# open-policy-agent/gatekeeper

Measured on AMD Instinct MI355X. Metric: AdmissionReview x constraint evals/sec, higher is better.
Workload: dtype u32; 1 GPU; configs[2]: pkg/audit sweep, 50 constraints x 1000000 mixed synthetic cluster objects (80% Pod, 10% Deployment, 5% Namespace, 5% Service/ConfigMap); constraints=50, reviews_total=1000000, reviews_rank0=1000000, rows_rank0=15859334, table_bytes_rank0=529437232, parallelism=1 GPU

## Files before the change

### gatekeeper_amd/_lib.py

```python
from __future__ import annotations

import atexit
import ctypes as C
import os

_HERE = os.path.dirname(os.path.abspath(__file__))
_ROOT = os.path.dirname(_HERE)

GK_OK = 0
GK_ERR_INVALID, GK_ERR_REGO, GK_ERR_UNSUPPORTED, GK_ERR_NOT_FOUND, GK_ERR_DEVICE, GK_ERR_REVIEW, GK_ERR_INTERNAL, GK_ERR_LIMIT = (
    -1, -2, -3, -4, -5, -6, -7, -8)
GK_REVIEW_ADMISSION_REQUEST, GK_REVIEW_OBJECT = 0, 1
GK_SRC_EMPTY, GK_SRC_ORIGINAL, GK_SRC_GENERATED, GK_SRC_ALL, GK_SRC_INVALID = 0, 1, 2, 3, 4
GK_TABLE_KEEP_DOCS = 1
GK_TABLE_RESIDENT = 2
GK_TABLE_KEEP_TEXT = 16
GK_TABLE_PRUNED = 32
GK_TABLE_PRE_MATCHED = 64
GK_TABLE_PROCESS_AUDIT = 4
GK_TABLE_PROCESS_WEBHOOK = 8
GK_REVIEW_EXCLUDED = 1
GK_EVAL_WANT_MATCH, GK_EVAL_NO_DOWNLOAD, GK_EVAL_WANT_LIST, GK_EVAL_ASYNC, GK_EVAL_COLLECT, GK_EVAL_TIME_EACH, GK_EVAL_KERNEL_ONLY = 1, 2, 4, 8, 16, 32, 64
GK_EVAL_DEVICE_ONLY = 128
GK_SWEEP_RESULT_TOTALS = 1
GK_VIOLATIONS_RENDER = 1

EXPORTS = [
    "gk_engine_create", "gk_engine_destroy", "gk_last_error", "gk_version", "gk_template_add", "gk_template_remove",
    "gk_constraint_add", "gk_constraint_remove", "gk_data_put", "gk_data_remove", "gk_excluder_replace", "gk_excluder_excluded", "gk_table_create", "gk_table_free",
    "gk_table_eval", "gk_eval_free", "gk_render", "gk_render_error", "gk_free", "gk_dump", "gk_table_topk", "gk_topk_free",
    "gk_table_totals", "gk_totals_free", "gk_table_get_stats", "gk_batcher_start", "gk_batcher_stop", "gk_query", "gk_query_ex", "gk_query_ex2",
    "gk_resident_sweep", "gk_sweep_free", "gk_resident_review", "gk_resident_review_ex", "gk_resident_audit", "gk_audit_free",
    "gk_resident_violations", "gk_violations_free", "gk_table_verify", "gk_verify_free", "gk_resident_verify",
    "gk_comm_unique_id", "gk_comm_init", "gk_comm_destroy", "gk_comm_info", "gk_table_sweep_sharded", "gk_shard_free",
    "gk_jit_quiesce", "gk_jit_cache_stats", "gk_jit_cache_dir", "gk_jit_cache_drop_memory", "gk_host_cpus", "gk_table_create_spool", "gk_spool_info_free", "gk_debug_set",
    "gk_synth_batch_create", "gk_synth_batch_reviews", "gk_synth_batch_size", "gk_synth_batch_json_bytes", "gk_synth_batch_free", "gk_synth_query_storm", "gk_synth_query_storm_ex",
]


GK_OPT_NO_REFERENTIAL, GK_OPT_GATHER_STATS, GK_OPT_TRACE = 1, 2, 4
GK_QUERY_TRACE = 1
GK_QUERY_PRE_MATCHED = 2


class gk_opts(C.Structure):
    _fields_ = [("device", C.c_int32), ("elem_cap", C.c_uint16 * 3), ("reserved", C.c_uint16), ("flags", C.c_uint32), ("reserved2", C.c_uint32),
                ("disabled_builtins", C.POINTER(C.c_char_p)), ("n_disabled_builtins", C.c_size_t)]


class gk_review_in(C.Structure):
    _fields_ = [("kind", C.c_int32), ("source", C.c_int32),
                ("json", C.c_char_p), ("json_len", C.c_size_t),
                ("namespace_json", C.c_char_p), ("namespace_len", C.c_size_t),
                ("ns_object_json", C.c_char_p), ("ns_object_len", C.c_size_t),
                ("operation", C.c_char_p)]


class gk_eval_out(C.Structure):
    _fields_ = [("n_reviews", C.c_uint32), ("n_constraints", C.c_uint32), ("n_tiles", C.c_uint32),
                ("constraint_ids", C.POINTER(C.c_uint32)),
                ("viol", C.POINTER(C.c_uint64)), ("err", C.POINTER(C.c_uint64)), ("match", C.POINTER(C.c_uint64)),
                ("too_big", C.POINTER(C.c_uint64)), ("counts", C.POINTER(C.c_uint32)), ("list", C.POINTER(C.c_uint32)),
                ("list_len", C.c_uint32), ("list_total", C.c_uint32), ("n_overflow", C.c_uint32),
                ("kernel_ms", C.c_float), ("fast_kernel_ms", C.c_float),
                ("algo_bytes", C.c_uint64), ("n_rows", C.c_uint64), ("n_launches", C.c_uint32), ("lds_bytes", C.c_uint32),
                ("d_viol", C.c_void_p), ("d_err", C.c_void_p), ("d_counts", C.c_void_p), ("n_rows_read", C.c_uint64),
                ("algo_bytes_once", C.c_uint64), ("n_plan_groups", C.c_uint32), ("n_host_evaluated", C.c_uint32),
                ("host_evaluated", C.POINTER(C.c_uint32)), ("kernel_text_hash", C.c_uint64)]


class gk_topk_out(C.Structure):
    _fields_ = [("n_constraints", C.c_uint32), ("stride", C.c_uint32), ("constraint_ids", C.POINTER(C.c_uint32)),
                ("counts", C.POINTER(C.c_uint32)), ("reviews", C.POINTER(C.c_uint32)), ("overflow", C.POINTER(C.c_uint32))]


class gk_totals_out(C.Structure):
    _fields_ = [("n_constraints", C.c_uint32), ("constraint_ids", C.POINTER(C.c_uint32)), ("results", C.POINTER(C.c_uint64)),
                ("pairs", C.POINTER(C.c_uint64)), ("rendered_pairs", C.c_uint64)]


class gk_table_stats(C.Structure):
    _fields_ = [("n_reviews", C.c_uint64), ("n_rows", C.c_uint64), ("json_bytes", C.c_uint64), ("heap_bytes", C.c_uint64),
                ("device_bytes", C.c_uint64), ("flatten_s", C.c_double), ("upload_s", C.c_double), ("host_threads", C.c_uint32),
                ("reserved", C.c_uint32), ("fast_reviews", C.c_uint64), ("digest", C.c_uint64)]


class gk_sweep_out(C.Structure):
    _fields_ = [("n_objects", C.c_uint64), ("n_constraints", C.c_uint32), ("n_chunks", C.c_uint32), ("constraint_ids", C.POINTER(C.c_uint32)),
                ("pairs", C.POINTER(C.c_uint64)), ("results", C.POINTER(C.c_uint64)), ("flattened", C.c_uint64), ("beyond_limits", C.c_uint64),
                ("sync_s", C.c_double), ("eval_s", C.c_double)]


class gk_audit_out(C.Structure):
    _fields_ = [("n_objects", C.c_uint64), ("n_constraints", C.c_uint32), ("stride", C.c_uint32), ("n_chunks", C.c_uint32),
                ("constraint_ids", C.POINTER(C.c_uint32)), ("pairs", C.POINTER(C.c_uint64)), ("results", C.POINTER(C.c_uint64)),
                ("counts", C.POINTER(C.c_uint32)), ("objects", C.POINTER(C.c_uint32)), ("overflow", C.POINTER(C.c_uint32)),
                ("n_paths", C.c_uint32), ("paths", C.POINTER(C.c_char_p)), ("beyond_limits", C.c_uint64), ("err_pairs", C.POINTER(C.c_uint64))]


class gk_violations_out(C.Structure):
    _fields_ = [("n_objects", C.c_uint64), ("n_constraints", C.c_uint32), ("n_chunks", C.c_uint32), ("mask_words", C.c_uint32),
                ("constraint_ids", C.POINTER(C.c_uint32)), ("total_objects", C.c_uint64), ("n_entries", C.c_uint32), ("paths", C.POINTER(C.c_char_p)),
                ("viol", C.POINTER(C.c_uint64)), ("err", C.POINTER(C.c_uint64)), ("results_json", C.POINTER(C.c_char_p)),
                ("beyond_limits", C.c_uint64), ("next_cursor", C.c_uint64)]


class gk_verify_entry(C.Structure):
    _fields_ = [("kind", C.c_uint32), ("row", C.c_uint32), ("review", C.c_uint32), ("specialised_bit", C.c_uint32)]


class gk_verify_out(C.Structure):
    _fields_ = [("n_reviews", C.c_uint32), ("n_constraints", C.c_uint32), ("n_plan_groups", C.c_uint32), ("constraint_ids", C.POINTER(C.c_uint32)),
                ("specialised_groups", C.c_uint32), ("kernel_text_hash", C.c_uint64),
                ("diff_viol", C.POINTER(C.c_uint64)), ("diff_err", C.POINTER(C.c_uint64)), ("diff_match", C.POINTER(C.c_uint64)),
                ("diff_too_big", C.c_uint64), ("diff_total", C.c_uint64), ("n_entries", C.c_uint32), ("entries_total", C.c_uint64),
                ("entries", C.POINTER(gk_verify_entry)), ("quarantined_groups", C.c_uint32),
                ("specialised_ms", C.c_float), ("bytecode_ms", C.c_float), ("diff_ms", C.c_float)]


GK_VERIFY_WANT_MATCH = 1
GK_VERIFY_QUARANTINE = 2
GK_VERIFY_KINDS = ("viol", "err", "match", "too_big")


class gk_shard_out(C.Structure):
    _fields_ = [("world", C.c_uint32), ("rank", C.c_uint32), ("n_constraints", C.c_uint32), ("stride_tiles", C.c_uint32), ("slot_bytes", C.c_uint64),
                ("constraint_ids", C.POINTER(C.c_uint32)), ("shard_reviews", C.POINTER(C.c_uint32)), ("totals", C.POINTER(C.c_int64)),
                ("gathered", C.POINTER(C.c_uint64)), ("d_gathered", C.c_void_p), ("kernel_ms", C.c_float), ("fast_kernel_ms", C.c_float),
                ("n_overflow", C.c_uint32), ("err_totals", C.POINTER(C.c_int64)), ("beyond_limits", C.c_int64), ("not_evaluated", C.c_int64),
                ("exchange_ms", C.c_float), ("exchange_overlapped", C.c_uint32), ("exchange_bytes_inbound", C.c_uint64)]


GK_SHARD_DOWNLOAD = 1
GK_SHARD_ENQUEUE = 2
GK_SHARD_COLLECT = 4
GK_COMM_ID_BYTES = 128
HE_ALLGATHER = C.CFUNCTYPE(None, C.c_void_p, C.c_void_p, C.c_uint64)
HE_ALLREDUCE = C.CFUNCTYPE(None, C.c_void_p, C.POINTER(C.c_longlong), C.c_uint64)


class gk_spool_info(C.Structure):
    _fields_ = [("n_files", C.c_uint64), ("n_reviews", C.c_uint64), ("n_unreadable", C.c_uint64), ("n_namespace_missing", C.c_uint64), ("bytes", C.c_uint64),
                ("names", C.POINTER(C.c_char_p)), ("n_folders_missing", C.c_uint64), ("statuses", C.POINTER(C.c_int32)), ("n_rejected", C.c_uint64),
                ("n_excluded", C.c_uint64)]


class gk_batch_opts(C.Structure):
    _fields_ = [("max_batch", C.c_uint32), ("window_us", C.c_uint32), ("workers", C.c_uint32), ("reserved", C.c_uint32)]


class gk_storm_out(C.Structure):
    _fields_ = [("calls", C.c_uint64), ("errors", C.c_uint64), ("seconds", C.c_double), ("p50_us", C.c_double), ("p90_us", C.c_double),
                ("p99_us", C.c_double), ("max_us", C.c_double), ("mean_batch", C.c_double), ("mean_queue_us", C.c_double),
                ("mean_device_us", C.c_double), ("results", C.c_uint64)]


class gk_query_stats(C.Structure):
    _fields_ = [("batch_size", C.c_uint32), ("reserved", C.c_uint32), ("queue_us", C.c_double), ("device_us", C.c_double),
                ("total_us", C.c_double)]


class EngineLoadError(RuntimeError):
    pass


def library_path(hostemu: bool = False) -> str:
    if hostemu:
        return os.path.join(_ROOT, "tests", "native", "libgkgpu_hostemu.so")
    return os.path.join(_HERE, "libgkgpu.so")


_cache = {}


def load(hostemu: bool | None = None):
    hostemu = bool(hostemu)
    if hostemu in _cache:
        return _cache[hostemu]
    path = library_path(hostemu)
    if not os.path.exists(path):
        raise EngineLoadError(
            "%s not found: build it with `python -c 'import __graft_entry__ as g; g.build()'` "
            "(there is no CPU fallback for the constraint-evaluation path)" % path)
    if not hostemu:
        try:
            import torch
        except ImportError:
            pass
    lib = C.CDLL(path)
    vp, cp, sz, u32 = C.c_void_p, C.c_char_p, C.c_size_t, C.c_uint32
    lib.gk_engine_create.argtypes = [C.POINTER(gk_opts), C.POINTER(vp)]
    lib.gk_engine_destroy.argtypes = [vp]
    lib.gk_engine_destroy.restype = None
    lib.gk_last_error.restype = cp
    lib.gk_version.restype = cp
    lib.gk_host_cpus.argtypes = []
    lib.gk_host_cpus.restype = C.c_uint32
    lib.gk_template_add.argtypes = [vp, cp, cp, C.POINTER(cp), sz]
    lib.gk_template_remove.argtypes = [vp, cp]
    lib.gk_constraint_add.argtypes = [vp, cp, sz, C.POINTER(u32)]
    lib.gk_constraint_remove.argtypes = [vp, cp, cp]
    lib.gk_data_put.argtypes = [vp, C.POINTER(cp), sz, cp, sz]
    lib.gk_data_remove.argtypes = [vp, C.POINTER(cp), sz]
    lib.gk_excluder_replace.argtypes = [vp, C.c_char_p, sz]
    lib.gk_excluder_excluded.argtypes = [vp, C.c_char_p, C.POINTER(gk_review_in), C.POINTER(C.c_int32)]
    lib.gk_table_create.argtypes = [vp, C.POINTER(gk_review_in), sz, u32, C.POINTER(C.c_int32), C.POINTER(vp)]
    lib.gk_table_free.argtypes = [vp]
    lib.gk_table_free.restype = None
    lib.gk_table_create_spool.argtypes = [vp, cp, cp, u32, u32, C.POINTER(C.POINTER(gk_spool_info)), C.POINTER(vp)]
    lib.gk_spool_info_free.argtypes = [C.POINTER(gk_spool_info)]
    lib.gk_spool_info_free.restype = None
    lib.gk_jit_quiesce.argtypes = []
    lib.gk_jit_quiesce.restype = None
    lib.gk_jit_cache_stats.argtypes = [C.POINTER(C.c_uint64), C.POINTER(C.c_uint64)]
    lib.gk_jit_cache_stats.restype = None
    lib.gk_jit_cache_dir.argtypes = []
    lib.gk_jit_cache_dir.restype = C.c_char_p
    lib.gk_jit_cache_drop_memory.argtypes = []
    lib.gk_jit_cache_drop_memory.restype = None
    lib.gk_table_eval.argtypes = [vp, vp, u32, C.POINTER(C.POINTER(gk_eval_out))]
    lib.gk_eval_free.argtypes = [C.POINTER(gk_eval_out)]
    lib.gk_eval_free.restype = None
    lib.gk_render.argtypes = [vp, vp, u32, u32, C.POINTER(vp)]
    lib.gk_render_error.argtypes = [vp, vp, u32, u32, C.POINTER(vp)]
    lib.gk_free.argtypes = [vp]
    lib.gk_free.restype = None
    lib.gk_dump.argtypes = [vp, C.POINTER(vp)]
    lib.gk_table_topk.argtypes = [vp, vp, u32, C.POINTER(C.POINTER(gk_topk_out))]
    lib.gk_topk_free.argtypes = [C.POINTER(gk_topk_out)]
    lib.gk_topk_free.restype = None
    lib.gk_comm_unique_id.argtypes = [C.c_char_p]
    lib.gk_comm_init.argtypes = [vp, C.c_char_p, C.c_int, C.c_int]
    lib.gk_comm_destroy.argtypes = [vp]
    lib.gk_comm_destroy.restype = None
    lib.gk_comm_info.argtypes = [vp, C.POINTER(C.c_int32), C.POINTER(C.c_int32)]
    lib.gk_table_sweep_sharded.argtypes = [vp, vp, u32, C.POINTER(C.POINTER(gk_shard_out))]
    lib.gk_shard_free.argtypes = [C.POINTER(gk_shard_out)]
    lib.gk_shard_free.restype = None
    if hostemu:
        lib.gk_comm_init_host.argtypes = [vp, C.c_int, C.c_int, HE_ALLGATHER, HE_ALLREDUCE, vp]
    lib.gk_resident_sweep.argtypes = [vp, u32, C.POINTER(C.POINTER(gk_sweep_out))]
    lib.gk_sweep_free.argtypes = [C.POINTER(gk_sweep_out)]
    lib.gk_sweep_free.restype = None
    lib.gk_resident_review.argtypes = [vp, C.POINTER(cp), sz, C.POINTER(vp)]
    lib.gk_resident_audit.argtypes = [vp, u32, u32, C.POINTER(C.POINTER(gk_audit_out))]
    lib.gk_audit_free.argtypes = [C.POINTER(gk_audit_out)]
    lib.gk_audit_free.restype = None
    lib.gk_resident_violations.argtypes = [vp, C.c_uint64, u32, u32, C.POINTER(C.POINTER(gk_violations_out))]
    lib.gk_violations_free.argtypes = [C.POINTER(gk_violations_out)]
    lib.gk_violations_free.restype = None
    lib.gk_table_verify.argtypes = [vp, vp, u32, u32, C.POINTER(C.POINTER(gk_verify_out))]
    lib.gk_verify_free.argtypes = [C.POINTER(gk_verify_out)]
    lib.gk_verify_free.restype = None
    lib.gk_resident_verify.argtypes = [vp, u32, u32, C.POINTER(C.POINTER(gk_verify_out)), C.POINTER(C.POINTER(cp))]
    lib.gk_batcher_start.argtypes = [vp, C.POINTER(gk_batch_opts)]
    lib.gk_batcher_stop.argtypes = [vp]
    lib.gk_batcher_stop.restype = None
    lib.gk_query.argtypes = [vp, C.POINTER(gk_review_in), C.POINTER(vp), C.POINTER(gk_query_stats)]
    lib.gk_query_ex.argtypes = [vp, C.POINTER(gk_review_in), u32, C.POINTER(vp), C.POINTER(vp), C.POINTER(gk_query_stats)]
    lib.gk_query_ex2.argtypes = [vp, C.POINTER(gk_review_in), C.POINTER(u32), sz, u32, C.POINTER(vp), C.POINTER(vp), C.POINTER(gk_query_stats)]
    lib.gk_resident_review_ex.argtypes = [vp, C.POINTER(cp), sz, C.POINTER(u32), sz, u32, C.POINTER(vp)]
    lib.gk_debug_set.argtypes = [cp, C.c_int64]
    lib.gk_table_get_stats.argtypes = [vp, C.POINTER(gk_table_stats)]
    lib.gk_table_totals.argtypes = [vp, vp, C.POINTER(C.POINTER(gk_totals_out))]
    lib.gk_totals_free.argtypes = [C.POINTER(gk_totals_out)]
    lib.gk_totals_free.restype = None
    lib.gk_synth_batch_create.argtypes = [C.c_uint64, C.c_uint64, C.c_uint64, C.c_int, C.POINTER(cp), sz, C.POINTER(vp)]
    lib.gk_synth_batch_reviews.argtypes = [vp]
    lib.gk_synth_batch_reviews.restype = C.POINTER(gk_review_in)
    lib.gk_synth_batch_size.argtypes = [vp]
    lib.gk_synth_batch_size.restype = sz
    lib.gk_synth_batch_json_bytes.argtypes = [vp]
    lib.gk_synth_batch_json_bytes.restype = C.c_uint64
    lib.gk_synth_batch_free.argtypes = [vp]
    lib.gk_synth_batch_free.restype = None
    lib.gk_synth_query_storm.argtypes = [vp, vp, u32, u32, C.POINTER(gk_storm_out)]
    lib.gk_synth_query_storm_ex.argtypes = [vp, vp, u32, u32, C.POINTER(u32), sz, u32, C.POINTER(gk_storm_out)]
    atexit.register(lib.gk_jit_quiesce)
    _cache[hostemu] = lib
    return lib
```

### gatekeeper_amd/csrc/device.hpp

```cpp
#pragma once
#include <cstdint>
#include <string>
#include <vector>

#include "flatten.hpp"
#include "lower.hpp"
#include "verify_merge.hpp"

namespace gk {

struct DevTable;
struct DevPlan;

struct EvalOptions {
  bool download = true;
  bool want_match = false;
  uint32_t list_capacity = 0;
  bool shard = false;
  bool detached = false;
  bool kernel_only = false;
  bool time_each = false;
  bool timed = true;
  bool jit_wait = true;
  bool bytecode = false;
};

struct EvalOut {
  uint32_t n_reviews = 0, n_constraints = 0, n_tiles = 0;
  std::vector<uint64_t> viol;
  std::vector<uint64_t> err;
  std::vector<uint64_t> match;
  std::vector<uint64_t> too_big;
  std::vector<uint32_t> counts;
  std::vector<uint32_t> list;
  uint32_t list_total = 0;
  uint32_t n_overflow = 0;
  float kernel_ms = 0;
  float fast_kernel_ms = 0;
  uint32_t n_launches = 0;
  uint32_t lds_bytes = 0;
  uint64_t list_bytes = 0;
  uint64_t kernel_hash = 0;
  bool specialised = false;
  const void *d_viol = nullptr, *d_err = nullptr, *d_counts = nullptr;
};

std::string dev_init(int device);
int dev_count();
struct DevPart;
DevPart* dev_part_upload(int device, HostTable& part);
void dev_part_free(DevPart* p);
DevTable* dev_table_assemble(int device, std::vector<DevPart*>& parts, const HostTable& meta);
void dev_table_free(DevTable* t);
DevTable* dev_table_view(DevTable* base);
uint64_t dev_table_bytes(const DevTable* t);
DevPlan* dev_plan_upload(int device, const HostPlan& fast, const HostPlan& big);
void dev_plan_free(DevPlan* p);
void dev_plan_no_jit(DevPlan* p);
void dev_eval(const DevPlan* p, const DevTable* t, const EvalOptions& opt, EvalOut* out);
void dev_topk(const DevTable* t, uint32_t nc, const std::vector<uint32_t>& order, const std::vector<uint32_t>& grp, uint32_t k, uint32_t cap,
              std::vector<uint32_t>* idx, std::vector<uint32_t>* n, std::vector<uint32_t>* ovf);
void dev_audit_select(const DevTable* t, uint32_t nc, uint32_t n_reviews, const std::vector<uint32_t>& order, const std::vector<uint32_t>& grp,
                      const std::vector<uint64_t>& shown, uint64_t shown_gen, uint32_t k, uint32_t cap,
                      std::vector<uint32_t>* pairs, std::vector<uint32_t>* idx, std::vector<uint32_t>* n, std::vector<uint32_t>* ovf);
void dev_viol_index(const DevTable* t, uint32_t nc, uint32_t n_reviews, const std::vector<uint64_t>& shown, uint64_t shown_gen,
                    std::vector<uint32_t>* cnt, std::vector<uint64_t>* any = nullptr);
void dev_viol_entries(const DevTable* t, uint32_t nc, uint32_t n_reviews, const std::vector<uint64_t>& shown, uint64_t shown_gen, uint32_t w0, uint32_t w1,
                      std::vector<uint32_t>* reviews, std::vector<uint64_t>* masks);
void dev_last_viol(const DevTable* t, uint32_t nc, std::vector<uint64_t>* viol);
void dev_verify_eval(const DevPlan* p, const DevTable* t, const EvalOptions& opt, EvalOut* out);
DevPlan* dev_verify_twin(int device, const HostPlan& fast, const HostPlan& big);
void dev_verify_forget(const DevTable* t);
void dev_verify_diff(const DevTable* a, const DevTable* b, uint32_t nc, uint32_t n_reviews, bool want_match, const std::vector<uint64_t>* mask,
                     uint32_t cap, VerifyDiff* out);
void dev_verify_flip(const DevTable* t, uint32_t nc, uint32_t kind, uint32_t row, uint32_t review, bool whole_word);
struct DevComm;
bool dev_comm_unique_id(char id[128], std::string* err);
DevComm* dev_comm_init(int device, const char id[128], int rank, int world, std::string* err);
void dev_comm_free(DevComm* c);
int dev_comm_rank(const DevComm* c);
int dev_comm_world(const DevComm* c);
bool dev_comm_query(const DevComm* c, int* rank, int* world, std::string* err);
struct ShardInfo {
  uint32_t stride_tiles = 0;
  uint64_t slot_bytes = 0;
  std::vector<uint32_t> shard_reviews;
};
void dev_shard_setup(DevTable* t, DevComm* c, uint32_t nc, ShardInfo* info);
void dev_shard_exchange(DevTable* t, DevComm* c, uint32_t nc, uint64_t not_evaluated, std::vector<int64_t>* totals,
                        std::vector<uint64_t>* gathered , const void** d_gathered);
struct ShardExchangeStats { float exchange_ms = 0; uint64_t inbound_bytes = 0; bool overlap = false; };
ShardExchangeStats dev_shard_exchange_stats(const DevTable* t, const DevComm* c);
void dev_shard_enqueue(const DevPlan* p, DevTable* t, DevComm* c, const EvalOptions& opt, uint32_t nc, uint64_t not_evaluated, bool allow_graph);
bool dev_shard_collect(DevTable* t, DevComm* c, uint32_t nc, std::vector<int64_t>* totals, std::vector<uint64_t>* gathered, const void** d_gathered);
void dev_jit_quiesce();
void dev_jit_cache_stats(uint64_t* hits, uint64_t* compiles);
void dev_jit_cache_drop_memory();
const char* dev_jit_cache_dir();
void dev_jit_prefetch(const DevPlan* p, const DevTable* t);
void dev_eval_launch(const DevPlan* p, const DevTable* t, const EvalOptions& opt);
void dev_eval_finish(const DevPlan* p, const DevTable* t, const EvalOptions& opt, EvalOut* out);

}
```

### gatekeeper_amd/csrc/embed_sources.py

```python
#!/usr/bin/env python3
import os
import sys

here = os.path.dirname(os.path.abspath(__file__))


def text(name):
    out = []
    for line in open(os.path.join(here, name), encoding="utf-8"):
        if line.startswith("#include") or line.startswith("#pragma once"):
            continue
        out.append(line)
    return "".join(out)


with open(sys.argv[1], "w", encoding="utf-8") as f:
    for var, name in (("kPlanHpp", "plan.hpp"), ("kVmCoreHpp", "vm_core.hpp"), ("kKernelBody", "kernel_body.inc")):
        f.write("static const char %s[] = R\"GKSRC(%s)GKSRC\";\n" % (var, text(name)))
```

### gatekeeper_amd/csrc/engine.cpp

```cpp
#include <atomic>
#include <cstring>
#include <dirent.h>
#include <algorithm>
#include <chrono>
#include <condition_variable>
#include <deque>
#include <functional>
#include <thread>
#include <map>
#include <set>
#include <unordered_map>
#include <unordered_set>
#include <memory>
#include <mutex>
#include <shared_mutex>
#include <sstream>

#include "../../include/gkgpu.h"
#include "audit_merge.hpp"
#include "codegen.hpp"
#include "device.hpp"
#include "flatten.hpp"
#include "lower.hpp"
#include "pe.hpp"
#include "regex.hpp"
#include "verify_merge.hpp"
#include "viol_stream.hpp"

using namespace gk;

static std::atomic<int64_t> g_debug_verify_flip{-1};
static std::atomic<int> g_debug_group_max{0};
namespace {

thread_local std::string g_err;
int fail(int code, const std::string& msg) { g_err = msg; return code; }

std::string lower_str(std::string s) { for (auto& c : s) if (c >= 'A' && c <= 'Z') c += 32; return s; }

struct ConstraintRec {
  uint32_t id;
  std::string kind, name;
  Value object, params, match;
  FP viol;
  MatchFormulas mf;
  std::shared_ptr<const PreparedConstraint> prep;
  std::shared_ptr<const PreparedConstraint> multi_prep;
  bool multi_ready = false;
  std::shared_ptr<const Template::CountForms> cforms;
  std::vector<Pattern> count_reads;
  std::vector<std::shared_ptr<const PreparedConstraint>> count_rows;
  std::shared_ptr<const PreparedConstraint> count_flag;
  bool count_ready = false;
  bool referential = false;
  std::string broken;
  bool alive = true;
};

bool wildcard_matches(const std::string& w, const std::string& c) {
  bool pre = !w.empty() && w.front() == '*', suf = !w.empty() && w.back() == '*';
  if (pre && suf) { std::string in = w.substr(1); if (!in.empty() && in.back() == '*') in.pop_back(); return c.find(in) != std::string::npos; }
  if (pre) { std::string s = w.substr(1); return c.size() >= s.size() && c.compare(c.size() - s.size(), s.size(), s) == 0; }
  if (suf) { std::string p = w.substr(0, w.size() - 1); return c.compare(0, p.size(), p) == 0; }
  return w == c;
}

std::string selector_error(const Value& sel) { return selector_error_text(sel); }

bool excluder_matches(const std::vector<std::string>& pats, const std::string& ns);
bool review_excluded(const std::vector<std::string>& pats, int kind, const Value& body) {
  if (!body.is_object()) return false;
  const Value* obj = &body;
  std::string ns;
  if (kind == GK_REVIEW_ADMISSION_REQUEST) {
    const Value* op = body.get("operation");
    const bool del = op && op->is_string() && op->str() == "DELETE";
    obj = body.get(del ? "oldObject" : "object");
    const Value* k = obj && obj->is_object() ? obj->get("kind") : nullptr;
    if (!k || !k->is_string() || k->str().empty()) return false;
    const Value* rns = body.get("namespace");
    if (rns && rns->is_string()) ns = rns->str();
  } else {
    ns = obj_string(*obj, "metadata", "namespace");
  }
  if (obj_is_namespace(*obj)) return excluder_matches(pats, obj_string(*obj, "metadata", "name"));
  return excluder_matches(pats, ns);
}

bool excluder_matches(const std::vector<std::string>& pats, const std::string& ns) {
  for (auto& w : pats) if (wildcard_matches(w, ns)) return true;
  return false;
}

std::string candidate_error(const Value& m, const Value& obj, const Value& ns, int source, bool* matched) {
  *matched = false;
  std::string g, v, k;
  obj_gvk(obj, &g, &v, &k);
  bool is_ns = k == "Namespace" && g.empty();
  std::string name = obj_string(obj, "metadata", "name"), nsfield = obj_string(obj, "metadata", "namespace");
  auto strs = [](const Value* l) { std::vector<std::string> o; if (l && l->is_array()) for (auto& x : l->items()) if (x.is_string()) o.push_back(x.str()); return o; };
  const Value* kinds = m.get("kinds");
  if (kinds && kinds->is_array() && kinds->size()) {
    bool any = false;
    for (auto& kk : kinds->items()) {
      auto ks = strs(kk.get("kinds")), gs = strs(kk.get("apiGroups"));
      auto has = [](const std::vector<std::string>& l, const std::string& x) { return l.empty() || std::find(l.begin(), l.end(), "*") != l.end() || std::find(l.begin(), l.end(), x) != l.end(); };
      if (has(ks, k) && has(gs, g)) any = true;
    }
    if (!any) return "";
  }
  std::string scope = obj_string(m, "scope");
  bool has_ns = !nsfield.empty() || ns.defined();
  if (scope == "Cluster" && !(is_ns || !has_ns)) return "";
  if (scope == "Namespaced" && !(!is_ns && has_ns)) return "";
  bool has_nsname = true;
  std::string nsname;
  if (is_ns) nsname = name; else if (ns.defined()) nsname = obj_string(ns, "metadata", "name"); else if (!nsfield.empty()) nsname = nsfield; else has_nsname = false;
  auto nss = strs(m.get("namespaces"));
  if (!nss.empty() && has_nsname) { bool any = false; for (auto& w : nss) if (wildcard_matches(w, nsname)) any = true; if (!any) return ""; }
  auto ex = strs(m.get("excludedNamespaces"));
  if (!ex.empty() && has_nsname) for (auto& w : ex) if (wildcard_matches(w, nsname)) return "";
  const Value* ls = m.get("labelSelector");
  if (ls && ls->is_object()) { std::string e = selector_error(*ls); if (!e.empty()) return e; }
  const Value* nsel = m.get("namespaceSelector");
  if (nsel && nsel->is_object() && !(!is_ns && !ns.defined() && nsfield.empty())) {
    std::string e = selector_error(*nsel);
    if (!e.empty()) return e;
    if (!is_ns && !ns.defined()) return "namespace selector for namespace-scoped object but missing Namespace";
  }
  std::string src = obj_string(m, "source");
  if (src.empty()) src = "All";
  if (src != "All" && src != "Original" && src != "Generated") return "invalid source field \"" + src + "\"";
  if (source == SRC_EMPTY && src != "All") return "source field not specified for resource " + name;
  if (src != "All" && source == SRC_INVALID) return "invalid source field";
  *matched = true;
  return "";
}

std::string autoreject_message(const Value& match, const ReviewDoc& doc) {
  const Value* obj = doc.request.get("object");
  const Value* old = doc.request.get("oldObject");
  if (obj && obj->is_object() && obj_string(*obj, "kind").empty())
    return "unable to match constraints: invalid request object: failed to unmarshal gkReview object " + to_json(*obj);
  if (old && old->is_object() && obj_string(*old, "kind").empty())
    return "unable to match constraints: invalid request object: failed to unmarshal gkReview oldObject " + to_json(*old);
  bool any = false;
  for (const Value* c : {obj, old}) {
    if (!c || !c->is_object()) continue;
    any = true;
    bool matched;
    std::string e = candidate_error(match, *c, doc.match_ns, doc.source, &matched);
    if (!e.empty())
      return "unable to match constraints: error matching the requested object: " + obj_string(*c, "metadata", "name") +
             " :failed to run Match criteria: " + e;
    if (matched) break;
  }
  if (!any) return "unable to match constraints: invalid request object: neither object nor old object are defined";
  return "unable to match constraints: error matching the requested object";
}

}

class HostWorkers {
 public:
  static HostWorkers& get() { static HostWorkers w; return w; }
  void run(size_t n, const std::function<void(size_t)>& fn) {
    if (n <= 1) { if (n) fn(0); return; }
    std::lock_guard<std::mutex> serial(run_mu_);
    {
      std::lock_guard<std::mutex> l(mu_);
      while (threads_.size() + 1 < n && threads_.size() < max_) threads_.emplace_back([this] { loop(); });
      fn_ = &fn; n_ = n; next_ = 0; done_ = 0; gen_++;
    }
    cv_.notify_all();
    work();
    std::unique_lock<std::mutex> l(mu_);
    done_cv_.wait(l, [&] { return done_ == n_; });
    fn_ = nullptr;
  }
  ~HostWorkers() {
    { std::lock_guard<std::mutex> l(mu_); stop_ = true; }
    cv_.notify_all();
    for (auto& t : threads_) t.join();
  }
// ... 1003 lines not shown
          const gk_review_in& r = reviews[i];
          if (i + 2 < hi && reviews[i + 2].json) {
            const char* nj = reviews[i + 2].json;
            const size_t nl = std::min<size_t>(reviews[i + 2].json_len, 4096);
            for (size_t o = 0; o < nl; o += 64) __builtin_prefetch(nj + o, 0, 1);
          }
          if (!slow_only) {
            RawReview rr;
            rr.kind = r.kind; rr.source = r.source; rr.json = r.json; rr.json_len = r.json_len;
            rr.ns_json = r.namespace_json; rr.ns_len = r.namespace_len; rr.nsobj_json = r.ns_object_json; rr.nsobj_len = r.ns_object_len;
            rr.operation = r.operation;
            int rc = fl.add_json(rr, e->ns_cache, &parts[w], &key_scratch, excl.empty() ? nullptr : &excl_fn);
            if (rc == Flattener::ADDED) { put_key(i, key_scratch); if (statuses) statuses[i] = GK_OK; part_fast[w]++; keep_if_big(i, parts[w]); continue; }
            if (rc == Flattener::EXCLUDED) {
              if (statuses) statuses[i] = GK_REVIEW_EXCLUDED;
              fl.add_skipped(&parts[w]);
              part_fast[w]++;
              continue;
            }
          }
          ReviewDoc doc;
          int st = GK_OK;
          try {
            Value body = parse_json(r.json, r.json_len);
            Value mns = parse_opt(r.namespace_json, r.namespace_len);
            Value nso = parse_opt(r.ns_object_json, r.ns_object_len);
            if (!excl.empty() && review_excluded(excl, r.kind, body)) {
              if (statuses) statuses[i] = GK_REVIEW_EXCLUDED;
              doc.request = Value::object({});
              fl.add_skipped(&parts[w]);
              if (keep) t->docs[i] = doc;
              continue;
            }
            if (r.kind == GK_REVIEW_OBJECT) doc = normalize_object(body, mns, nso, r.source, r.operation ? r.operation : "", e->ns_cache);
            else doc = normalize_admission_request(body, mns, nso, r.source, e->ns_cache);
          } catch (const std::exception& ex) {
            st = GK_ERR_REVIEW;
            t->review_errors[i] = ex.what();
            doc = ReviewDoc();
            doc.request = Value::object({});
          }
          if (statuses) statuses[i] = st;
          {
            const Value* o = doc.request.get("object");
            if (!o || !o->is_object()) o = doc.request.get("oldObject");
            std::string g_, v_, k_, key;
            if (o && o->is_object()) {
              obj_gvk(*o, &g_, &v_, &k_);
              key = g_; key.push_back('\0'); key += v_; key.push_back('\0'); key += k_; key.push_back('\0');
              key += obj_string(*o, "metadata", "namespace"); key.push_back('\0'); key += obj_string(*o, "metadata", "name");
            }
            put_key(i, key);
          }
          if (st == GK_ERR_REVIEW) fl.add_skipped(&parts[w]);
          else { fl.add(doc, &parts[w]); keep_if_big(i, parts[w]); }
          if (keep) t->docs[i] = doc;
        }
        fl.flush(&parts[w]);
      } catch (const std::exception& ex) { part_err[w] = ex.what(); }
    };
    auto run_threads = [&](const std::function<void(size_t)>& fn) {
      if (n_threads <= 1) { fn(0); return; }
      HostWorkers::get().run(n_threads, fn);
    };
    const bool want_digest = getenv("GK_TABLE_DIGEST") != nullptr;
    std::vector<std::vector<uint64_t>> part_digest(n_threads);
    auto digest_part = [&](size_t w) {
      const HostTable& P = parts[w];
      for (size_t tl = 0; tl + 0 < P.tile_seg.size(); tl++) {
        uint64_t d = 1469598103934665603ull;
        auto mix = [&](uint64_t v) { d ^= v; d *= 1099511628211ull; d ^= d >> 31; };
        const uint32_t s0 = P.tile_seg[tl], s1 = tl + 1 < P.tile_seg.size() ? P.tile_seg[tl + 1] : (uint32_t)P.segs.size();
        for (uint32_t sg = s0; sg < s1; sg++) {
          const uint32_t a = P.segs[sg].start, b = sg + 1 < P.segs.size() ? P.segs[sg + 1].start : (uint32_t)P.rows.size();
          for (uint32_t i = a; i < b; i++) {
            const Row& r = P.rows[i];
            mix(P.segs[sg].path); mix(((uint64_t)r.rev << 32) | r.meta);
            if ((r.meta & ROW_TYPE_MASK) == T_STRING && !(r.meta & ROW_STR_INLINE)) {
              uint32_t len; memcpy(&len, &P.heap[r.lo - 4], 4);
              mix(len); mix(r.hi);
              for (uint32_t k = 0; k < len; k++) mix(P.heap[r.lo + k]);
              for (int k = 0; k < 4; k++) mix(P.shdr[i].w[k]);
            } else mix(((uint64_t)r.hi << 32) | r.lo);
          }
        }
        part_digest[w].push_back(d);
      }
    };
    std::vector<DevPart*> dev_parts(n_threads, nullptr);
    std::vector<double> part_upload_s(n_threads, 0);
    run_threads([&](size_t w) {
      work(w);
      if (!part_err[w].empty()) return;
      try {
        if (want_digest) digest_part(w);
        const auto u0 = std::chrono::steady_clock::now();
        dev_parts[w] = dev_part_upload(e->opts.device, parts[w]);
        part_upload_s[w] = std::chrono::duration<double>(std::chrono::steady_clock::now() - u0).count();
      } catch (const std::exception& ex) { part_err[w] = ex.what(); }
    });
    for (auto& pe_ : part_err) if (!pe_.empty()) { for (DevPart* dp : dev_parts) dev_part_free(dp); return fail(GK_ERR_INTERNAL, pe_); }
    HostTable& H = t->host;
    H.rpt = rpt;
    {
      size_t rb = 0, hb = 0;
      for (size_t w = 0; w < n_threads; w++) {
        HostTable& P = parts[w];
        const uint32_t sb = (uint32_t)H.segs.size();
        for (const auto& sg : P.segs) H.segs.push_back({sg.path, (uint32_t)(sg.start + rb)});
        for (uint32_t ts : P.tile_seg) H.tile_seg.push_back(ts + sb);
        H.rflags.insert(H.rflags.end(), P.rflags.begin(), P.rflags.end());
        if (P.path_rows.size() > H.path_rows.size()) H.path_rows.resize(P.path_rows.size(), 0);
        for (size_t i = 0; i < P.path_rows.size(); i++) H.path_rows[i] += P.path_rows[i];
        if (P.path_max.size() > H.path_max.size()) H.path_max.resize(P.path_max.size(), 0);
        for (size_t i = 0; i < P.path_max.size(); i++) H.path_max[i] = std::max(H.path_max[i], P.path_max[i]);
        rb += P.n_rows_total; hb += P.heap_total;
        t->stats.fast_reviews += part_fast[w];
        H.n_reviews += P.n_reviews;
      }
      if (rb >= 0xFFFFFFF0ull || hb >= 0xFFFFFFF0ull) {
        for (DevPart* dp : dev_parts) dev_part_free(dp);
        return fail(GK_ERR_INVALID, "table too large for 32-bit row/heap offsets: split the batch");
      }
      t->n_rows = rb;
      t->stats.heap_bytes = hb;
      H.n_rows_total = rb;
    }
    if (prem || (flags & GK_TABLE_PRE_MATCHED))
      for (size_t i = 0; i < n && i < H.rflags.size(); i++) if ((flags & GK_TABLE_PRE_MATCHED) || prem[i]) { H.rflags[i] |= RF_PREMATCHED; t->any_prematched = true; }
    Flattener::build_index(&t->host);
    if (want_digest) {
      uint64_t d = 1469598103934665603ull;
      auto mix = [&](uint64_t v) { d ^= v; d *= 1099511628211ull; d ^= d >> 31; };
      for (auto& pd : part_digest) for (uint64_t x : pd) mix(x);
      for (uint32_t f : H.rflags) mix(f);
      for (uint32_t sp : H.slot_path) mix(sp);
      for (size_t i = 0; i < n; i++) for (unsigned char c : t->obj_key(i)) mix(c);
      t->stats.digest = d;
    }
    const auto t_indexed = std::chrono::steady_clock::now();
    t->dev = dev_table_assemble(e->opts.device, dev_parts, t->host);
    const auto t_up = std::chrono::steady_clock::now();
    t->n_reviews = (uint32_t)n;
    t->dir_bytes = t->host.rflags.size() * 4;
    t->slot_path = t->host.slot_path;
    t->path_rows = t->host.path_rows;
    t->path_max = t->host.path_max;
    t->resident = (flags & GK_TABLE_RESIDENT) != 0;
    t->stats.n_reviews = n; t->stats.n_rows = t->n_rows; t->stats.host_threads = (uint32_t)n_threads;
    t->stats.device_bytes = dev_table_bytes(t->dev);
    t->stats.upload_s = std::chrono::duration<double>(t_up - t_indexed).count();
    t->stats.flatten_s = std::chrono::duration<double>(t_indexed - t_begin).count();
    for (size_t i = 0; i < n; i++) t->stats.json_bytes += reviews[i].json_len;
    t->host.tile_idx.clear(); t->host.tile_idx.shrink_to_fit();
    *out = t.release();
    return GK_OK;
  } catch (const std::exception& ex) { return fail(GK_ERR_DEVICE, ex.what()); }
}

namespace {
struct SpoolHolder {
  gk_spool_info pub;
  std::vector<std::string> names;
  std::vector<const char*> ptrs;
  std::vector<int32_t> statuses;
};
bool read_file(const std::string& path, std::string* out) {
  FILE* f = fopen(path.c_str(), "rb");
  if (!f) return false;
  char buf[65536];
  size_t n;
  out->clear();
  while ((n = fread(buf, 1, sizeof buf, f)) > 0) out->append(buf, n);
  const bool ok = !ferror(f);
  fclose(f);
  return ok;
}
}

int gk_table_create_spool(gk_engine* e, const char* api_cache_dir, const char* kind, uint32_t folders, uint32_t flags,
                          gk_spool_info** info, gk_table** out) {
  if (!e || !api_cache_dir || !kind || !out) return fail(GK_ERR_INVALID, "NULL argument");
  try {
    std::unique_ptr<SpoolHolder> h(new SpoolHolder());
    memset(&h->pub, 0, sizeof h->pub);
    struct Item { std::string name, text, ns_text; };
    std::vector<Item> items;
    for (uint32_t fo = 0; fo < folders; fo++) {
      const std::string sub = std::string(kind) + "_" + std::to_string(fo), dir = std::string(api_cache_dir) + "/" + sub;
      std::vector<std::string> files;
      if (DIR* d = opendir(dir.c_str())) {
        while (dirent* de = readdir(d)) { if (de->d_name[0] != '.') files.emplace_back(de->d_name); }
        closedir(d);
      } else h->pub.n_folders_missing++;
      std::sort(files.begin(), files.end(), [](const std::string& a, const std::string& b) { return a.size() != b.size() ? a.size() < b.size() : a < b; });
      for (const std::string& fn : files) {
        h->pub.n_files++;
        Item it;
        it.name = sub + "/" + fn;
        if (!read_file(dir + "/" + fn, &it.text)) { h->pub.n_unreadable++; continue; }
        h->pub.bytes += it.text.size();
        items.push_back(std::move(it));
      }
    }
    std::unordered_map<std::string, std::string> ns_json;
    std::vector<Item> kept;
    for (Item& it : items) {
      std::string nsname;
      try {
        Value v = parse_json(it.text.data(), it.text.size());
        if (!v.is_object()) { h->pub.n_unreadable++; continue; }
        nsname = obj_string(v, "metadata", "namespace");
      } catch (const std::exception&) { h->pub.n_unreadable++; continue; }
      if (!nsname.empty()) {
        auto f = ns_json.find(nsname);
        if (f == ns_json.end()) {
          Value ns = e->ns_cache.get(nsname);
          f = ns_json.emplace(nsname, ns.defined() ? to_json(ns) : std::string()).first;
        }
        if (f->second.empty()) { h->pub.n_namespace_missing++; continue; }
        it.ns_text = f->second;
      }
      kept.push_back(std::move(it));
    }
    std::vector<gk_review_in> rins(kept.size());
    for (size_t i = 0; i < kept.size(); i++) {
      gk_review_in& r = rins[i];
      memset(&r, 0, sizeof r);
      r.kind = GK_REVIEW_OBJECT;
      r.source = GK_SRC_ORIGINAL;
      r.json = kept[i].text.data(); r.json_len = kept[i].text.size();
      if (!kept[i].ns_text.empty()) {
        r.namespace_json = kept[i].ns_text.data(); r.namespace_len = kept[i].ns_text.size();
        r.ns_object_json = kept[i].ns_text.data(); r.ns_object_len = kept[i].ns_text.size();
      }
      h->names.push_back(kept[i].name);
    }
    h->statuses.assign(std::max<size_t>(1, kept.size()), GK_OK);
    int rc = gk_table_create(e, rins.data(), rins.size(), flags, h->statuses.data(), out);
    if (rc != GK_OK) return rc;
    h->statuses.resize(kept.size());
    h->pub.n_reviews = kept.size();
    h->pub.statuses = h->statuses.data();
    for (int32_t st : h->statuses) { if (st == GK_REVIEW_EXCLUDED) h->pub.n_excluded++; else if (st != GK_OK) h->pub.n_rejected++; }
    if ((*out)->texts.size() == kept.size() && !kept.empty()) (*out)->owned_text = std::make_shared<std::vector<Item>>(std::move(kept));
    for (auto& nm : h->names) h->ptrs.push_back(nm.c_str());
    h->pub.names = h->ptrs.data();
    if (info) *info = &h.release()->pub;
    return GK_OK;
  } catch (const std::exception& ex) { return fail(GK_ERR_INTERNAL, ex.what()); }
}

void gk_spool_info_free(gk_spool_info* info) { if (info) delete reinterpret_cast<SpoolHolder*>(info); }

int gk_table_get_stats(const gk_table* t, gk_table_stats* out) {
  if (!t || !out) return fail(GK_ERR_INVALID, "NULL argument");
  *out = t->stats;
  return GK_OK;
}

void gk_table_free(gk_table* t) {
  if (!t) return;
  for (DevTable* v : t->views) dev_table_free(v);
  for (DevTable* v : t->tviews) dev_table_free(v);
  for (DevTable* v : t->views) dev_verify_forget(v);
  for (DevTable* v : t->vviews) { dev_verify_forget(v); dev_table_free(v); }
  for (DevPlan* p : t->vtwins) dev_plan_free(p);
  dev_verify_forget(t->dev);
  dev_table_free(t->dev);
  delete t;
}

struct EvalHolder {
  gk_eval_out pub;
  uint32_t lds_bytes = 0;
  EvalOut out;
  std::vector<uint32_t> ids;
  std::vector<uint32_t> host_evaluated;
};
static void complete_on_host(gk_engine* e, gk_table* t, EvalHolder* h, bool want_match, bool want_list);

int gk_table_eval(gk_engine* e, gk_table* t, uint32_t flags, gk_eval_out** out) {
  if (!e || !t || !out) return fail(GK_ERR_INVALID, "NULL argument");
  try {
    ensure_plan(e);
    if (t->dict_gen != e->dict_reg.gen())
      return fail(GK_ERR_INVALID, "the table was flattened before a constraint with dictionary predicates was added (its <leaf>.$d rows are missing): create it again");
    if (t->pruned && t->reads_gen != e->dict_reg.reads_gen())
      return fail(GK_ERR_INVALID, "the pruned table was flattened before a constraint that reads other key paths was added (GK_TABLE_PRUNED): create it again");
    std::unique_ptr<EvalHolder> h(new EvalHolder());
    EvalOptions opt;
    opt.download = !(flags & GK_EVAL_NO_DOWNLOAD);
    opt.want_match = flags & GK_EVAL_WANT_MATCH;
    opt.time_each = (flags & GK_EVAL_TIME_EACH) != 0;
    opt.kernel_only = (flags & GK_EVAL_KERNEL_ONLY) != 0 && (flags & GK_EVAL_ASYNC) != 0;
    opt.timed = !(flags & GK_EVAL_ASYNC) || opt.time_each || opt.kernel_only;
    opt.jit_wait = t->resident || t->n_reviews >= 8192;
    {
      { std::lock_guard<std::mutex> gate(e->plan_gate); }
      std::shared_lock<std::shared_mutex> l(e->plan_rw);
      h->ids = e->plan_ids;
      if (flags & GK_EVAL_WANT_LIST) opt.list_capacity = std::max<uint32_t>(1024, t->n_reviews * 4u);
      const HostPlan* hp = nullptr;
      DevPlan* dp = nullptr;
      { std::lock_guard<std::mutex> vl(e->variants_mu); dp = plan_for_table(e, t, &hp); }
      while (t->views.size() < e->extra.size()) t->views.push_back(dev_table_view(t->dev));
      std::vector<DevPlan*> gdev(e->extra.size(), nullptr);
      { std::lock_guard<std::mutex> vl(e->variants_mu); for (size_t gi = 0; gi < e->extra.size(); gi++) { const HostPlan* gh = nullptr; gdev[gi] = plan_for_group(e, t, gi + 1, &gh); } }
      if (!(flags & GK_EVAL_COLLECT)) {
        if (!e->extra.empty() && opt.jit_wait) { dev_jit_prefetch(dp, t->dev); for (size_t gi = 0; gi < e->extra.size(); gi++) dev_jit_prefetch(gdev[gi], t->views[gi]); }
        dev_eval_launch(dp, t->dev, opt);
        for (size_t gi = 0; gi < e->extra.size(); gi++) dev_eval_launch(gdev[gi], t->views[gi], opt);
      }
      if (flags & GK_EVAL_ASYNC) {
        *out = nullptr;
        return GK_OK;
      }
      dev_eval_finish(dp, t->dev, opt, &h->out);
      h->lds_bytes = h->out.lds_bytes;
      for (size_t gi = 0; gi < e->extra.size(); gi++) {
        EvalOut og;
        dev_eval_finish(gdev[gi], t->views[gi], opt, &og);
        const uint32_t row_base = h->out.n_constraints;
        EvalOut& o = h->out;
        o.viol.insert(o.viol.end(), og.viol.begin(), og.viol.end());
        o.err.insert(o.err.end(), og.err.begin(), og.err.end());
        o.match.insert(o.match.end(), og.match.begin(), og.match.end());
        o.counts.insert(o.counts.end(), og.counts.begin(), og.counts.end());
        for (size_t k = 0; k + 1 < og.list.size(); k += 2) { o.list.push_back(og.list[k] + row_base); o.list.push_back(og.list[k + 1]); }
        for (size_t k = 0; k < og.too_big.size() && k < o.too_big.size(); k++) o.too_big[k] |= og.too_big[k];
        o.list_total += og.list_total;
        o.n_overflow += og.n_overflow;
        o.kernel_ms += og.kernel_ms; o.fast_kernel_ms += og.fast_kernel_ms;
        o.list_bytes += og.list_bytes;
        o.kernel_hash = o.kernel_hash * 1099511628211ull ^ og.kernel_hash;
        o.n_constraints += og.n_constraints;
        o.d_viol = o.d_err = o.d_counts = nullptr;
        h->ids.insert(h->ids.end(), e->extra[gi]->ids.begin(), e->extra[gi]->ids.end());
      }
    }
    if (opt.download && !(flags & GK_EVAL_DEVICE_ONLY)) complete_on_host(e, t, h.get(), opt.want_match, (flags & GK_EVAL_WANT_LIST) != 0);
    else if (opt.download) { std::lock_guard<std::mutex> hl(t->host_mu); t->host_viol.clear(); t->host_err.clear(); t->host_ids.clear(); }
    gk_eval_out& p = h->pub;
    memset(&p, 0, sizeof p);
    p.n_host_evaluated = (uint32_t)h->host_evaluated.size();
    p.host_evaluated = h->host_evaluated.empty() ? nullptr : h->host_evaluated.data();
    p.n_reviews = h->out.n_reviews; p.n_constraints = h->out.n_constraints; p.n_tiles = h->out.n_tiles;
    p.constraint_ids = h->ids.data();
    p.viol = h->out.viol.data(); p.err = h->out.err.data();
    p.match = h->out.match.empty() ? nullptr : h->out.match.data();
    p.too_big = h->out.too_big.data();
    p.counts = h->out.counts.data();
    p.list = h->out.list.data(); p.list_len = (uint32_t)(h->out.list.size() / 2); p.list_total = h->out.list_total;
    p.n_overflow = h->out.n_overflow;
    p.kernel_ms = h->out.kernel_ms; p.fast_kernel_ms = h->out.fast_kernel_ms; p.n_launches = h->out.n_launches;
    p.d_viol = h->out.d_viol; p.d_err = h->out.d_err; p.d_counts = h->out.d_counts;
    p.n_rows = t->n_rows;
    t->last_nc = p.n_constraints; t->last_ids = h->ids;
    p.lds_bytes = h->lds_bytes;
    p.kernel_text_hash = h->out.kernel_hash;
    uint64_t rows_read = 0, hdrs_read = 0, bound = 0, plan_bytes = 0;
    std::vector<uint8_t> seen(t->slot_path.size(), 0);
    uint64_t rows_once = 0, hdrs_once = 0;
    auto account = [&](const HostPlan& hp) {
      for (size_t si = 0; si < t->slot_path.size(); si++) {
        const uint32_t pth = t->slot_path[si];
        if (pth >= hp.ptab.size() || !hp.ptab[pth]) continue;
        bound++;
        uint64_t n = pth < t->path_rows.size() ? t->path_rows[pth] : 0;
        rows_read += n;
        uint32_t ent = hp.ptab[pth];
        bool str = false;
        for (uint32_t j = 0; j < (ent & 0xFF); j++) str = str || pred_needs_str(hp.path_preds[(ent >> 8) + j]);
        if (str) hdrs_read += n;
        static const bool dbg_path_rows = getenv("GK_DEBUG_PATH_ROWS") != nullptr;
        if (dbg_path_rows) fprintf(stderr, "[gkgpu paths] %-70s rows %9llu preds %3u%s\n", e->dict.to_string(pth).c_str(), (unsigned long long)n, ent & 0xFF, str ? " +hdr" : "");
        if (!(seen[si] & 1)) { seen[si] |= 1; rows_once += n; }
        if (str && !(seen[si] & 2)) { seen[si] |= 2; hdrs_once += n; }
      }
      plan_bytes += (uint64_t)hp.path_preds.size() * sizeof(Pred) + hp.code.size() * 4 + hp.cheap.size();
    };
    {
      std::shared_lock<std::shared_mutex> l(e->plan_rw);
      account(e->fast);
      for (auto& g : e->extra) account(g->fast);
    }
    p.n_rows_read = rows_read;
    (void)bound;
    p.algo_bytes = rows_read * sizeof(Row) + hdrs_read * sizeof(StrHdr) + h->out.list_bytes +
                   t->dir_bytes * (1 + e->extra.size()) + plan_bytes + (uint64_t)p.n_constraints * p.n_tiles * 16 + (uint64_t)p.list_total * 8;
    p.algo_bytes_once = p.algo_bytes - (rows_read - rows_once) * sizeof(Row) - (hdrs_read - hdrs_once) * sizeof(StrHdr) - t->dir_bytes * e->extra.size();
    p.n_plan_groups = 1 + (uint32_t)e->extra.size();
    *out = &h.release()->pub;
    return GK_OK;
  } catch (const Unsupported& ex) { return fail(GK_ERR_UNSUPPORTED, ex.what());
  } catch (const std::exception& ex) { return fail(GK_ERR_DEVICE, ex.what()); }
}

struct TopkHolder {
  gk_topk_out pub;
  std::vector<uint32_t> ids, counts, reviews, overflow;
};

static void table_key_order(gk_table* t) {
  if (t->order.size() == t->n_reviews) return;
  t->order.resize(t->n_reviews);
  for (uint32_t i = 0; i < t->n_reviews; i++) t->order[i] = i;
  std::stable_sort(t->order.begin(), t->order.end(), [&](uint32_t a, uint32_t b) { return t->obj_key(a) < t->obj_key(b); });
  t->grp.resize(t->n_reviews);
  uint32_t gid = 0;
  for (uint32_t p = 0; p < t->n_reviews; p++) {
    if (p && t->obj_key(t->order[p]) != t->obj_key(t->order[p - 1])) gid++;
    t->grp[p] = gid;
  }
}

int gk_table_topk(gk_engine* e, gk_table* t, uint32_t k, gk_topk_out** out) {
  if (!e || !t || !out) return fail(GK_ERR_INVALID, "NULL argument");
  try {
    table_key_order(t);
    std::unique_ptr<TopkHolder> h(new TopkHolder());
    const uint32_t cap = k + 64;
    h->ids = t->last_ids;
    {
      std::shared_lock<std::shared_mutex> l(e->plan_rw);
      const uint32_t nc0 = (uint32_t)e->plan_ids.size();
      dev_topk(t->dev, nc0, t->order, t->grp, k, cap, &h->reviews, &h->counts, &h->overflow);
      for (size_t gi = 0; gi < e->extra.size() && gi < t->views.size(); gi++) {
        std::vector<uint32_t> r, c, o;
        dev_topk(t->views[gi], (uint32_t)e->extra[gi]->ids.size(), t->order, t->grp, k, cap, &r, &c, &o);
        h->reviews.insert(h->reviews.end(), r.begin(), r.end());
        h->counts.insert(h->counts.end(), c.begin(), c.end());
        h->overflow.insert(h->overflow.end(), o.begin(), o.end());
      }
    }
    std::vector<std::pair<uint32_t, uint32_t>> hv;
    { std::lock_guard<std::mutex> hl(t->host_mu); if (t->host_ids == h->ids) hv = t->host_viol; }
    if (!hv.empty()) {
      std::vector<std::unordered_set<uint32_t>> have(h->counts.size());
      for (auto& hp : hv) {
        const uint32_t row = hp.first;
        if (row >= h->counts.size()) continue;
        uint32_t* lst = &h->reviews[(size_t)row * cap];
        if (have[row].empty()) have[row].insert(lst, lst + h->counts[row]);
        if (!have[row].insert(hp.second).second) continue;
        if (h->counts[row] < cap) lst[h->counts[row]++] = hp.second; else h->overflow[row] = 1;
      }
    }
    h->pub.n_constraints = t->last_nc; h->pub.stride = cap;
    h->pub.constraint_ids = h->ids.data(); h->pub.counts = h->counts.data(); h->pub.reviews = h->reviews.data(); h->pub.overflow = h->overflow.data();
    *out = &h.release()->pub;
    return GK_OK;
  } catch (const std::exception& ex) { return fail(GK_ERR_DEVICE, ex.what()); }
}

struct TotalsHolder {
  gk_totals_out pub;
  std::vector<uint32_t> ids;
  std::vector<uint64_t> results, pairs;
};

static ReviewDoc make_doc(gk_engine* e, const gk_review_in& in) {
  Value body = parse_json(in.json, in.json_len);
  Value mns = parse_opt(in.namespace_json, in.namespace_len);
  Value nso = parse_opt(in.ns_object_json, in.ns_object_len);
  if (in.kind == GK_REVIEW_OBJECT) return normalize_object(body, mns, nso, in.source, in.operation ? in.operation : "", e->ns_cache);
  return normalize_admission_request(body, mns, nso, in.source, e->ns_cache);
}
static const ReviewDoc* doc_for(gk_engine* e, const gk_table* t, uint32_t r, ReviewDoc* tmp) {
  if (r < t->docs.size()) return &t->docs[r];
  if (r < t->texts.size()) { *tmp = make_doc(e, t->texts[r]); return tmp; }
  auto it = t->big_texts.find(r);
  if (it != t->big_texts.end()) { const gk_review_in in = it->second.in(); *tmp = make_doc(e, in); return tmp; }
  return nullptr;
}

static Value strip_object(const Value& o) {
  if (!o.is_object()) return o;
  ValuePairs keep;
  for (auto& kv : o.pairs()) if (kv.first.is_string() && (kv.first.str() == "apiVersion" || kv.first.str() == "kind" || kv.first.str() == "metadata")) keep.push_back(kv);
  return Value::object(std::move(keep));
}
static thread_local int tl_host_completion_depth = 0;
static constexpr size_t GK_HOST_COMPLETIONS_MAX = 4096;
static void complete_on_host(gk_engine* e, gk_table* t, EvalHolder* h, bool want_match, bool want_list) {
  EvalOut& o = h->out;
  static const bool env_off = [] { const char* off = getenv("GK_HOST_EVAL"); return off && atoi(off) == 0; }();
  static const bool dbg = getenv("GK_DEBUG_HOST") != nullptr;
  auto why = [&](uint32_t r, const char* what) { if (dbg) fprintf(stderr, "[gkgpu host] review %u stays refused: %s\n", r, what); };
  std::vector<std::pair<uint32_t, uint32_t>> add_viol, add_err;
  struct Publish {
    gk_table* t; EvalHolder* h; std::vector<std::pair<uint32_t, uint32_t>>*v, *er;
    ~Publish() { std::lock_guard<std::mutex> hl(t->host_mu); t->host_viol.swap(*v); t->host_err.swap(*er); t->host_ids = h->ids; }
  } publish{t, h, &add_viol, &add_err};
  if (env_off || tl_host_completion_depth > 0) return;
  struct Depth { Depth() { tl_host_completion_depth++; } ~Depth() { tl_host_completion_depth--; } } depth_guard;
  const uint32_t nt = o.n_tiles, nc = o.n_constraints;
  if (nc == 0 || h->ids.size() != nc) return;
  struct Cand { uint32_t r; gk_review_in in; bool prem; std::string stext; int mrow = -1; };
  std::vector<Cand> cands;
  for (uint32_t w = 0; w < nt && w < o.too_big.size(); w++)
    for (uint64_t m = o.too_big[w]; m; m &= m - 1) {
      const uint32_t r = w * GK_TILE + (uint32_t)__builtin_ctzll(m);
      if (r >= t->n_reviews) continue;
      if (cands.size() >= GK_HOST_COMPLETIONS_MAX) { why(r, "more refused reviews than one evaluation completes"); continue; }
      Cand c;
      c.r = r;
      if (r < t->texts.size()) c.in = t->texts[r];
      else { auto it = t->big_texts.find(r); if (it == t->big_texts.end()) { why(r, "no text kept"); continue; } c.in = it->second.in(); }
      c.prem = r < t->host.rflags.size() && (t->host.rflags[r] & RF_PREMATCHED) != 0;
      cands.push_back(std::move(c));
    }
  if (cands.empty()) return;
  std::vector<gk_review_in> sins;
  for (Cand& c : cands) {
    if (c.prem) continue;
    try {
      Value body = parse_json(c.in.json, c.in.json_len);
      if (!body.is_object()) { why(c.r, "not an object"); continue; }
      Value stripped;
      if (c.in.kind == GK_REVIEW_OBJECT) stripped = strip_object(body);
      else {
        ValuePairs kv = body.pairs();
        for (auto& pr : kv) if (pr.first.is_string() && (pr.first.str() == "object" || pr.first.str() == "oldObject")) pr.second = strip_object(pr.second);
        stripped = Value::object(std::move(kv));
      }
      c.stext = to_json(stripped);
      c.mrow = (int)sins.size();
      sins.push_back(c.in);
    } catch (const std::exception& ex) { why(c.r, ex.what()); }
  }
  for (Cand& c : cands) if (c.mrow >= 0) { sins[c.mrow].json = c.stext.data(); sins[c.mrow].json_len = c.stext.size(); }
  gk_table* mt = nullptr;
  gk_eval_out* mo = nullptr;
  std::vector<int32_t> mst(sins.size(), GK_OK);
  std::unique_ptr<gk_table, void (*)(gk_table*)> mt_guard(nullptr, gk_table_free);
  std::unique_ptr<gk_eval_out, void (*)(gk_eval_out*)> mo_guard(nullptr, gk_eval_free);
  bool match_ok = sins.empty();
  if (!sins.empty()) {
    if (gk_table_create(e, sins.data(), sins.size(), 0, mst.data(), &mt) == GK_OK && mt) {
      mt_guard.reset(mt);
      if (gk_table_eval(e, mt, GK_EVAL_WANT_MATCH | GK_EVAL_DEVICE_ONLY, &mo) == GK_OK && mo) {
// ... 1369 lines not shown
    std::lock_guard<std::mutex> l(B.mu);
    if (!B.running) return;
    B.stop = true;
  }
  B.cv.notify_all();
  for (auto& w : B.workers) w.join();
  std::lock_guard<std::mutex> l(B.mu);
  B.workers.clear();
  B.running = false;
  B.stop = false;
  for (auto* r : B.queue) { r->status = GK_ERR_INVALID; r->error = "the admission batcher was stopped"; r->done = true; r->cv.notify_one(); }
  B.queue.clear();
}

int gk_query(gk_engine* e, const gk_review_in* review, char** results_json, gk_query_stats* stats) { return gk_query_ex(e, review, 0, results_json, nullptr, stats); }

static std::string query_trace(gk_engine* e, const char* where, const std::string& results, const gk_query_stats* st, const std::vector<uint32_t>* wanted = nullptr) {
  std::ostringstream os;
  os << "gkgpu trace: evaluated " << where;
  if (st) os << "; batch of " << st->batch_size << " review(s), queued " << (long long)(st->queue_us * 1e3) << " ns, device " << (long long)(st->device_us * 1e3) << " ns";
  os << "\n";
  std::map<uint32_t, std::vector<std::string>> by;
  try {
    Value rows = parse_json(results.data(), results.size());
    if (rows.is_array()) for (const Value& r : rows.items()) {
      const Value* c = r.get("constraint"); const Value* m = r.get("msg"); const Value* ar = r.get("autoreject");
      if (c && c->is_number() && m && m->is_string()) by[(uint32_t)c->i].push_back(std::string(ar ? "autoreject: " : "violation: ") + m->str());
    }
  } catch (const std::exception&) {}
  std::shared_lock<std::shared_mutex> l(e->mu);
  for (const ConstraintRec& c : e->constraints) {
    if (!c.alive || (wanted && !std::binary_search(wanted->begin(), wanted->end(), c.id))) continue;
    os << "  constraint " << c.kind << "/" << c.name << " (id " << c.id << "): ";
    auto it = by.find(c.id);
    if (it == by.end()) { os << (wanted ? "no result\n" : "no result (does not match, or matches and is satisfied)\n"); continue; }
    os << it->second.size() << " result(s)\n";
    for (auto& m : it->second) os << "    " << m << "\n";
  }
  return os.str();
}

int gk_query_ex(gk_engine* e, const gk_review_in* review, uint32_t qflags, char** results_json, char** trace_out, gk_query_stats* stats) {
  return gk_query_ex2(e, review, nullptr, 0, qflags, results_json, trace_out, stats);
}

int gk_query_ex2(gk_engine* e, const gk_review_in* review, const uint32_t* constraint_ids, size_t n_constraints, uint32_t qflags,
                 char** results_json, char** trace_out, gk_query_stats* stats) {
  if (!e || !review || !results_json) return fail(GK_ERR_INVALID, "NULL argument");
  if (trace_out) *trace_out = nullptr;
  const bool pre_matched = (qflags & GK_QUERY_PRE_MATCHED) != 0;
  std::vector<uint32_t> wanted_v;
  const std::vector<uint32_t>* wanted = nullptr;
  if (constraint_ids) {
    int rc = wanted_ids(e, constraint_ids, n_constraints, &wanted_v);
    if (rc != GK_OK) return rc;
    wanted = &wanted_v;
    if (wanted_v.empty()) {
      if (stats) memset(stats, 0, sizeof *stats);
      return put_string("[]", results_json);
    }
  }
  const bool want_trace = trace_out && ((qflags & GK_QUERY_TRACE) || (e->opts.flags & GK_OPT_TRACE));
  auto put_trace = [&](const char* where, const std::string& js, const gk_query_stats* st) {
    if (!want_trace) return;
    const std::string t = query_trace(e, where, js, st, wanted);
    char* b = (char*)malloc(t.size() + 1);
    memcpy(b, t.c_str(), t.size() + 1);
    *trace_out = b;
  };
  if (!pre_matched && review->kind == GK_REVIEW_OBJECT && review->source == GK_SRC_EMPTY && review->json && !(review->operation && *review->operation)) {
    gk_engine::Resident& R = e->resident;
    std::unique_lock<std::mutex> rl(R.mu, std::try_to_lock);
    if (rl.owns_lock() && R.swept) {
      auto it = R.by_text.find(text_hash(review->json, review->json_len));
      if (it != R.by_text.end()) {
        const gk_engine::ResObj& o = R.objs[it->second];
        const gk_review_in want = resident_review_in(R, o);
        auto same = [](const char* a, size_t an, const char* b, size_t bn) { return (an == 0 && bn == 0) || (a && b && an == bn && memcmp(a, b, an) == 0); };
        if (o.alive && same(o.json.data(), o.json.size(), review->json, review->json_len) &&
            same(want.namespace_json, want.namespace_len, review->namespace_json, review->namespace_len) &&
            same(want.ns_object_json, want.ns_object_len, review->ns_object_json, review->ns_object_len)) {
          std::string js, err;
          int st = GK_OK;
          try {
            if (resident_answer(e, it->second, &js, &st, &err, false, wanted)) {
              if (stats) { stats->batch_size = 0; stats->queue_us = 0; stats->device_us = 0; stats->total_us = 0; }
              if (st != GK_OK) return fail(st, err);
              char* buf = (char*)malloc(js.size() + 1);
              memcpy(buf, js.c_str(), js.size() + 1);
              *results_json = buf;
              put_trace("from the resident sweep's bitmaps (the review is a swept object: no flatten, no launch)", js, nullptr);
              return GK_OK;
            }
          } catch (const std::exception&) {  }
        }
      }
    }
  }
  gk_engine::Request req;
  req.in = review;
  req.pre_matched = pre_matched;
  req.arrived = std::chrono::steady_clock::now();
  gk_engine::Batcher& B = e->batcher;
  for (;;) {
    std::unique_lock<std::mutex> l(B.mu);
    if (B.running && !B.stop) {
      B.queue.push_back(&req);
      B.cv.notify_all();
      req.cv.wait(l, [&] { return req.done; });
      break;
    }
    if (B.stop) return fail(GK_ERR_INVALID, "the admission batcher is shutting down");
    l.unlock();
    int rc = gk_batcher_start(e, nullptr);
    if (rc != GK_OK) return rc;
  }
  std::string results;
  bool on_host = false;
  if (req.status == GK_OK && req.batch) {
    try {
      bool too_big = false;
      for (uint32_t k = 0; k < req.batch->ev->n_host_evaluated; k++) on_host = on_host || req.batch->ev->host_evaluated[k] == req.index;
      results = query_results_json(e, req.batch->table, *req.batch->ev, req.index, *review, &too_big, wanted);
      if (too_big) { req.status = GK_ERR_LIMIT; req.error = "review is beyond the engine's limits (more than 255 elements in an array that constraint predicates iterate, or an object where they iterate array elements)"; }
    } catch (const RegoError& ex) { req.status = GK_ERR_REGO; req.error = ex.what();
    } catch (const std::exception& ex) { req.status = GK_ERR_INTERNAL; req.error = ex.what(); }
    req.batch.reset();
  }
  if (stats) {
    stats->batch_size = req.batch_size;
    stats->queue_us = req.queue_us;
    stats->device_us = req.device_us;
    stats->total_us = std::chrono::duration<double, std::micro>(std::chrono::steady_clock::now() - req.arrived).count();
  }
  if (req.status != GK_OK) return fail(req.status, req.error);
  char* buf = (char*)malloc(results.size() + 1);
  memcpy(buf, results.c_str(), results.size() + 1);
  *results_json = buf;
  gk_query_stats mine{};
  mine.batch_size = req.batch_size; mine.queue_us = req.queue_us; mine.device_us = req.device_us;
  put_trace(on_host ? (pre_matched ? "by the host evaluator (the review is beyond the device's limits; pre-matched by the caller: violation sets by the concrete evaluator)"
                                   : "by the host evaluator (the review is beyond the device's limits: match layer from the stripped review on the device, violation sets by the concrete evaluator)")
                    : (pre_matched ? "on the device (pre-matched by the caller: violation bitmaps of the batch's one launch; messages rendered by the host evaluator for the flagged pairs)"
                                   : "on the device (match + violation bitmaps of the batch's one launch; messages rendered by the host evaluator for the flagged pairs)"), results, &mine);
  return GK_OK;
}

int gk_debug_set(const char* key, int64_t value) {
  if (!key) return fail(GK_ERR_INVALID, "NULL argument");
  if (strcmp(key, "dict_facts") == 0) { g_debug_dict_facts.store(value != 0); return GK_OK; }
  if (strcmp(key, "group_max") == 0) { g_debug_group_max.store((int)std::max<int64_t>(0, std::min<int64_t>(value, 1 << 20))); return GK_OK; }
  if (strcmp(key, "verify_flip") == 0) { g_debug_verify_flip.store(value < 0 ? -1 : value); return GK_OK; }
  if (strcmp(key, "fold_match_labels") == 0) { g_test_fold_match_labels.store(value != 0); return GK_OK; }
  return fail(GK_ERR_NOT_FOUND, std::string("gk_debug_set: unknown key ") + key);
}

void gk_jit_quiesce(void) { dev_jit_quiesce(); }
void gk_jit_cache_drop_memory(void) { dev_jit_cache_drop_memory(); }
const char* gk_jit_cache_dir(void) { return dev_jit_cache_dir(); }
void gk_jit_cache_stats(uint64_t* cache_hits, uint64_t* compiles) {
  uint64_t h = 0, c = 0;
  dev_jit_cache_stats(&h, &c);
  if (cache_hits) *cache_hits = h;
  if (compiles) *compiles = c;
}

int gk_dump(gk_engine* e, char** text_out) {
  if (!e || !text_out) return fail(GK_ERR_INVALID, "NULL argument");
  try {
    ensure_plan(e);
    std::ostringstream os;
    std::shared_lock<std::shared_mutex> l(e->plan_rw);
    const HostPlan& p = e->fast;
    os << "constraints=" << p.dims.n_constraints << " viol_formulas=" << p.n_viol << " match_formulas=" << p.n_match
       << " preds=" << p.dims.n_preds << " scopes=" << p.dims.n_scopes << " code_words=" << p.dims.n_code
       << " gwords=" << p.dims.n_gwords << " acc_words=" << p.dims.acc_words << " lds_bytes_per_64_reviews=" << p.dims.acc_words * 256
       << " paths=" << p.dims.n_paths << "\n";
    for (size_t i = 0; i < p.preds.size(); i++)
      os << "pred " << i << " op=" << (int)p.preds[i].op << " dst=" << (int)p.preds[i].dst << " scope=" << (int)p.preds[i].scope
         << " bit=" << p.preds[i].bit << " " << pattern_to_string(p.pred_patterns[i]) << "\n";
    {
      std::shared_lock<std::shared_mutex> rl(e->mu);
      for (auto& c : e->constraints) if (c.alive) os << "constraint " << c.id << " " << c.kind << "/" << c.name << " viol: " << f_to_string(c.viol) << "\n";
    }
    std::string s = os.str();
    char* buf = (char*)malloc(s.size() + 1);
    memcpy(buf, s.c_str(), s.size() + 1);
    *text_out = buf;
    return GK_OK;
  } catch (const std::exception& ex) { return fail(GK_ERR_INTERNAL, ex.what()); }
}

}
```

### gatekeeper_amd/csrc/jit_source.hpp

```cpp
#pragma once
#include <algorithm>
#include <cstdio>
#include <cstdlib>
#include <stdexcept>
#include <string>
#include <vector>

#include "codegen.hpp"
#include "lower.hpp"
#include "plan.hpp"

namespace gk {

constexpr size_t GK_LDS_PER_CU = 160 * 1024;

inline int jit_block_of(uint32_t rpt) {
  static const int forced = getenv("GK_JIT_BLOCK") ? atoi(getenv("GK_JIT_BLOCK")) : 0;
  if (forced >= (int)rpt && forced <= 1024 && forced % (int)rpt == 0 && forced % GK_TILE == 0) return forced;
  return gk_block_of((int)rpt);
}
inline uint32_t list_cap_of(int block) { return (uint32_t)std::min(block / GK_TILE, 8) * GK_WAVE_CHUNKS; }
inline uint32_t jit_list_cap(int block, uint32_t need) {
  static const bool trim = !(getenv("GK_JIT_LIST_TRIM") && atoi(getenv("GK_JIT_LIST_TRIM")) == 0);
  const uint32_t full = list_cap_of(block);
  if (!trim || need == 0) return full;
  return std::min(full, std::max<uint32_t>(128u, (need + 127u) / 128u * 128u));
}
inline uint32_t jit_tot_k(uint32_t n_constraints) {
  static const bool on = !(getenv("GK_FUSED_TOTALS") && atoi(getenv("GK_FUSED_TOTALS")) == 0);
  return on && n_constraints && n_constraints <= 256u ? (n_constraints + 63u) / 64u * 64u : 0u;
}
constexpr size_t GK_LDS_PER_CU_MEASURED = 157696;
inline size_t jit_static_lds_exact(uint32_t rpt, uint32_t res_k, uint32_t list_cap, uint32_t tot_k) {
  const size_t list = (size_t)list_cap * 8, masks = (size_t)(rpt / GK_TILE) * res_k * 8;
  return 2 * list + (masks <= list ? 0 : masks) + GK_TILE * 4 + (size_t)tot_k * 4;
}
inline uint32_t jit_tot_k(uint32_t n_constraints, size_t dyn_lds, uint32_t rpt, int block, uint32_t res_k, uint32_t list_cap) {
  const uint32_t tk = jit_tot_k(n_constraints);
  if (!tk || !list_cap) return tk;
  const size_t by_waves = std::max<size_t>(1, 32 / (size_t)std::max(1, block / GK_TILE));
  const size_t with = std::min(by_waves, GK_LDS_PER_CU_MEASURED / (dyn_lds + jit_static_lds_exact(rpt, res_k, list_cap, tk)));
  const size_t without = std::min(by_waves, GK_LDS_PER_CU_MEASURED / (dyn_lds + jit_static_lds_exact(rpt, res_k, list_cap, 0)));
  return with < without ? 0u : tk;
}
inline size_t static_lds_of(uint32_t rpt, int block, uint32_t res_k, uint32_t list_cap = 0, uint32_t tot_k = 0) {
  const size_t list = (size_t)(list_cap ? list_cap : list_cap_of(block)) * 8;
  const size_t masks = (size_t)(rpt / GK_TILE) * (res_k ? res_k : (uint32_t)(GK_MAX_VIOL + 2 * GK_MAX_RES)) * 8;
  const size_t bounds = res_k ? 0 : (size_t)(block / GK_TILE) * GK_MAX_SCOPES * 4;
  return 2 * list + (masks <= list ? 8 : masks) + bounds + GK_TILE * 4 + 64 + (size_t)tot_k * 4;
}
inline size_t max_dyn_lds_of(uint32_t rpt) { return GK_LDS_PER_CU - static_lds_of(rpt, gk_block_of((int)rpt), 0) - 256; }
inline size_t max_dyn_lds_jit(uint32_t rpt, uint32_t res_k, uint32_t list_cap = 0, uint32_t tot_k = 0) { return GK_LDS_PER_CU - static_lds_of(rpt, jit_block_of(rpt), res_k, list_cap, tot_k) - 256; }

inline std::string jit_res_macros() {
  static const bool lanes = !(getenv("GK_JIT_RES_LANES") && atoi(getenv("GK_JIT_RES_LANES")) == 0);
  const std::string bit =
      "#ifndef GK_BIT\nstatic __device__ inline uint32_t gk_bit(uint32_t b) { asm volatile(\"\" : \"+v\"(b)); return b & 1u; }\n#define GK_BIT(b) gk_bit(b)\n#endif\n";
  const std::string base = bit +
      "#define GK_RES_BASE(kind) ((kind) == 0 ? 0u : (kind) == 1 ? (uint32_t)GK_RES_KV : (kind) == 2 ? (uint32_t)(GK_RES_KV + GK_RES_KM) : ((uint32_t)(kind) - 2u) * 64u)\n";
  if (!lanes)
    return base +
           "#define GK_RES_PROLOGUE const bool gk_l0 = GK_LANE_ID() == 0u;\n"
           "#define GK_RES(kind, slot, b) do { const unsigned long long m_ = __ballot(GK_BIT(b) != 0u); if (gk_l0) masks[GK_RES_BASE(kind) + (slot)] = m_; } while (0)\n"
           "#define GK_RES_FLUSH(m0, m1, m2, m3, m4, m5)\n";
  std::string pro = "#define GK_RES_PROLOGUE uint32_t", flush = "#define GK_RES_FLUSH(m0, m1, m2, m3, m4, m5) do { const uint32_t l_ = GK_LANE_ID() & 63u; ", voids;
  for (int k = 0; k < 2 + GK_VIOL_WORDS; k++) {
    const std::string ks = std::to_string(k);
    pro += std::string(k ? "," : "") + " gk_rl" + ks + " = 0u, gk_rh" + ks + " = 0u";
    flush += "if (((unsigned long long)(m" + ks + ") >> l_) & 1ull) masks[GK_RES_BASE(" + ks + ") + l_] = ((unsigned long long)gk_rh" + ks + " << 32) | gk_rl" + ks + "; ";
    voids += "(void)gk_rl" + ks + "; (void)gk_rh" + ks + "; ";
  }
  return base + pro + ";\n"
         "#define GK_RES(kind, slot, b) do { const unsigned long long m_ = __ballot(GK_BIT(b) != 0u); GK_WRITELANE2(m_, slot, gk_rl##kind, gk_rh##kind); } while (0)\n" +
         flush + voids + "} while (0)\n";
}

inline std::string assemble_jit_source(const HostPlan& plan, uint32_t rpt, uint32_t rpp, const char* plan_hpp,
                                       const char* vm_core_hpp, const char* kernel_body, uint32_t list_cap = 0) {
  std::string src =
      "typedef unsigned char uint8_t; typedef unsigned short uint16_t; typedef unsigned int uint32_t; typedef unsigned long long uint64_t;\n"
      "typedef short int16_t; typedef int int32_t; typedef long long int64_t;\n";
  src += plan_hpp;
  src += vm_core_hpp;
  src += "#define GK_LANE_ID() __builtin_amdgcn_mbcnt_hi(~0u, __builtin_amdgcn_mbcnt_lo(~0u, 0u))\n"
         "static __device__ inline void gk_writelane2(unsigned long long m, const uint32_t l, uint32_t& lo, uint32_t& hi) {\n"
         "  asm(\"s_nop 1\\n\\tv_writelane_b32 %0, %2, %4\\n\\tv_writelane_b32 %1, %3, %4\" : \"+v\"(lo), \"+v\"(hi) : \"s\"((uint32_t)m), \"s\"((uint32_t)(m >> 32)), \"n\"(l)); }\n"
         "#define GK_WRITELANE2(m, l, lo, hi) gk_writelane2((m), (l), (lo), (hi))\n";
  src += jit_res_macros();
  const int block = jit_block_of(rpt);
  src += generate_plan_source(plan, (uint32_t)(block / GK_TILE / ((int)rpt / GK_TILE)));
  if (block != gk_block_of((int)rpt)) src += "#define GK_BLOCK_K " + std::to_string(block) + "\n";
  {
    const size_t per_group = (size_t)plan.dims.acc_words * rpp * 4 + static_lds_of(rpt, block, jit_res_k(plan), list_cap, jit_tot_k(plan.dims.n_constraints, (size_t)plan.dims.acc_words * rpp * 4, rpt, block, jit_res_k(plan), list_cap ? list_cap : list_cap_of(block)));
    const size_t groups_per_cu = std::max<size_t>(1, GK_LDS_PER_CU / per_group);
    int waves = (int)std::min<size_t>(8, std::max<size_t>(block / 256, groups_per_cu * (block / GK_TILE) / 4));
    if (const char* w = getenv("GK_JIT_WAVES")) waves = atoi(w);
    src += "#define GK_TILES_BOUNDS __launch_bounds__(" + std::to_string(block) + ", " + std::to_string(waves) + ")\n";
  }
  {
    int depth = 1;
    if (const char* d = getenv("GK_JIT_PREFETCH")) depth = std::max(1, std::min(8, atoi(d)));
    src += "#define GK_PREFETCH " + std::to_string(depth) + "\n";
  }
  {
    int prio = 3003;
    if (const char* pm = getenv("GK_JIT_PRIO")) prio = std::max(0, std::min(3333, atoi(pm)));
    if (prio) src += "#define GK_PRIO_LEVELS " + std::to_string(prio) + "\n";
    int part0 = 1;
    if (const char* pp = getenv("GK_JIT_PRIO_PART0")) part0 = std::max(0, std::min(3, atoi(pp)));
    if (prio && part0) src += "#define GK_PRIO_PART0 " + std::to_string(part0) + "\n";
  }
  if (getenv("GK_KERNEL_PROF") || getenv("GK_DBG_PHASE")) src += "#define GK_WITH_PROF 1\n";
  src += "#define GK_RPT_K " + std::to_string(rpt) + "\n#define GK_RPP_K " + std::to_string(rpp) + "\n";
  if (list_cap) src += "#define GK_LIST_CAP_K " + std::to_string(list_cap) + "\n";
  if (const uint32_t tk = jit_tot_k(plan.dims.n_constraints, (size_t)plan.dims.acc_words * rpp * 4, rpt, block, jit_res_k(plan), list_cap ? list_cap : list_cap_of(block))) src += "#define GK_TOT_K " + std::to_string(tk) + "\n";
  if (const char* defs = getenv("GK_JIT_DEFINES")) {
    std::string d = defs, item;
    for (size_t i = 0; i <= d.size(); i++) {
      if (i < d.size() && d[i] != ';') { item.push_back(d[i]); continue; }
      if (!item.empty()) { size_t eq = item.find('='); src += "#define " + (eq == std::string::npos ? item : item.substr(0, eq) + " " + item.substr(eq + 1)) + "\n"; }
      item.clear();
    }
  }
  src += "namespace gk {\n#define GK_KERNEL_TILES gk_jit_tiles\n#define GK_KERNEL_BIG gk_jit_big\n#define GK_KERNEL_LINKAGE extern \"C\"\n#define GK_SKIP_BIG\n"
         "#define GK_ROW_FN(r, i, ent, h, pv, heap, acc, on) jit_row(r, ent, h, heap, acc, on)\n#define GK_BIND_ALWAYS_STR 0\n"
         "#define GK_FORMULA_FN(pv, acc, flags, rows, heap, bounds) jit_formulas(pv, acc, flags, rows, heap, bounds)\n";
  if (const char* bf = getenv("GK_JIT_BODY_FILE")) {
    FILE* f = fopen(bf, "r");
    if (!f) throw std::runtime_error(std::string("GK_JIT_BODY_FILE: cannot open ") + bf);
    std::string body, line;
    char buf[4096];
    while (fgets(buf, sizeof buf, f)) { line = buf; if (line.rfind("#include", 0) != 0 && line.rfind("#pragma once", 0) != 0) body += line; }
    fclose(f);
    src += body;
  } else src += kernel_body;
  src += "}\n";
  return src;
}

}
```

### gatekeeper_amd/csrc/kernels.hip

```cpp
#include <hip/hip_runtime.h>
#include <hip/hiprtc.h>
#include <dlfcn.h>
#include <sys/wait.h>
#include <spawn.h>
#include <unistd.h>
#include <cstring>
#include <cerrno>

#include <cstdio>
#include <cstdlib>
#include <atomic>
#include <condition_variable>
#include <list>
#include <map>
#include <thread>
#include <memory>
#include <mutex>
#include <stdexcept>
#include <string>
#include <vector>

extern char** environ;

#include "chunks.hpp"
#include "code_cache.hpp"
#include "codegen.hpp"
#include "device.hpp"
#include "jit_source.hpp"
#include "shard_pipe.hpp"
#include "jit_sources.inc"
#include "vm_core.hpp"

namespace gk {

#define HIP_OK(expr)                                                                                          \
  do {                                                                                                        \
    hipError_t e_ = (expr);                                                                                   \
    if (e_ != hipSuccess) throw std::runtime_error(std::string("HIP error: ") + hipGetErrorString(e_) + " at " #expr); \
  } while (0)

namespace {
struct DevPool {
  std::mutex mu;
  std::map<size_t, std::vector<void*>> free_;
  std::map<void*, size_t> class_of;
  size_t cached = 0;
};
DevPool& pool() { static DevPool p; return p; }
constexpr size_t kPoolMaxBlock = 32u << 20, kPoolMaxCached = 2048ull << 20;
std::mutex g_hip_alloc_mu;
hipError_t hip_malloc_serial(void** out, size_t bytes) { std::lock_guard<std::mutex> l(g_hip_alloc_mu); return hipMalloc(out, bytes); }
void hip_free_serial(void* p) { std::lock_guard<std::mutex> l(g_hip_alloc_mu); (void)hipFree(p); }
}
static size_t pool_max_block() {
  static const size_t v = [] { const char* mb = getenv("GK_DEVICE_POOL_BLOCK_MB"); return mb ? (size_t)std::max(0, atoi(mb)) << 20 : kPoolMaxBlock; }();
  return v;
}
static hipError_t pool_malloc(void** out, size_t bytes) {
  if (bytes > pool_max_block()) return hip_malloc_serial(out, bytes);
  size_t bytes_cls = 256;
  while (bytes_cls < bytes) bytes_cls <<= 1;
  int dev = 0;
  (void)hipGetDevice(&dev);
  const size_t cls = bytes_cls | ((size_t)dev << 48);
  DevPool& P = pool();
  {
    std::lock_guard<std::mutex> l(P.mu);
    auto it = P.free_.find(cls);
    if (it != P.free_.end() && !it->second.empty()) { *out = it->second.back(); it->second.pop_back(); P.cached -= bytes_cls; return hipSuccess; }
  }
  hipError_t e = hip_malloc_serial(out, bytes_cls);
  if (e == hipSuccess) { std::lock_guard<std::mutex> l(P.mu); P.class_of[*out] = cls; }
  return e;
}
static void pool_free(void* p) {
  if (!p) return;
  DevPool& P = pool();
  {
    std::lock_guard<std::mutex> l(P.mu);
    auto it = P.class_of.find(p);
    if (it != P.class_of.end()) {
      const size_t b = it->second & ((1ull << 48) - 1);
      if (P.cached + b <= kPoolMaxCached) { P.free_[it->second].push_back(p); P.cached += b; return; }
      P.class_of.erase(it);
    }
  }
  hip_free_serial(p);
}
template <class T>
static hipError_t pool_malloc(T** out, size_t bytes) { return pool_malloc(reinterpret_cast<void**>(out), bytes); }

namespace {
struct StreamPool { std::mutex mu; std::map<int, std::vector<hipStream_t>> free_; };
StreamPool& stream_pool() { static StreamPool p; return p; }
}
static hipStream_t stream_acquire(int device) {
  {
    StreamPool& P = stream_pool();
    std::lock_guard<std::mutex> l(P.mu);
    auto& v = P.free_[device];
    if (!v.empty()) { hipStream_t s = v.back(); v.pop_back(); return s; }
  }
  hipStream_t s = nullptr;
  if (hipStreamCreateWithFlags(&s, hipStreamNonBlocking) != hipSuccess) { (void)hipGetLastError(); return nullptr; }
  return s;
}
static void stream_release(int device, hipStream_t s) {
  if (!s) return;
  (void)hipStreamSynchronize(s);
  StreamPool& P = stream_pool();
  std::lock_guard<std::mutex> l(P.mu);
  auto& v = P.free_[device];
  if (v.size() < 96) v.push_back(s); else hipStreamDestroy(s);
}

namespace {
struct PinPool { std::mutex mu; std::map<size_t, std::vector<uint8_t*>> free_; size_t cached = 0; };
PinPool& pin_pool() { static PinPool p; return p; }
}
static uint8_t* pinned_acquire(size_t bytes, size_t* cap) {
  size_t c = 4096;
  while (c < bytes) c <<= 1;
  {
    PinPool& P = pin_pool();
    std::lock_guard<std::mutex> l(P.mu);
    auto it = P.free_.find(c);
    if (it != P.free_.end() && !it->second.empty()) { uint8_t* p = it->second.back(); it->second.pop_back(); P.cached -= c; *cap = c; return p; }
  }
  uint8_t* p = nullptr;
  if (hipHostMalloc(reinterpret_cast<void**>(&p), c, hipHostMallocDefault) != hipSuccess) { (void)hipGetLastError(); *cap = 0; return nullptr; }
  *cap = c;
  return p;
}
static void pinned_release(uint8_t* p, size_t cap) {
  if (!p) return;
  PinPool& P = pin_pool();
  {
    std::lock_guard<std::mutex> l(P.mu);
    if (P.cached + cap <= ((size_t)256 << 20)) { P.free_[cap].push_back(p); P.cached += cap; return; }
  }
  hipHostFree(p);
}

struct Work;
struct AuditSide {
  uint64_t* d_shown = nullptr;
  uint64_t shown_gen = 0;
  uint32_t *d_order = nullptr, *d_grp = nullptr;
  ~AuditSide() { pool_free(d_shown); pool_free(d_order); pool_free(d_grp); }
};
struct ViolIndex {
  uint64_t* d_any = nullptr;
  uint32_t* d_off = nullptr;
  std::vector<uint32_t> off;
  uint32_t nc = 0, pw = 0;
  uint64_t shown_gen = 0;
  ~ViolIndex() { pool_free(d_any); pool_free(d_off); }
};
struct DevTable {
  Work* work = nullptr;
  std::shared_ptr<AuditSide> audit = std::make_shared<AuditSide>();
  std::shared_ptr<ViolIndex> vidx = std::make_shared<ViolIndex>();
  hipStream_t stream = nullptr;
  Row* rows = nullptr;
  StrHdr* shdr = nullptr;
  uint32_t* tile_idx = nullptr;
  uint32_t* rflags = nullptr;
  uint8_t* heap = nullptr;
  uint32_t n_reviews = 0, n_rows = 0, n_slots = 0;
  uint64_t bytes = 0;
  int device = 0;
  uint32_t rpt = GK_RPT_MIN;
  std::vector<uint32_t> slot_path;
  std::shared_ptr<const std::vector<uint32_t>> h_tile_idx;
  struct Binding { uint64_t plan_id = 0; Bind* d = nullptr; uint32_t n = 0; ChunkDesc* lists = nullptr; uint32_t capg = 1; uint64_t list_bytes = 0; };
  Binding bind_fast, bind_big;
  bool is_view = false;
  uint64_t chunk_need_plan = 0;
  uint32_t chunk_need = 0;
  uint64_t launch_plan = 0;
  uint32_t launch_rpp = 0, launch_lcap = 0;
  void* launch_jit = nullptr;
};

struct DevPlanVariant {
  uint32_t* ptab = nullptr;
  Pred* preds = nullptr;
  Scope* scopes = nullptr;
  uint32_t* code = nullptr;
  uint8_t* cheap = nullptr;
  PlanDims dims{};
  PlanView view() const { return PlanView{ptab, preds, scopes, code, cheap, dims}; }
};

struct JitKernel {
  hipModule_t module = nullptr;
  hipFunction_t tiles = nullptr;
  size_t max_dyn_lds = 64 * 1024;
  std::string source;
  uint64_t source_hash = 0;
  uint32_t tot_k = 0;
};
struct JitSlot {
  std::mutex mu;
  std::condition_variable cv;
  enum State { PENDING, READY, FAILED } state = PENDING;
  std::unique_ptr<JitKernel> k;
  std::string error;
  bool abandoned = false;
  ~JitSlot() { if (k && k->module) hipModuleUnload(k->module); }
};

struct DevPlan {
  uint64_t id = 0;
  int device = 0;
  std::vector<uint32_t> ptab_fast, ptab_big;
  DevPlanVariant fast, big;
  ConstraintSlot* slots = nullptr;
  uint32_t n_constraints = 0;
  bool want_jit = false;
  HostPlan host_fast;
  std::mutex jit_mu;
  std::map<uint32_t, std::shared_ptr<JitSlot>> jit;
  std::vector<uint32_t> cls;
  std::vector<uint32_t> path_cost;
  uint32_t res_k = GK_MAX_VIOL + 2 * GK_MAX_RES, n_scopes = 0;
};

#define GK_RPT_K 64
#define GK_KERNEL_TILES gk_eval_tiles_64
#define GK_KERNEL_BIG gk_eval_big
#define GK_KERNEL_LINKAGE
#define GK_ROW_FN(r, i, ent, h, pv, heap, acc, on) do { if (on) eval_row_ent(r, i, ent, h, pv, heap, acc); } while (0)
#define GK_FORMULA_FN(pv, acc, flags, rows, heap, bounds) eval_formulas(pv, acc, flags, rows, heap, bounds)
#include "kernel_body.inc"
#define GK_SKIP_BIG
#undef GK_RPT_K
#undef GK_KERNEL_TILES
#undef GK_TILES_BOUNDS
#define GK_RPT_K 128
#define GK_KERNEL_TILES gk_eval_tiles_128
#include "kernel_body.inc"
#undef GK_RPT_K
#undef GK_KERNEL_TILES
#undef GK_TILES_BOUNDS
#define GK_RPT_K 256
#define GK_KERNEL_TILES gk_eval_tiles_256
#include "kernel_body.inc"
#undef GK_RPT_K
#undef GK_KERNEL_TILES
#undef GK_TILES_BOUNDS
#define GK_RPT_K 512
#define GK_KERNEL_TILES gk_eval_tiles_512
#include "kernel_body.inc"
#undef GK_RPT_K
#undef GK_KERNEL_TILES

__device__ __forceinline__ uint32_t gk_row_popcount(const uint64_t* __restrict__ row, uint32_t n_words, uint32_t* partial ) {
  uint32_t c = 0;
  uint32_t i = threadIdx.x;
  for (; i + 3072u < n_words; i += 4096u) {
    const uint64_t a0 = row[i], a1 = row[i + 1024u], a2 = row[i + 2048u], a3 = row[i + 3072u];
    c += (uint32_t)__popcll(a0) + (uint32_t)__popcll(a1) + (uint32_t)__popcll(a2) + (uint32_t)__popcll(a3);
  }
  for (; i < n_words; i += 1024u) c += (uint32_t)__popcll(row[i]);
  for (int off = 32; off > 0; off >>= 1) c += (uint32_t)__shfl_xor((int)c, off);
  if ((threadIdx.x & 63u) == 0u) partial[threadIdx.x >> 6] = c;
  __syncthreads();
  uint32_t sum = 0;
  if (threadIdx.x == 0) for (int k = 0; k < 16; k++) sum += partial[k];
  return sum;
}
__global__ __launch_bounds__(1024) void gk_count_rows(const uint64_t* __restrict__ bitmap, uint32_t stride, uint32_t n_words, uint32_t* __restrict__ counts) {
  __shared__ uint32_t partial[16];
  const uint32_t sum = gk_row_popcount(bitmap + (size_t)blockIdx.x * stride, n_words, partial);
  if (threadIdx.x == 0) counts[blockIdx.x] = sum;
}
__global__ __launch_bounds__(1024) void gk_count_rows_sliced(const uint64_t* __restrict__ bitmap, uint32_t stride, uint32_t n_words, uint32_t* __restrict__ counts) {
  __shared__ uint32_t partial[16];
  const uint32_t per = (n_words + gridDim.y - 1u) / gridDim.y, lo = blockIdx.y * per, hi = lo + per < n_words ? lo + per : n_words;
  if (lo >= hi) return;
  const uint32_t sum = gk_row_popcount(bitmap + (size_t)blockIdx.x * stride + lo, hi - lo, partial);
  if (threadIdx.x == 0 && sum) atomicAdd(&counts[blockIdx.x], sum);
}
__global__ __launch_bounds__(1024) void gk_sum_partials(const uint32_t* __restrict__ partial, uint32_t rows, uint32_t stride, uint32_t nc, uint32_t* __restrict__ counts) {
  __shared__ uint32_t s[64][64];
  __shared__ uint32_t s2[4][64];
  const uint32_t tid = threadIdx.x, lane = tid & 63u, wave = tid >> 6, sub = lane >> 4, q = (lane & 15u) * 4u;
  const uint32_t c0 = blockIdx.x * 64u + q;
  uint32_t a0 = 0, a1 = 0, a2 = 0, a3 = 0;
#pragma unroll 4
  for (uint32_t r = wave * 4u + sub; r < rows; r += 64u) {
    const uint4 v = *reinterpret_cast<const uint4*>(partial + (size_t)r * stride + c0);
    a0 += v.x; a1 += v.y; a2 += v.z; a3 += v.w;
  }
  uint32_t* mine = &s[wave * 4u + sub][q];
  mine[0] = a0; mine[1] = a1; mine[2] = a2; mine[3] = a3;
  __syncthreads();
  if (tid < 256u) {
    uint32_t t = 0;
#pragma unroll
    for (uint32_t k = 0; k < 16u; k++) t += s[wave * 16u + k][lane];
    s2[wave][lane] = t;
  }
  __syncthreads();
  const uint32_t c = blockIdx.x * 64u + lane;
  if (tid < 64u && c < nc) counts[c] = s2[0][lane] + s2[1][lane] + s2[2][lane] + s2[3][lane];
}
static void launch_sum_partials(const uint32_t* d_partial, uint32_t rows, uint32_t stride, uint32_t nc, uint32_t* d_counts, hipStream_t stream) {
  hipLaunchKernelGGL(gk_sum_partials, dim3((nc + 63u) / 64u), dim3(1024), 0, stream, d_partial, rows, stride, nc, d_counts);
  HIP_OK(hipGetLastError());
}
static void launch_count_rows(const uint64_t* d_viol, uint32_t nc, uint32_t n_tiles, uint32_t* d_counts, hipStream_t stream, uint32_t n_words = 0, bool zeroed = false) {
  if (!n_words) n_words = n_tiles;
  static const bool sliced_on = !(getenv("GK_COUNT_SLICED") && atoi(getenv("GK_COUNT_SLICED")) == 0);
  if (zeroed && sliced_on && n_words >= 8192u) {
    const uint32_t slices = n_words >= 65536u ? 16u : 8u;
    hipLaunchKernelGGL(gk_count_rows_sliced, dim3(nc, slices), dim3(1024), 0, stream, d_viol, n_tiles, n_words, d_counts);
  } else hipLaunchKernelGGL(gk_count_rows, dim3(nc), dim3(1024), 0, stream, d_viol, n_tiles, n_words, d_counts);
  HIP_OK(hipGetLastError());
}

__global__ __launch_bounds__(GK_TILE) void gk_topk_rows(const uint64_t* __restrict__ viol, uint32_t n_tiles, const uint32_t* __restrict__ order,
                                                        const uint32_t* __restrict__ grp, uint32_t n, uint32_t k, uint32_t cap,
                                                        uint32_t* __restrict__ out_idx, uint32_t* __restrict__ out_n, uint32_t* __restrict__ out_ovf) {
  const uint32_t c = blockIdx.x, lane = threadIdx.x;
  const uint64_t* row = viol + (size_t)c * n_tiles;
  uint32_t count = 0, grp_k = 0, ovf = 0;
  bool known = false;
  for (uint32_t base = 0; base < n; base += GK_TILE) {
    const uint32_t p = base + lane;
    uint32_t rev = 0, g = 0;
    bool bit = false;
    if (p < n) { rev = order[p]; g = grp[p]; bit = (row[rev / GK_TILE] >> (rev % GK_TILE)) & 1ull; }
    const uint64_t mask = __ballot(bit);
    if (!mask) continue;
    const uint32_t pos = count + (uint32_t)__popcll(mask & ((1ull << lane) - 1ull));
    if (!known && count + (uint32_t)__popcll(mask) >= k) {
      const uint64_t kth = __ballot(bit && pos == k - 1u);
      grp_k = (uint32_t)__shfl((int)g, (int)__builtin_ctzll(kth));
      known = true;
    }
    const bool emit = bit && (pos < k || (known && g == grp_k));
    const bool stop = bit && pos >= k && known && g != grp_k;
    if (emit) { if (pos < cap) out_idx[(size_t)c * cap + pos] = rev; else ovf = 1; }
    count += (uint32_t)__popcll(__ballot(emit));
    if (__ballot(stop)) break;
  }
  ovf = __ballot(ovf != 0) ? 1u : 0u;
  if (lane == 0) { out_n[c] = count < cap ? count : cap; out_ovf[c] = ovf; }
}

__global__ __launch_bounds__(256) void gk_audit_permute(const uint64_t* __restrict__ viol, uint32_t n_tiles, uint32_t nc, const uint32_t* __restrict__ order,
                                                        const uint64_t* __restrict__ shown, uint32_t n, uint32_t pw, uint64_t* __restrict__ perm) {
  const uint32_t lane = threadIdx.x & 63u, word = blockIdx.x * 4u + (threadIdx.x >> 6);
  if (word >= pw) return;
  const uint32_t p = word * GK_TILE + lane;
  uint32_t wi = 0, sh = 0;
  uint64_t keep = 0;
  if (p < n) {
    const uint32_t rev = order[p];
    if (rev < n) { wi = rev / GK_TILE; sh = rev % GK_TILE; keep = (shown[wi] >> sh) & 1ull; }
  }
  for (uint32_t c0 = 0; c0 < nc; c0 += 64u) {
    const uint32_t m = nc - c0 < 64u ? nc - c0 : 64u;
    uint64_t mine = 0;
    uint32_t j = 0;
    for (; j + 4u <= m; j += 4u) {
      const uint64_t* v = viol + (size_t)(c0 + j) * n_tiles + wi;
      const uint64_t x0 = v[0], x1 = v[n_tiles], x2 = v[(size_t)n_tiles * 2u], x3 = v[(size_t)n_tiles * 3u];
      const uint64_t b0 = __ballot(((x0 >> sh) & keep) != 0ull), b1 = __ballot(((x1 >> sh) & keep) != 0ull);
      const uint64_t b2 = __ballot(((x2 >> sh) & keep) != 0ull), b3 = __ballot(((x3 >> sh) & keep) != 0ull);
      if (lane == j) mine = b0;
      if (lane == j + 1u) mine = b1;
      if (lane == j + 2u) mine = b2;
      if (lane == j + 3u) mine = b3;
    }
    for (; j < m; j++) {
      const uint64_t b = __ballot(((viol[(size_t)(c0 + j) * n_tiles + wi] >> sh) & keep) != 0ull);
      if (lane == j) mine = b;
// ... 177 lines not shown
  const void* fns[4] = {reinterpret_cast<const void*>(gk_eval_tiles_64), reinterpret_cast<const void*>(gk_eval_tiles_128),
                        reinterpret_cast<const void*>(gk_eval_tiles_256), reinterpret_cast<const void*>(gk_eval_tiles_512)};
  const uint32_t rpts[4] = {64, 128, 256, 512};
  for (int k = 0; k < 4; k++) {
    e = hipFuncSetAttribute(fns[k], hipFuncAttributeMaxDynamicSharedMemorySize, (int)max_dyn_lds_of(rpts[k]));
    if (e != hipSuccess) return std::string("hipFuncSetAttribute(MaxDynamicSharedMemorySize) failed: ") + hipGetErrorString(e);
  }
  {
    static std::mutex mu;
    static std::vector<int> warmed;
    std::lock_guard<std::mutex> l(mu);
    if (std::find(warmed.begin(), warmed.end(), device) == warmed.end()) {
      warmed.push_back(device);
      void* d = nullptr;
      if (hipMalloc(&d, 512u << 20) == hipSuccess) {
        std::vector<char> h(16u << 20, 1);
        hipStream_t st = stream_acquire(device);
        if (hipMemcpyAsync(d, h.data(), h.size(), hipMemcpyHostToDevice, st) == hipSuccess) (void)hipStreamSynchronize(st);
        stream_release(device, st);
        (void)hipFree(d);
      }
      {
        std::vector<hipStream_t> ss;
        const size_t want = std::min<size_t>(std::max<size_t>(std::thread::hardware_concurrency(), 8), 64) + 8;
        for (size_t i = 0; i < want; i++) ss.push_back(stream_acquire(device));
        for (hipStream_t x : ss) stream_release(device, x);
      }
      (void)hipGetLastError();
    }
  }
  return "";
}

int dev_count() {
  int n = 0;
  if (hipGetDeviceCount(&n) != hipSuccess) return 0;
  return n;
}

template <class T>
static T* upload(const T* src, size_t n) {
  T* d = nullptr;
  size_t bytes = std::max<size_t>(n, 1) * sizeof(T);
  HIP_OK(pool_malloc(&d, bytes));
  if (n) HIP_OK(hipMemcpy(d, src, n * sizeof(T), hipMemcpyHostToDevice));
  return d;
}

__global__ __launch_bounds__(256) void gk_place_rows(Row* __restrict__ dst, const Row* __restrict__ src, uint32_t n, uint32_t heap_base) {
  const uint32_t i = blockIdx.x * 256u + threadIdx.x;
  if (i >= n) return;
  uint4 v = reinterpret_cast<const uint4*>(src)[i];
  if ((v.y & ROW_TYPE_MASK) == T_STRING && !(v.y & ROW_STR_INLINE)) v.z += heap_base;
  reinterpret_cast<uint4*>(dst)[i] = v;
}

struct DevPart {
  Row* rows = nullptr; StrHdr* shdr = nullptr; uint8_t* heap = nullptr;
  size_t n_rows = 0, heap_bytes = 0;
};

DevPart* dev_part_upload(int device, HostTable& part) {
  HIP_OK(hipSetDevice(device));
  std::unique_ptr<DevPart> p(new DevPart());
  p->n_rows = part.rows.size();
  p->heap_bytes = part.heap.size();
  hipStream_t st = stream_acquire(device);
  auto put = [&](void** d, const void* src, size_t bytes) {
    HIP_OK(pool_malloc(d, std::max<size_t>(bytes, 16)));
    if (bytes) HIP_OK(hipMemcpyAsync(*d, src, bytes, hipMemcpyHostToDevice, st));
  };
  put(reinterpret_cast<void**>(&p->rows), part.rows.data(), part.rows.size() * sizeof(Row));
  put(reinterpret_cast<void**>(&p->shdr), part.shdr.data(), part.shdr.size() * sizeof(StrHdr));
  {
    HIP_OK(pool_malloc(reinterpret_cast<void**>(&p->heap), part.heap.size() + 16));
    if (part.heap.size()) HIP_OK(hipMemcpyAsync(p->heap, part.heap.data(), part.heap.size(), hipMemcpyHostToDevice, st));
    HIP_OK(hipMemsetAsync(p->heap + part.heap.size(), 0, 16, st));
  }
  HIP_OK(hipStreamSynchronize(st));
  stream_release(device, st);
  part.rows = PodVec<Row>(); part.shdr = PodVec<StrHdr>(); part.heap = PodVec<uint8_t>();
  return p.release();
}

void dev_part_free(DevPart* p) {
  if (!p) return;
  pool_free(p->rows); pool_free(p->shdr); pool_free(p->heap);
  delete p;
}

DevTable* dev_table_assemble(int device, std::vector<DevPart*>& parts, const HostTable& meta) {
  HIP_OK(hipSetDevice(device));
  DevTable* d = new DevTable();
  d->device = device;
  size_t n_rows = 0, heap_bytes = 0;
  for (DevPart* p : parts) { n_rows += p->n_rows; heap_bytes += p->heap_bytes; }
  d->n_reviews = meta.n_reviews;
  d->rpt = meta.rpt;
  d->n_rows = (uint32_t)n_rows;
  d->n_slots = meta.n_slots();
  d->slot_path = meta.slot_path;
  d->h_tile_idx = std::make_shared<const std::vector<uint32_t>>(meta.tile_idx.data(), meta.tile_idx.data() + meta.tile_idx.size());
  d->tile_idx = upload(meta.tile_idx.data(), meta.tile_idx.size());
  d->rflags = upload(meta.rflags.data(), meta.rflags.size());
  d->stream = stream_acquire(device);
  hipStream_t st = d->stream;
  if (parts.size() == 1 && parts[0]->n_rows) {
    DevPart* p = parts[0];
    d->rows = p->rows; d->shdr = p->shdr; d->heap = p->heap;
    p->rows = nullptr; p->shdr = nullptr; p->heap = nullptr;
    dev_part_free(p);
    parts.clear();
    d->bytes = n_rows * (sizeof(Row) + sizeof(StrHdr)) + meta.tile_idx.size() * 4 + meta.rflags.size() * 4 + heap_bytes + 16;
    return d;
  }
  HIP_OK(pool_malloc(&d->rows, std::max<size_t>(n_rows, 1) * sizeof(Row)));
  HIP_OK(pool_malloc(&d->shdr, std::max<size_t>(n_rows, 1) * sizeof(StrHdr)));
  HIP_OK(pool_malloc(&d->heap, heap_bytes + 16));
  HIP_OK(hipMemsetAsync(d->heap + heap_bytes, 0, 16, st));
  size_t rb = 0, hb = 0;
  for (DevPart* p : parts) {
    if (p->n_rows) {
      hipLaunchKernelGGL(gk_place_rows, dim3((unsigned)((p->n_rows + 255) / 256)), dim3(256), 0, st, d->rows + rb, p->rows, (uint32_t)p->n_rows, (uint32_t)hb);
      HIP_OK(hipGetLastError());
      HIP_OK(hipMemcpyAsync(d->shdr + rb, p->shdr, p->n_rows * sizeof(StrHdr), hipMemcpyDeviceToDevice, st));
    }
    if (p->heap_bytes) HIP_OK(hipMemcpyAsync(d->heap + hb, p->heap, p->heap_bytes, hipMemcpyDeviceToDevice, st));
    rb += p->n_rows; hb += p->heap_bytes;
  }
  HIP_OK(hipStreamSynchronize(st));
  for (DevPart* p : parts) dev_part_free(p);
  parts.clear();
  d->bytes = n_rows * (sizeof(Row) + sizeof(StrHdr)) + meta.tile_idx.size() * 4 + meta.rflags.size() * 4 + heap_bytes + 16;
  return d;
}

void dev_table_free_work(DevTable* t);
DevTable* dev_table_view(DevTable* base) {
  DevTable* v = new DevTable(*base);
  v->work = nullptr;
  v->vidx = std::make_shared<ViolIndex>();
  v->bind_fast = DevTable::Binding();
  v->bind_big = DevTable::Binding();
  v->is_view = true;
  v->stream = stream_acquire(base->device);
  return v;
}

void dev_table_free(DevTable* t) {
  if (!t) return;
  if (t->stream) { stream_release(t->device, t->stream); t->stream = nullptr; }
  else (void)hipStreamSynchronize(0);
  dev_table_free_work(t);
  if (t->is_view) { pool_free(t->bind_fast.d); pool_free(t->bind_big.d); pool_free(t->bind_fast.lists); delete t; return; }
  pool_free(t->rows); pool_free(t->shdr); pool_free(t->tile_idx); pool_free(t->rflags); pool_free(t->heap);
  pool_free(t->bind_fast.d); pool_free(t->bind_big.d); pool_free(t->bind_fast.lists);
  delete t;
}
uint64_t dev_table_bytes(const DevTable* t) { return t->bytes; }

static void upload_variant(const HostPlan& h, DevPlanVariant* v) {
  v->ptab = upload(h.ptab.data(), h.ptab.size());
  v->preds = upload(h.path_preds.data(), h.path_preds.size());
  v->scopes = upload(h.scopes.data(), h.scopes.size());
  v->code = upload(h.code.data(), h.code.size());
  v->cheap = upload(h.cheap.data(), h.cheap.size());
  v->dims = h.dims;
}
static void free_variant(DevPlanVariant* v) {
  pool_free(v->ptab); pool_free(v->preds); pool_free(v->scopes); pool_free(v->code); pool_free(v->cheap);
}

#define RTC_OK(expr)                                                                                  \
  do {                                                                                                \
    hiprtcResult r_ = (expr);                                                                         \
    if (r_ != HIPRTC_SUCCESS) throw std::runtime_error(std::string("hiprtc: ") + hiprtcGetErrorString(r_) + " at " #expr); \
  } while (0)

namespace {
std::atomic<bool> g_exiting{false};
void quiesce_at_exit() { g_exiting.store(true); dev_jit_quiesce(); }
}

static bool helper_compile(const std::string& src, std::vector<char>* code) {
  static const std::string helper = [] {
    Dl_info info;
    if (getenv("GK_JIT_INPROCESS") || !dladdr(reinterpret_cast<const void*>(&helper_compile), &info) || !info.dli_fname) return std::string();
    std::string path = info.dli_fname;
    const size_t slash = path.rfind('/');
    path = (slash == std::string::npos ? std::string(".") : path.substr(0, slash)) + "/gkjitc";
    return access(path.c_str(), X_OK) == 0 ? path : std::string();
  }();
  if (helper.empty()) return false;
  std::string base = cache_dir();
  if (base.empty()) { const char* t = getenv("TMPDIR"); base = (t && *t) ? t : "/tmp"; }
  std::string tmpl = base + "/gk_build_XXXXXX";
  if (!mkdtemp(&tmpl[0])) return false;
  const std::string dir = tmpl;
  const std::string in = dir + "/plan.hip", out = dir + "/plan.co";
  bool ok = false;
  {
    const bool wrote = write_new(in, src.data(), src.size(), nullptr, 0);
    if (wrote) {
      char* argv[] = {const_cast<char*>(helper.c_str()), const_cast<char*>(in.c_str()), const_cast<char*>(out.c_str()), nullptr};
      pid_t pid = 0;
      if (posix_spawn(&pid, helper.c_str(), nullptr, nullptr, argv, environ) == 0) {
        int status = 0;
        while (waitpid(pid, &status, 0) < 0 && errno == EINTR) {}
        if (WIFEXITED(status) && WEXITSTATUS(status) == 0)
          ok = read_whole(out, code) && code->size() > 64 && memcmp(code->data(), "\x7f" "ELF", 4) == 0;
      }
    }
  }
  unlink(in.c_str());
  unlink(out.c_str());
  unlink((out + ".part").c_str());
  rmdir(dir.c_str());
  if (!ok) code->clear();
  return ok;
}

static std::shared_ptr<const std::vector<char>> jit_compile(const std::string& src) {
  static const int rtc_version = [] {
    code_cache_set_compile_slots(std::max<size_t>(1, std::min<size_t>(8, host_cpus() / 2)));
    int major = 0, minor = 0;
    return hiprtcVersion(&major, &minor) == HIPRTC_SUCCESS ? major * 1000 + minor : 0;
  }();
  return code_cache_get(src, rtc_version, [](const std::string& text) {
    std::vector<char> code;
    if (!helper_compile(text, &code)) {
      hiprtcProgram prog;
      RTC_OK(hiprtcCreateProgram(&prog, text.c_str(), "gk_plan.hip", 0, nullptr, nullptr));
      const char* opt_level = getenv("GK_JIT_OPT") ? getenv("GK_JIT_OPT") : "-O3";
      const char* opts[] = {"--offload-arch=gfx950", opt_level, "-std=c++17"};
      hiprtcResult rc = hiprtcCompileProgram(prog, 3, opts);
      if (rc != HIPRTC_SUCCESS) {
        size_t ls = 0;
        hiprtcGetProgramLogSize(prog, &ls);
        std::string log(ls, 0);
        if (ls) hiprtcGetProgramLog(prog, &log[0]);
        hiprtcDestroyProgram(&prog);
        throw std::runtime_error("hiprtc compile failed: " + log.substr(0, 2000));
      }
      size_t cs = 0;
      RTC_OK(hiprtcGetCodeSize(prog, &cs));
      code.resize(cs);
      RTC_OK(hiprtcGetCode(prog, code.data()));
      hiprtcDestroyProgram(&prog);
    }
    { static std::once_flag once; std::call_once(once, [] { std::atexit(quiesce_at_exit); }); }
    return code;
  });
}
void dev_jit_cache_stats(uint64_t* hits, uint64_t* compiles) { code_cache_stats(hits, compiles); }
void dev_jit_cache_drop_memory() { code_cache_drop_memory(); }
const char* dev_jit_cache_dir() { return code_cache_dir(); }

static JitKernel* jit_build(int device, const std::string& src, uint32_t rpt, uint32_t res_k, uint32_t list_cap, uint32_t tot_k) {
  std::unique_ptr<JitKernel> j(new JitKernel());
  j->source = src;
  j->tot_k = tot_k;
  j->source_hash = fnv64(src);
  if (const char* dump = getenv("GK_JIT_DUMP")) { FILE* f = fopen(dump, "w"); if (f) { fwrite(src.data(), 1, src.size(), f); fclose(f); } }
  std::shared_ptr<const std::vector<char>> code = jit_compile(src);
  if (g_exiting.load()) throw std::runtime_error("process is exiting");
  HIP_OK(hipSetDevice(device));
  HIP_OK(hipModuleLoadData(&j->module, code->data()));
  HIP_OK(hipModuleGetFunction(&j->tiles, j->module, "gk_jit_tiles"));
  const size_t want_lds = max_dyn_lds_jit(rpt, res_k, list_cap, tot_k);
  if (hipFuncSetAttribute(reinterpret_cast<const void*>(j->tiles), hipFuncAttributeMaxDynamicSharedMemorySize, (int)want_lds) == hipSuccess)
    j->max_dyn_lds = want_lds;
  else (void)hipGetLastError();
  return j.release();
}

static std::atomic<uint64_t> g_next_plan_id{1};
DevPlan* dev_plan_upload(int device, const HostPlan& fast, const HostPlan& big) {
  HIP_OK(hipSetDevice(device));
  DevPlan* p = new DevPlan();
  p->id = g_next_plan_id++;
  p->device = device;
  p->ptab_fast = fast.ptab;
  p->ptab_big = big.ptab;
  upload_variant(fast, &p->fast);
  upload_variant(big, &p->big);
  p->slots = upload(fast.slots.data(), fast.slots.size());
  p->n_constraints = (uint32_t)fast.slots.size();
  size_t lds = (size_t)fast.dims.acc_words * GK_TILE * 4;
  if (lds > max_dyn_lds_of(64)) {
    dev_plan_free(p);
    throw Unsupported("plan needs " + std::to_string(lds) + " B of LDS per 64 reviews (limit 160 KiB): lower the element capacities");
  }
  p->want_jit = !getenv("GK_NO_JIT");
  if (p->want_jit) {
    p->host_fast = fast;
    std::vector<std::vector<Pred>> classes;
    p->cls = jit_path_classes(fast, &classes);
  }
  p->path_cost.assign(fast.ptab.size(), 0);
  for (size_t i = 0; i < fast.ptab.size(); i++) {
    const uint32_t ent = fast.ptab[i];
    p->path_cost[i] = ent ? pred_list_cost<Pred>(&fast.path_preds[ent >> 8], ent & 0xFF, [](const Pred& q) { return pred_needs_str(q); }) : 0u;
  }
  p->res_k = jit_res_k(fast);
  p->n_scopes = (uint32_t)fast.scopes.size();
  return p;
}

void dev_plan_no_jit(DevPlan* p) { if (p) { p->want_jit = false; p->id = g_next_plan_id++; } }
void dev_plan_free(DevPlan* p) {
  if (!p) return;
  int prev = -1;
  (void)hipGetDevice(&prev);
  if (prev != p->device) (void)hipSetDevice(p->device);
  (void)hipDeviceSynchronize();
  free_variant(&p->fast); free_variant(&p->big);
  pool_free(p->slots);
  for (auto& kv : p->jit) { std::lock_guard<std::mutex> l(kv.second->mu); kv.second->abandoned = true; }
  const int dev = p->device;
  delete p;
  if (prev >= 0 && prev != dev) (void)hipSetDevice(prev);
}

static uint32_t chunk_need(const DevPlan* p, const DevTable* t) {
  if (!t || !t->h_tile_idx) return 0xFFFFFFFFu;
  const uint32_t n_groups = (t->n_reviews + t->rpt - 1) / t->rpt, S = t->n_slots;
  const uint32_t* ix = t->h_tile_idx->data();
  std::vector<uint32_t> slots;
  for (uint32_t s = 0; s < t->slot_path.size(); s++) { const uint32_t path = t->slot_path[s]; if (path < p->ptab_fast.size() && p->ptab_fast[path]) slots.push_back(s); }
  uint32_t most = 0;
  for (uint32_t g = 0; g < n_groups; g++) {
    uint32_t n = 0;
    for (uint32_t s : slots) n += (ix[(size_t)g * (S + 1) + s + 1] - ix[(size_t)g * (S + 1) + s] + GK_TILE - 1) / GK_TILE;
    most = std::max(most, n);
  }
  return most + 1u;
}

namespace {
struct JitThreads {
  std::mutex mu;
  std::list<std::pair<std::thread, std::shared_ptr<std::atomic<bool>>>> running;
  void reap(bool all) {
    std::list<std::pair<std::thread, std::shared_ptr<std::atomic<bool>>>> done;
    {
      std::lock_guard<std::mutex> l(mu);
      for (auto it = running.begin(); it != running.end();) { auto nx = std::next(it); if (all || it->second->load()) done.splice(done.end(), running, it); it = nx; }
    }
    for (auto& t : done) if (t.first.joinable()) t.first.join();
  }
};
JitThreads& jit_threads() {
  static JitThreads* t = new JitThreads();
  static struct Guard { ~Guard() { quiesce_at_exit(); } } guard;
  return *t;
}
}
void dev_jit_quiesce() { jit_threads().reap(true); }

static JitKernel* jit_for(DevPlan* p, uint32_t rpt, uint32_t rpp, const DevTable* t, bool wait, uint32_t list_cap, bool prefetch = false) {
  if (!p->want_jit) return nullptr;
  const bool always_wait = getenv("GK_JIT_SYNC") != nullptr || getenv("GK_JIT_STRICT") != nullptr;
  const bool never_wait = getenv("GK_JIT_ASYNC") != nullptr;
  wait = (wait || always_wait) && !never_wait && !prefetch;
  std::shared_ptr<JitSlot> slot;
  {
    std::lock_guard<std::mutex> l(p->jit_mu);
    const uint32_t key = (rpt * 1024u + rpp) ^ (list_cap << 20);
    auto it = p->jit.find(key);
    if (it != p->jit.end()) slot = it->second;
    else {
      slot = std::make_shared<JitSlot>();
      p->jit.emplace(key, slot);
      std::string src;
      try { src = assemble_jit_source(p->host_fast, rpt, rpp, kPlanHpp, kVmCoreHpp, kKernelBody, list_cap); }
      catch (const std::exception& ex) { slot->state = JitSlot::FAILED; slot->error = ex.what(); }
      if (slot->state == JitSlot::PENDING) {
        const int device = p->device;
        const uint32_t res_k = jit_res_k(p->host_fast), tot_k = jit_tot_k(p->host_fast.dims.n_constraints, (size_t)p->host_fast.dims.acc_words * rpp * 4, rpt, jit_block_of(rpt), res_k, list_cap ? list_cap : list_cap_of(jit_block_of(rpt)));
        auto build = [slot, src, device, rpt, res_k, list_cap, tot_k]() {
          std::unique_ptr<JitKernel> k;
          std::string err;
          try { k.reset(jit_build(device, src, rpt, res_k, list_cap, tot_k)); } catch (const std::exception& ex) { err = ex.what(); }
          std::lock_guard<std::mutex> l(slot->mu);
          slot->k = std::move(k);
          slot->error = err;
          slot->state = slot->k ? JitSlot::READY : JitSlot::FAILED;
          slot->cv.notify_all();
        };
        if (wait) build();
        else {
          jit_threads().reap(false);
          auto flag = std::make_shared<std::atomic<bool>>(false);
          std::thread th([build, flag]() { build(); flag->store(true); });
          std::lock_guard<std::mutex> tl(jit_threads().mu);
          jit_threads().running.emplace_back(std::move(th), flag);
        }
      }
    }
  }
  std::unique_lock<std::mutex> l(slot->mu);
  if (prefetch) return nullptr;
  if (wait) slot->cv.wait(l, [&] { return slot->state != JitSlot::PENDING; });
  if (slot->state == JitSlot::PENDING) return nullptr;
  if (slot->state == JitSlot::FAILED) {
    if (getenv("GK_JIT_STRICT")) throw std::runtime_error("plan specialisation failed: " + slot->error);
    if (!slot->error.empty()) { fprintf(stderr, "[gkgpu] plan specialisation unavailable, using the bytecode kernel: %s\n", slot->error.c_str()); slot->error.clear(); }
    return nullptr;
  }
  return slot->k.get();
}

struct Work {
  uint32_t nc = 0, n_tiles = 0, list_cap = 0;
  bool has_match = false, own_viol = true;
  uint64_t *d_viol = nullptr, *d_err = nullptr, *d_match = nullptr, *d_ovf = nullptr, *d_big = nullptr;
  uint32_t *d_counts = nullptr, *d_list = nullptr, *d_lc = nullptr, *d_done = nullptr;
  bool lc_pinned = false;
  size_t lc_pin_cap = 0;
  unsigned long long* d_prof = nullptr;
  uint32_t* d_partial = nullptr;
  uint32_t partial_cap = 0, partial_rows = 0, partial_stride = 0;
  bool partial_live = false;
  uint8_t* d_all = nullptr;
  size_t slot_bytes = 0;
  uint32_t stride_tiles = 0, shard_nc = 0;
  int shard_rank = 0, shard_world = 1;
  long long* d_totals = nullptr;
  bool overlap = false;
  uint8_t* d_all_buf[2] = {nullptr, nullptr};
  int shard_device = 0;
  hipStream_t comm_stream = nullptr;
  hipEvent_t ev_sweep[2] = {nullptr, nullptr}, ev_xchg[2] = {nullptr, nullptr};
  struct HipShardBackend;
  ShardPipe<HipShardBackend> pipe;
  void shard_teardown() {
    if (comm_stream) { stream_release(shard_device, comm_stream); comm_stream = nullptr; }
    for (int b = 0; b < 2; b++) {
      if (ev_sweep[b]) { hipEventDestroy(ev_sweep[b]); ev_sweep[b] = nullptr; }
      if (ev_xchg[b]) { hipEventDestroy(ev_xchg[b]); ev_xchg[b] = nullptr; }
    }
    pool_free(d_all_buf[0]); pool_free(d_all_buf[1]);
    d_all_buf[0] = d_all_buf[1] = nullptr; d_all = nullptr; overlap = false; pipe.overlap = false; pipe.reset();
  }
  uint32_t* last_lc = nullptr;
  unsigned long long shard_not_eval = ~0ull;
  int graph_state = 0;
  uint64_t graph_key = 0;
  hipGraphExec_t graph_exec = nullptr;
  void drop_graph() { if (graph_exec) hipGraphExecDestroy(graph_exec); graph_exec = nullptr; graph_state = 0; graph_key = 0; }
  static constexpr uint32_t LC_SLOTS = 64;
  static constexpr uint32_t LC_WORDS = 2, LC_BYTES = LC_WORDS * 4;
  std::vector<uint32_t*> lc_more;
  std::vector<size_t> lc_more_cap;
  size_t lc_used = 0;
  uint32_t* lc_slot(size_t i) const { return (i < LC_SLOTS ? d_lc : lc_more[i / LC_SLOTS - 1]) + LC_WORDS * (i % LC_SLOTS); }
  template <class Fill> void lc_zero_used(Fill fill) {
    if (lc_used) fill(d_lc, std::min<size_t>(lc_used, LC_SLOTS) * LC_BYTES);
    for (size_t k = 0; k < lc_more.size() && (k + 1) * LC_SLOTS < lc_used; k++) fill(lc_more[k], std::min<size_t>(lc_used - (k + 1) * LC_SLOTS, LC_SLOTS) * LC_BYTES);
    lc_used = 0;
  }
  void lc_release_more() {
    for (size_t k = 0; k < lc_more.size(); k++) { if (lc_pinned) pinned_release(reinterpret_cast<uint8_t*>(lc_more[k]), lc_more_cap[k]); else pool_free(lc_more[k]); }
    lc_more.clear(); lc_more_cap.clear(); lc_used = 0;
  }
  struct Launch {
    uint64_t plan = 0;
    bool want_match = false;
    hipFunction_t fn = nullptr;
    uint32_t grid = 0, block = 0, lds = 0, tot_k = 0;
    uint64_t kernel_hash = 0;
    PlanView pv{};
    const Row* rows = nullptr; const StrHdr* shdr = nullptr; const ChunkDesc* lists = nullptr; const uint32_t* rflags = nullptr; const uint8_t* heap = nullptr;
    const ConstraintSlot* slots = nullptr;
    uint32_t cg = 0, nn = 0, nt = 0, dd = 0, rp = 0;
    OutPtrs out{};
  } cached;
  bool timed = false;
  size_t timed_from = 0;
  void open_bracket(size_t launch_no, bool want, hipStream_t stream) {
    if (launch_no == 0) timed = false;
    if (want && !timed) { HIP_OK(hipEventRecord(ev_first, stream)); timed = true; timed_from = launch_no; }
  }
  hipEvent_t ev_first = nullptr, ev_last = nullptr;
  std::vector<std::pair<hipEvent_t, hipEvent_t>> evs;
  size_t pending = 0;
  bool lc_dirty = false;
  bool per_launch = false;
  uint32_t lds_bytes = 0;
  hipEvent_t ev_x0 = nullptr, ev_x1 = nullptr;
  float exchange_ms = 0;
  uint64_t kernel_hash = 0;
  uint8_t* h_pin = nullptr;
  size_t pin_cap = 0;
  uint8_t* pinned(size_t bytes) {
    if (bytes > pin_cap) {
      pinned_release(h_pin, pin_cap);
      h_pin = pinned_acquire(bytes, &pin_cap);
    }
    return h_pin;
  }
  void release() {
    drop_graph();
    cached.plan = 0;
    lc_release_more();
    pool_free(own_viol ? d_viol : nullptr); pool_free(d_err); pool_free(d_match); pool_free(d_ovf); pool_free(d_big); pool_free(d_list); if (lc_pinned) pinned_release(reinterpret_cast<uint8_t*>(d_lc), lc_pin_cap); else pool_free(d_lc); lc_pinned = false; pool_free(d_done); pool_free(d_partial);
    d_viol = d_err = d_match = d_ovf = d_big = nullptr; d_counts = d_list = d_lc = d_done = d_partial = nullptr; partial_cap = partial_rows = 0; partial_live = false; last_lc = nullptr;
  }
  ~Work() { drop_graph(); release(); pinned_release(h_pin, pin_cap); shard_teardown(); pool_free(d_totals); for (auto& e : evs) { hipEventDestroy(e.first); hipEventDestroy(e.second); } if (ev_first) hipEventDestroy(ev_first); if (ev_last) hipEventDestroy(ev_last); if (ev_x0) hipEventDestroy(ev_x0); if (ev_x1) hipEventDestroy(ev_x1); }
};

static bool host_atomics_work(int device) {
  static std::mutex mu;
  static std::map<int, bool> known;
  std::lock_guard<std::mutex> l(mu);
  auto it = known.find(device);
  if (it == known.end()) {
    int v = 0;
    if (hipDeviceGetAttribute(&v, hipDeviceAttributeHostNativeAtomicSupported, device) != hipSuccess) { (void)hipGetLastError(); v = 0; }
    it = known.emplace(device, v != 0).first;
  }
  return it->second;
}

static Work* get_work(const DevTable* t, uint32_t nc, uint32_t n_tiles, const EvalOptions& opt) {
  DevTable* mt = const_cast<DevTable*>(t);
  if (!mt->work) mt->work = new Work();
  Work* w = mt->work;
  bool want_match = opt.want_match;
  if (opt.shard && (!w->d_all || w->shard_nc != nc || w->stride_tiles != n_tiles)) throw std::runtime_error("sharded evaluation without dev_shard_setup for this plan");
  if (w->nc != nc || w->n_tiles != n_tiles || w->list_cap < opt.list_capacity || (want_match && !w->has_match) || w->own_viol == opt.shard) {
    if (w->d_err) (void)hipStreamSynchronize(t->stream);
    w->release();
    const size_t bm = std::max<size_t>((size_t)nc * n_tiles, 1);
    if (opt.shard) {
      w->d_viol = reinterpret_cast<uint64_t*>(w->d_all + (size_t)w->shard_rank * w->slot_bytes);
      w->own_viol = false;
    } else {
      HIP_OK(pool_malloc(&w->d_viol, bm * 8 + std::max<size_t>(nc, 1) * 4));
      w->own_viol = true;
    }
    w->d_counts = reinterpret_cast<uint32_t*>(w->d_viol + bm);
    HIP_OK(pool_malloc(&w->d_err, bm * 8));
    if (want_match) HIP_OK(pool_malloc(&w->d_match, bm * 8));
    HIP_OK(pool_malloc(&w->d_ovf, std::max<size_t>(n_tiles, 1) * 8));
    HIP_OK(pool_malloc(&w->d_big, std::max<size_t>(n_tiles, 1) * 8));
    static const bool lc_host = !(getenv("GK_LC_PINNED") && atoi(getenv("GK_LC_PINNED")) == 0);
    if (lc_host && !opt.shard && opt.list_capacity == 0 && host_atomics_work(t->device)) {
      w->d_lc = reinterpret_cast<uint32_t*>(pinned_acquire((Work::LC_SLOTS + 1) * Work::LC_BYTES, &w->lc_pin_cap));
      w->lc_pinned = w->d_lc != nullptr;
    }
    if (!w->lc_pinned) HIP_OK(pool_malloc(&w->d_lc, (Work::LC_SLOTS + 1) * Work::LC_BYTES));
    HIP_OK(hipMemsetAsync(w->d_lc, 0, (Work::LC_SLOTS + 1) * Work::LC_BYTES, t->stream));
    HIP_OK(pool_malloc(&w->d_done, 4));
    HIP_OK(hipMemsetAsync(w->d_done, 0, 4, t->stream));
    if (opt.list_capacity) HIP_OK(pool_malloc(&w->d_list, (size_t)opt.list_capacity * 8));
    w->nc = nc; w->n_tiles = n_tiles; w->list_cap = opt.list_capacity; w->has_match = want_match;
  }
  return w;
}

void dev_table_free_work(DevTable* t) { delete t->work; t->work = nullptr; }

static void bind_paths(DevTable* t, DevTable::Binding* b, uint64_t plan_id, const std::vector<uint32_t>& entries) {
  if (b->plan_id == plan_id) return;
  std::vector<Bind> v;
  for (uint32_t s = 0; s < t->slot_path.size(); s++) {
    uint32_t path = t->slot_path[s];
    if (path < entries.size() && entries[path] != 0) v.push_back(Bind{s, entries[path]});
  }
  if (b->d) (void)hipStreamSynchronize(t->stream);
  pool_free(b->d);
  b->d = upload(v.data(), v.size());
  b->n = (uint32_t)v.size();
  b->plan_id = plan_id;
}

static void bind_chunks(DevTable* t, DevTable::Binding* b, uint64_t key, const std::vector<uint32_t>& entries, const std::vector<uint32_t>& cost,
                        bool generic, int block, uint32_t list_cap) {
  if (b->plan_id == key && b->lists) return;
  if (!t->h_tile_idx) throw std::runtime_error("table without a host slot index");
  std::vector<BoundPath> bound;
  for (uint32_t s = 0; s < t->slot_path.size(); s++) {
    const uint32_t path = t->slot_path[s];
    if (path >= entries.size() || entries[path] == 0) continue;
    if (generic && entries[path] > GK_DESC_ENT_MASK) throw Unsupported("plan too large for the chunk descriptors (predicate table beyond 2^17 entries)");
    bound.push_back(BoundPath{s, entries[path], path < cost.size() ? cost[path] : 1u});
  }
  const uint32_t n_groups = (t->n_reviews + t->rpt - 1) / t->rpt;
  ChunkLists cl = build_chunk_lists(t->h_tile_idx->data(), n_groups, t->n_slots, std::move(bound), list_cap, (uint32_t)(block / GK_TILE));
  if (b->lists) (void)hipStreamSynchronize(t->stream);
  pool_free(b->lists);
  b->lists = upload(cl.d.data(), cl.d.size());
  b->capg = cl.capg;
  b->list_bytes = (uint64_t)cl.d.size() * sizeof(ChunkDesc);
  b->plan_id = key;
}

static uint32_t grid_for(int device, uint32_t n_groups, size_t lds_per_group, int block) {
  static std::mutex mu;
  static std::map<int, int> cus;
  int n_cu;
  {
    std::lock_guard<std::mutex> l(mu);
    auto it = cus.find(device);
    if (it == cus.end()) {
      int v = 0;
      if (hipDeviceGetAttribute(&v, hipDeviceAttributeMultiprocessorCount, device) != hipSuccess || v <= 0) v = 256;
      it = cus.emplace(device, v).first;
    }
    n_cu = it->second;
  }
  const uint32_t all = (n_groups + 7u) / 8u * 8u;
  static const int persist = getenv("GK_PERSIST") ? atoi(getenv("GK_PERSIST")) : -1;
  if (persist == 0) return all;
  size_t per_cu = std::max<size_t>(1, std::min<size_t>(GK_LDS_PER_CU / std::max<size_t>(lds_per_group, 1), (size_t)2048 / (size_t)block));
  if (persist > 0) per_cu = (size_t)persist;
  const uint32_t fit = (uint32_t)((size_t)n_cu * per_cu + 7u) / 8u * 8u;
  return std::min(all, fit);
}

static void jit_geometry(const DevPlan* p, const DevTable* t, uint32_t* rpp_out, uint32_t* lcap_out) {
  const uint32_t rpt = t->rpt;
  uint32_t rpp = rpt;
  const size_t dyn_cap = p->want_jit ? max_dyn_lds_jit(rpt, p->res_k, 0, jit_tot_k(p->n_constraints)) : max_dyn_lds_of(rpt);
  while (rpp > (uint32_t)GK_TILE && (size_t)p->fast.dims.acc_words * rpp * 4 > dyn_cap) rpp /= 2;
  if (const char* f = getenv("GK_FORCE_RPP")) rpp = std::min<uint32_t>(rpt, std::max<uint32_t>(GK_TILE, (uint32_t)atoi(f)));
  uint32_t jit_lcap = list_cap_of(jit_block_of(rpt));
  if (p->want_jit && rpt >= 256) {
    DevTable* mt = const_cast<DevTable*>(t);
    if (mt->chunk_need_plan != p->id) { mt->chunk_need = chunk_need(p, t); mt->chunk_need_plan = p->id; }
    jit_lcap = jit_list_cap(jit_block_of(rpt), mt->chunk_need);
  }
  *rpp_out = rpp; *lcap_out = jit_lcap;
}

void dev_jit_prefetch(const DevPlan* p, const DevTable* t) {
  if (!p || !t || !p->want_jit || t->n_reviews == 0 || p->n_constraints == 0) return;
  uint32_t rpp = 0, lcap = 0;
  jit_geometry(p, t, &rpp, &lcap);
  try { (void)jit_for(const_cast<DevPlan*>(p), t->rpt, rpp, t, false, lcap, true); } catch (const std::exception&) {}
}

static uint32_t* lc_for_launch(Work* w, const EvalOptions& opt, hipStream_t stream) {
  if (opt.detached) return w->d_lc + Work::LC_WORDS * Work::LC_SLOTS;
  if (w->lc_dirty && w->pending == 0) {
    w->lc_zero_used([&](uint32_t* at, size_t bytes) { HIP_OK(hipMemsetAsync(at, 0, bytes, stream)); });
    w->lc_dirty = false;
  }
  const size_t i = w->pending;
  while (i / Work::LC_SLOTS > w->lc_more.size()) {
    uint32_t* blk = nullptr;
    size_t cap = 0;
    if (w->lc_pinned) {
      blk = reinterpret_cast<uint32_t*>(pinned_acquire(Work::LC_SLOTS * Work::LC_BYTES, &cap));
      if (!blk) throw std::runtime_error("no pinned memory for the launch counters");
      memset(blk, 0, Work::LC_SLOTS * Work::LC_BYTES);
    } else {
      HIP_OK(pool_malloc(&blk, Work::LC_SLOTS * Work::LC_BYTES));
      HIP_OK(hipMemsetAsync(blk, 0, Work::LC_SLOTS * Work::LC_BYTES, stream));
    }
    w->lc_more.push_back(blk); w->lc_more_cap.push_back(cap);
  }
  return w->lc_slot(i);
}

void dev_eval_launch(const DevPlan* p, const DevTable* t, const EvalOptions& opt) {
  const uint32_t n = t->n_reviews, nc = p->n_constraints;
  const uint32_t n_tiles = opt.shard && t->work ? t->work->stride_tiles : (n + GK_TILE - 1) / GK_TILE;
  if (n == 0 || nc == 0) return;
  if (Work* cw = t->work; cw && cw->cached.plan == p->id && cw->cached.want_match == opt.want_match && !opt.shard && !opt.detached && !opt.time_each &&
                          opt.list_capacity == 0 && !opt.bytecode) {
    Work::Launch& c = cw->cached;
    hipStream_t stream = t->stream;
    c.out.list_count = cw->last_lc = lc_for_launch(cw, opt, stream);
    cw->open_bracket(cw->pending++, opt.timed, stream);
    cw->per_launch = false;
    cw->partial_rows = c.grid; cw->partial_stride = c.tot_k; cw->partial_live = true;
    cw->lds_bytes = c.lds; cw->kernel_hash = c.kernel_hash;
    void* args[] = {&c.pv, &c.rows, &c.shdr, &c.lists, &c.cg, &c.rflags, &c.heap, &c.nn, &c.nt, &c.slots, &c.out, &c.dd, &c.rp};
    HIP_OK(hipModuleLaunchKernel(c.fn, c.grid, 1, 1, c.block, 1, 1, c.lds, stream, args, nullptr));
    return;
  }
  Work* w = get_work(t, nc, n_tiles, opt);
  w->cached.plan = 0;
  hipStream_t stream = t->stream;
  if (opt.shard && !opt.detached && w->overlap && w->comm_stream) { HIP_OK(hipStreamSynchronize(w->comm_stream)); w->pipe.pending[0] = w->pipe.pending[1] = false; }
  uint32_t* lc = lc_for_launch(w, opt, stream);
  w->last_lc = lc;
  static const bool want_prof = getenv("GK_KERNEL_PROF") != nullptr;
  if (want_prof && !w->d_prof) { HIP_OK(pool_malloc(&w->d_prof, ((size_t)n / GK_RPT_MIN + 8) * 64)); HIP_OK(hipMemsetAsync(w->d_prof, 0, ((size_t)n / GK_RPT_MIN + 8) * 64, stream)); }
  OutPtrs out{w->d_viol, w->d_err, opt.want_match ? w->d_match : nullptr, w->d_ovf, w->d_big, w->d_counts, w->d_list, lc,
              opt.list_capacity, w->d_prof, nullptr};
  const bool per_launch = !opt.detached && opt.time_each;
  if (!w->ev_first) { HIP_OK(hipEventCreate(&w->ev_first)); HIP_OK(hipEventCreate(&w->ev_last)); }
  if (per_launch && w->pending == w->evs.size()) {
    hipEvent_t a, b;
    HIP_OK(hipEventCreate(&a)); HIP_OK(hipEventCreate(&b));
    w->evs.emplace_back(a, b);
  }
  const size_t launch_no = opt.detached ? ~(size_t)0 : w->pending++;
  const uint32_t rpt = t->rpt;
  int block = gk_block_of((int)rpt);
  const uint32_t n_groups = (n + rpt - 1) / rpt;
  static const uint32_t dbg_phase = getenv("GK_DBG_PHASE") ? (uint32_t)atoi(getenv("GK_DBG_PHASE")) : 0u;
  static const uint32_t stagger = getenv("GK_STAGGER") ? (uint32_t)atoi(getenv("GK_STAGGER")) & 0xFFFu : (uint32_t)GK_STAGGER_DEFAULT;
  constexpr uint32_t stagger_mode = 0u;
  uint32_t rpp = rpt, jit_lcap = 0;
  DevTable* mt = const_cast<DevTable*>(t);
  JitKernel* jit = nullptr;
  if (opt.bytecode) {
  } else if (mt->launch_plan == p->id && mt->launch_jit) {
    rpp = mt->launch_rpp; jit_lcap = mt->launch_lcap; jit = static_cast<JitKernel*>(mt->launch_jit);
  } else {
    jit_geometry(p, t, &rpp, &jit_lcap);
    const bool jit_wait = opt.jit_wait;
    jit = jit_for(const_cast<DevPlan*>(p), rpt, rpp, t, jit_wait, jit_lcap);
    if (jit && (size_t)p->fast.dims.acc_words * rpp * 4 > jit->max_dyn_lds) {
      while (rpp > (uint32_t)GK_TILE && (size_t)p->fast.dims.acc_words * rpp * 4 > jit->max_dyn_lds) rpp /= 2;
      jit = jit_for(const_cast<DevPlan*>(p), rpt, rpp, t, jit_wait, jit_lcap);
    }
    mt->launch_plan = p->id; mt->launch_rpp = rpp; mt->launch_lcap = jit_lcap; mt->launch_jit = jit;
  }
  if (jit) block = jit_block_of(rpt);
  else if ((size_t)p->fast.dims.acc_words * rpp * 4 > max_dyn_lds_of(rpt)) {
    while (rpp > (uint32_t)GK_TILE && (size_t)p->fast.dims.acc_words * rpp * 4 > max_dyn_lds_of(rpt)) rpp /= 2;
  }
  bind_chunks(mt, &mt->bind_fast, (p->id * 2 + (jit ? 1 : 0)) * 2048 + (uint64_t)block, jit ? p->cls : p->ptab_fast, p->path_cost, !jit, block,
              jit ? jit_lcap : list_cap_of(block));
  const size_t lds = (size_t)p->fast.dims.acc_words * rpp * 4;
  const uint32_t dbg = dbg_phase | (n_groups >= 1024u ? (stagger << 8) | (stagger_mode << 20) : 0u);
  uint32_t grid = grid_for(t->device, n_groups, lds + static_lds_of(rpt, block, jit ? p->res_k : 0, jit ? jit_lcap : 0, jit ? jit->tot_k : 0), block);
  const uint32_t grid_full = grid;
  if (opt.shard && opt.detached && w->overlap && grid < (n_groups + 7u) / 8u * 8u) {
    static const uint32_t reserve = getenv("GK_SHARD_RESERVE_WGS") ? (uint32_t)atoi(getenv("GK_SHARD_RESERVE_WGS")) / 8u * 8u : 32u;
    if (grid > reserve + 64u) grid -= reserve;
  }
  const bool fused_totals = jit && jit->tot_k >= nc && !opt.shard;
  if (jit && jit->tot_k) {
    if ((size_t)w->partial_cap < (size_t)grid_full * jit->tot_k) {
      if (w->d_partial) { w->drop_graph(); HIP_OK(hipStreamSynchronize(stream)); pool_free(w->d_partial); w->d_partial = nullptr; }
      w->partial_cap = ((grid_full + 255u) / 256u * 256u) * jit->tot_k;
      HIP_OK(pool_malloc(&w->d_partial, (size_t)w->partial_cap * 4));
    }
    out.partial = w->d_partial;
    if (!opt.detached) { w->partial_rows = grid; w->partial_stride = jit->tot_k; }
  }
  if (!opt.detached) w->partial_live = fused_totals;
  w->lds_bytes = (uint32_t)lds;
  w->kernel_hash = jit ? jit->source_hash : 0;
  if (per_launch) { HIP_OK(hipEventRecord(w->evs[launch_no].first, stream)); if (launch_no == 0) w->timed = false; }
  else if (!opt.detached) w->open_bracket(launch_no, opt.timed, stream);
  if (!opt.detached) w->per_launch = per_launch;
  if (jit) {
    PlanView pv = p->fast.view();
    const Row* rows = t->rows; const StrHdr* shdr = t->shdr; const uint32_t* rflags = t->rflags;
    const uint8_t* heap = t->heap;
    const ChunkDesc* lists = t->bind_fast.lists;
    uint32_t nn = n, nt = n_tiles, dd = dbg, cg = t->bind_fast.capg, rp = rpp;
    const ConstraintSlot* slots = p->slots;
    void* args[] = {&pv, &rows, &shdr, &lists, &cg, &rflags, &heap, &nn, &nt, &slots, &out, &dd, &rp};
    HIP_OK(hipModuleLaunchKernel(jit->tiles, grid, 1, 1, block, 1, 1, (unsigned)lds, stream, args, nullptr));
    if (fused_totals && !opt.detached && !per_launch && opt.list_capacity == 0 && !w->d_prof) {
      Work::Launch& c = w->cached;
      c.want_match = opt.want_match; c.fn = jit->tiles; c.grid = grid; c.block = (uint32_t)block; c.lds = (uint32_t)lds;
      c.tot_k = jit->tot_k; c.kernel_hash = jit->source_hash; c.pv = pv; c.rows = rows; c.shdr = shdr; c.lists = lists; c.rflags = rflags; c.heap = heap;
      c.slots = slots; c.cg = cg; c.nn = nn; c.nt = nt; c.dd = dd; c.rp = rp; c.out = out;
      c.plan = p->id;
    }
  } else {
    auto fn = rpt == 64 ? gk_eval_tiles_64 : rpt == 128 ? gk_eval_tiles_128 : rpt == 256 ? gk_eval_tiles_256 : gk_eval_tiles_512;
    hipLaunchKernelGGL(fn, dim3(grid), dim3(block), lds, stream, p->fast.view(), t->rows, t->shdr, t->bind_fast.lists, t->bind_fast.capg,
                       t->rflags, t->heap, n, n_tiles, p->slots, out, dbg, rpp);
    HIP_OK(hipGetLastError());
  }
  if (per_launch) HIP_OK(hipEventRecord(w->evs[launch_no].second, stream));
  if (!opt.shard && !opt.kernel_only && !fused_totals) launch_count_rows(w->d_viol, nc, n_tiles, w->d_counts, stream, 0, true);
}

void dev_eval_finish(const DevPlan* p, const DevTable* t, const EvalOptions& opt, EvalOut* o) {
  const uint32_t n = t->n_reviews, nc = p->n_constraints;
  const uint32_t n_tiles = opt.shard && t->work ? t->work->stride_tiles : (n + GK_TILE - 1) / GK_TILE;
  o->n_reviews = n; o->n_constraints = nc; o->n_tiles = n_tiles;
  o->kernel_ms = o->fast_kernel_ms = 0;
  o->n_overflow = 0; o->list_total = 0; o->n_launches = 0;
  if (n == 0 || nc == 0) {
    o->viol.assign((size_t)nc * n_tiles, 0); o->err = o->viol; o->match = o->viol; o->too_big.assign(n_tiles, 0); o->counts.assign(nc, 0); o->list.clear();
    return;
  }
  Work* w = t->work;
  if (!w || w->pending == 0) throw std::runtime_error("dev_eval_finish without a pending launch");
  hipStream_t stream = t->stream;
  const size_t bm_words = (size_t)nc * n_tiles;
  uint32_t lc[2] = {0, 0};
  if (!w->per_launch && w->timed) HIP_OK(hipEventRecord(w->ev_last, stream));
  uint32_t* d_lc_last = w->lc_slot(w->pending - 1);
  if (w->partial_live && !opt.shard) launch_sum_partials(w->d_partial, w->partial_rows, w->partial_stride, nc, w->d_counts, stream);
  if (w->lc_pinned) {
    HIP_OK(hipStreamSynchronize(stream));
    memcpy(lc, d_lc_last, 8);
  } else if (uint8_t* pin0 = w->pinned(64)) {
    HIP_OK(hipMemcpyAsync(pin0, d_lc_last, 8, hipMemcpyDeviceToHost, stream));
    HIP_OK(hipStreamSynchronize(stream));
    memcpy(lc, pin0, 8);
  } else {
    HIP_OK(hipMemcpyAsync(lc, d_lc_last, 8, hipMemcpyDeviceToHost, stream));
    HIP_OK(hipStreamSynchronize(stream));
  }
  float total = 0;
  if (w->per_launch) { for (size_t i = 0; i < w->pending; i++) { float ms = 0; HIP_OK(hipEventElapsedTime(&ms, w->evs[i].first, w->evs[i].second)); total += ms; } }
  else if (w->timed) HIP_OK(hipEventElapsedTime(&total, w->ev_first, w->ev_last));
  o->n_launches = (uint32_t)w->pending;
  w->lc_used = std::max(w->lc_used, w->pending);
  o->lds_bytes = w->lds_bytes;
  o->kernel_hash = w->kernel_hash;
  o->specialised = w->kernel_hash != 0;
  o->list_bytes = t->bind_fast.list_bytes;
  o->fast_kernel_ms = total / (float)(w->per_launch || !w->timed ? w->pending : w->pending - w->timed_from);
  o->kernel_ms = o->fast_kernel_ms;
  w->pending = 0;
  o->n_overflow = lc[1];
  OutPtrs out{w->d_viol, w->d_err, opt.want_match ? w->d_match : nullptr, w->d_ovf, w->d_big, w->d_counts, w->d_list, d_lc_last,
              opt.list_capacity, nullptr, nullptr};
  if (w->d_prof) {
    const size_t ng = (n + t->rpt - 1) / t->rpt;
    std::vector<unsigned long long> pr(ng * 8);
    HIP_OK(hipMemcpy(pr.data(), w->d_prof, pr.size() * 8, hipMemcpyDeviceToHost));
    if (const char* path = getenv("GK_KERNEL_PROF"); path && path[0] == '/') {
      if (FILE* f = fopen(path, "wb")) { fwrite(pr.data(), 8, pr.size(), f); fclose(f); }
    }
    double d[7] = {0}, waited = 0;
    for (size_t g = 0; g < ng; g++) { for (int k = 0; k < 6; k++) d[k] += (double)(pr[g * 8 + k + 1] - pr[g * 8 + k]); waited += (double)pr[g * 8 + 7]; }
    if (waited > 0) fprintf(stderr, "[gkgpu prof] wave 0 waited %.0f clocks per group for its rows in phase 1 (GK_PROF_WAIT)\n", waited / ng);
    fprintf(stderr, "[gkgpu prof] rpt %u groups %zu: mean clocks  zero+barrier %.0f | phase1 %.0f | barrier %.0f | bounds %.0f | formulas %.0f | outputs %.0f | group total %.0f\n",
            t->rpt, ng, d[0] / ng, d[1] / ng, d[2] / ng, d[3] / ng, d[4] / ng, d[5] / ng, (d[0] + d[1] + d[2] + d[3] + d[4] + d[5]) / ng);
  }
  if (lc[1]) {
    std::vector<uint64_t> ovf(n_tiles);
    HIP_OK(hipMemcpy(ovf.data(), w->d_ovf, (size_t)n_tiles * 8, hipMemcpyDeviceToHost));
    std::vector<uint32_t> ids;
    for (uint32_t tl = 0; tl < n_tiles; tl++) for (uint64_t m = ovf[tl]; m; m &= m - 1) ids.push_back(tl * GK_TILE + (uint32_t)__builtin_ctzll(m));
    uint32_t* d_ids = upload(ids.data(), ids.size());
    uint32_t* d_scratch;
    HIP_OK(pool_malloc(&d_scratch, ids.size() * (size_t)p->big.dims.acc_words * 4));
    hipEvent_t e1, e2;
    HIP_OK(hipEventCreate(&e1)); HIP_OK(hipEventCreate(&e2));
    HIP_OK(hipEventRecord(e1, stream));
    DevTable* mt = const_cast<DevTable*>(t);
    bind_paths(mt, &mt->bind_big, p->id, p->ptab_big);
    hipLaunchKernelGGL(gk_eval_big, dim3((uint32_t)ids.size()), dim3(GK_TILE), 0, stream, p->big.view(), t->rows, t->shdr, t->tile_idx, t->n_slots,
                       t->bind_big.d, t->bind_big.n, t->rflags, t->heap, d_ids,
                       (uint32_t)ids.size(), n_tiles, p->slots, d_scratch, out, t->rpt);
    HIP_OK(hipGetLastError());
    HIP_OK(hipEventRecord(e2, stream));
    launch_count_rows(w->d_viol, nc, n_tiles, w->d_counts, stream);
    HIP_OK(hipStreamSynchronize(stream));
    float ms = 0;
    HIP_OK(hipEventElapsedTime(&ms, e1, e2));
    o->kernel_ms += ms;
    hipEventDestroy(e1); hipEventDestroy(e2);
    pool_free(d_ids); pool_free(d_scratch);
    if (w->lc_pinned) memcpy(lc, d_lc_last, 8); else HIP_OK(hipMemcpy(lc, d_lc_last, 8, hipMemcpyDeviceToHost));
  }
  if (w->lc_pinned) {
    w->lc_zero_used([](uint32_t* at, size_t bytes) { memset(at, 0, bytes); });
  } else w->lc_dirty = true;
  o->list_total = lc[0];
  o->d_viol = w->d_viol; o->d_err = w->d_err; o->d_counts = w->d_counts;
  if (opt.download) {
    o->viol.resize(bm_words); o->err.resize(bm_words); o->counts.resize(nc); o->too_big.resize(n_tiles);
    if (opt.want_match) o->match.resize(bm_words);
    const uint32_t k = opt.list_capacity ? std::min(lc[0], opt.list_capacity) : 0u;
    o->list.resize((size_t)k * 2);
    struct Piece { void* dst; const void* src; size_t bytes; };
    const Piece pieces[] = {{o->viol.data(), w->d_viol, bm_words * 8}, {o->err.data(), w->d_err, bm_words * 8}, {o->counts.data(), w->d_counts, (size_t)nc * 4},
                            {o->too_big.data(), w->d_big, (size_t)n_tiles * 8}, {opt.want_match ? o->match.data() : nullptr, w->d_match, opt.want_match ? bm_words * 8 : 0},
                            {o->list.data(), w->d_list, (size_t)k * 8}};
    size_t total = 0;
    for (const Piece& pc : pieces) total += (pc.bytes + 15) & ~(size_t)15;
    uint8_t* pin = w->pinned(total);
    if (pin) {
      size_t at = 0;
      for (const Piece& pc : pieces) { if (pc.bytes) HIP_OK(hipMemcpyAsync(pin + at, pc.src, pc.bytes, hipMemcpyDeviceToHost, stream)); at += (pc.bytes + 15) & ~(size_t)15; }
      HIP_OK(hipStreamSynchronize(stream));
      at = 0;
      for (const Piece& pc : pieces) { if (pc.bytes) memcpy(pc.dst, pin + at, pc.bytes); at += (pc.bytes + 15) & ~(size_t)15; }
    } else {
      HIP_OK(hipStreamSynchronize(stream));
      for (const Piece& pc : pieces) if (pc.bytes) HIP_OK(hipMemcpy(pc.dst, pc.src, pc.bytes, hipMemcpyDeviceToHost));
    }
  }
}

struct Id128 { char b[128]; };
namespace {
struct Rccl {
  void* h = nullptr;
  int (*GetUniqueId)(void*) = nullptr;
  int (*CommInitRank)(void**, int, Id128, int) = nullptr;
  int (*CommDestroy)(void*) = nullptr;
  int (*AllGather)(const void*, void*, size_t, int, void*, hipStream_t) = nullptr;
  const char* (*GetErrorString)(int) = nullptr;
  int (*CommCount)(void*, int*) = nullptr;
  int (*CommUserRank)(void*, int*) = nullptr;
};
}
static Rccl* rccl_load(std::string* err) {
  static Rccl r;
  static std::mutex mu;
  std::lock_guard<std::mutex> l(mu);
  if (r.h) return &r;
  for (const char* name : {"librccl.so.1", "librccl.so", "/opt/rocm/lib/librccl.so.1"}) { r.h = dlopen(name, RTLD_NOW | RTLD_GLOBAL); if (r.h) break; }
  if (!r.h) { *err = std::string("RCCL not available: ") + dlerror(); return nullptr; }
  r.GetUniqueId = reinterpret_cast<int (*)(void*)>(dlsym(r.h, "ncclGetUniqueId"));
  r.CommInitRank = reinterpret_cast<int (*)(void**, int, Id128, int)>(dlsym(r.h, "ncclCommInitRank"));
  r.CommDestroy = reinterpret_cast<int (*)(void*)>(dlsym(r.h, "ncclCommDestroy"));
  r.AllGather = reinterpret_cast<int (*)(const void*, void*, size_t, int, void*, hipStream_t)>(dlsym(r.h, "ncclAllGather"));
  r.GetErrorString = reinterpret_cast<const char* (*)(int)>(dlsym(r.h, "ncclGetErrorString"));
  r.CommCount = reinterpret_cast<int (*)(void*, int*)>(dlsym(r.h, "ncclCommCount"));
  r.CommUserRank = reinterpret_cast<int (*)(void*, int*)>(dlsym(r.h, "ncclCommUserRank"));
  if (!r.GetUniqueId || !r.CommInitRank || !r.CommDestroy || !r.AllGather) { *err = "RCCL symbols missing"; dlclose(r.h); r.h = nullptr; return nullptr; }
  return &r;
}
constexpr int kNcclUint8 = 1;

struct DevComm { Rccl* lib = nullptr; void* comm = nullptr; int rank = 0, world = 1, device = 0; };
#define NCCL_OK(c, expr)                                                                                                   \
  do {                                                                                                                     \
    int r_ = (expr);                                                                                                       \
    if (r_ != 0) throw std::runtime_error(std::string("RCCL error: ") + ((c)->lib->GetErrorString ? (c)->lib->GetErrorString(r_) : "?") + " at " #expr); \
  } while (0)

bool dev_comm_unique_id(char id[128], std::string* err) {
  Rccl* r = rccl_load(err);
  if (!r) return false;
  if (r->GetUniqueId(id) != 0) { *err = "ncclGetUniqueId failed"; return false; }
  return true;
}
DevComm* dev_comm_init(int device, const char id[128], int rank, int world, std::string* err) {
  Rccl* r = rccl_load(err);
  if (!r) return nullptr;
  if (hipSetDevice(device) != hipSuccess) { *err = "hipSetDevice failed"; return nullptr; }
  std::unique_ptr<DevComm> c(new DevComm());
  c->lib = r; c->rank = rank; c->world = world; c->device = device;
  Id128 uid;
  memcpy(uid.b, id, 128);
  int rc = r->CommInitRank(&c->comm, world, uid, rank);
  if (rc != 0) { *err = std::string("ncclCommInitRank failed: ") + (r->GetErrorString ? r->GetErrorString(rc) : "?"); return nullptr; }
  return c.release();
}
void dev_comm_free(DevComm* c) { if (c) { if (c->comm) c->lib->CommDestroy(c->comm); delete c; } }
int dev_comm_rank(const DevComm* c) { return c->rank; }
int dev_comm_world(const DevComm* c) { return c->world; }
bool dev_comm_query(const DevComm* c, int* rank, int* world, std::string* err) {
  if (!c->lib->CommCount || !c->lib->CommUserRank) { *err = "this RCCL has no ncclCommCount / ncclCommUserRank"; return false; }
  int rc = c->lib->CommCount(c->comm, world);
  if (rc == 0) rc = c->lib->CommUserRank(c->comm, rank);
  if (rc != 0) { *err = std::string("RCCL error: ") + (c->lib->GetErrorString ? c->lib->GetErrorString(rc) : "?"); return false; }
  return true;
}

constexpr uint32_t GK_TAIL_EXTRA = 3;
__global__ void gk_slot_totals(const uint8_t* __restrict__ all, unsigned long long slot_bytes, unsigned long long tail_off, uint32_t world, uint32_t nc,
                               long long* __restrict__ totals) {
  const uint32_t i = blockIdx.x * 256u + threadIdx.x;
  if (i >= 2u * nc + GK_TAIL_EXTRA) return;
  long long s = 0;
  for (uint32_t r = 0; r < world; r++) {
    const uint8_t* tail = all + (size_t)r * slot_bytes + tail_off;
    s += i < 2u * nc ? (long long)reinterpret_cast<const uint32_t*>(tail)[i]
// ... 435 lines not shown
```

### gatekeeper_amd/driver.py

```python
from __future__ import annotations

import copy
import ctypes as C
import dataclasses
import json
import re

import numpy as np

from . import _lib as L

TARGET_NAME = "admission.k8s.gatekeeper.sh"
WEBHOOK_EP = "validation.gatekeeper.sh"
AUDIT_EP = "audit.gatekeeper.sh"
GATOR_EP = "gator.gatekeeper.sh"
ALL_EP = "*"

_SOURCES = {"": L.GK_SRC_EMPTY, "Original": L.GK_SRC_ORIGINAL, "Generated": L.GK_SRC_GENERATED, "All": L.GK_SRC_ALL}


class EngineError(Exception):
    def __init__(self, code, msg):
        super().__init__(msg)
        self.code = code
# ... 324 lines not shown
    def totals(self):
        out = C.POINTER(L.gk_totals_out)()
        self.engine._check(self.engine.lib.gk_table_totals(self.engine.handle, self.handle, C.byref(out)))
        o = out.contents
        res = {int(o.constraint_ids[i]): (int(o.results[i]), int(o.pairs[i])) for i in range(o.n_constraints)}
        self.rendered_pairs = int(o.rendered_pairs)
        self.engine.lib.gk_totals_free(out)
        return res

    def free(self):
        if self.handle:
            self.engine.lib.gk_table_free(self.handle)
            self.handle = None

    def __del__(self):
        try:
            self.free()
        except Exception:
            pass


class Engine:

    def __init__(self, device=0, elem_cap=None, hostemu=None, referential=True, gather_stats=False, tracing=False, disabled_builtins=None):
        self.lib = L.load(hostemu)
        self.hostemu = bool(hostemu)
        opts = L.gk_opts()
        opts.device = device
        if elem_cap:
            for i, v in enumerate(elem_cap):
                opts.elem_cap[i] = v
        opts.flags = (0 if referential else L.GK_OPT_NO_REFERENTIAL) | (L.GK_OPT_GATHER_STATS if gather_stats else 0) | (L.GK_OPT_TRACE if tracing else 0)
        if disabled_builtins is not None:
            names = [n.encode() for n in disabled_builtins]
            self._disabled = (C.c_char_p * max(len(names), 1))(*names)
            opts.disabled_builtins, opts.n_disabled_builtins = self._disabled, len(names)
        h = C.c_void_p()
        self._check(self.lib.gk_engine_create(C.byref(opts), C.byref(h)))
        self.handle = h

    def _check(self, rc):
        if rc != L.GK_OK:
            msg = self.lib.gk_last_error().decode()
            if rc == L.GK_ERR_UNSUPPORTED:
                raise UnsupportedError(rc, msg)
            raise EngineError(rc, msg)

    def close(self):
        if getattr(self, "handle", None):
            self.lib.gk_engine_destroy(self.handle)
            self.handle = None

    def __del__(self):
        try:
            self.close()
        except Exception:
            pass

    def add_template(self, kind, rego, libs=()):
        arr = (C.c_char_p * max(1, len(libs)))(*[l.encode() for l in libs])
        self._check(self.lib.gk_template_add(self.handle, kind.encode(), rego.encode(), arr, len(libs)))

    def remove_template(self, kind):
        self._check(self.lib.gk_template_remove(self.handle, kind.encode()))

    def add_constraint(self, constraint):
        body = json.dumps(constraint).encode()
        cid = C.c_uint32()
        self._check(self.lib.gk_constraint_add(self.handle, body, len(body), C.byref(cid)))
        return cid.value

    def remove_constraint(self, kind, name):
        self._check(self.lib.gk_constraint_remove(self.handle, kind.encode(), name.encode()))

    def put_data(self, path, obj):
        arr = (C.c_char_p * len(path))(*[p.encode() for p in path])
        body = json.dumps(obj).encode()
        self._check(self.lib.gk_data_put(self.handle, arr, len(path), body, len(body)))

    def remove_data(self, path):
        arr = (C.c_char_p * len(path))(*[p.encode() for p in path])
        self._check(self.lib.gk_data_remove(self.handle, arr, len(path)))

    @staticmethod
    def _process_flag(process):
        if process is None:
            return 0
        if process not in ("audit", "webhook"):
            raise ValueError("tables are built for process 'audit' or 'webhook', not %r" % (process,))
        return L.GK_TABLE_PROCESS_AUDIT if process == "audit" else L.GK_TABLE_PROCESS_WEBHOOK

    def set_excluder(self, match_entries):
        js = json.dumps(match_entries or []).encode()
        self._check(self.lib.gk_excluder_replace(self.handle, js, len(js)))

    def is_excluded(self, process, review):
        arr = (L.gk_review_in * 1)()
        self._fill(arr[0], review)
        out = C.c_int32(0)
        self._check(self.lib.gk_excluder_excluded(self.handle, process.encode(), arr, C.byref(out)))
        return bool(out.value)

    @staticmethod
    def _fill(a, r):
        a.kind, a.source = r.kind, r.source
        a.json, a.json_len = r.json, len(r.json)
        if r.namespace is not None:
            a.namespace_json, a.namespace_len = r.namespace, len(r.namespace)
        if r.ns_object is not None:
            a.ns_object_json, a.ns_object_len = r.ns_object, len(r.ns_object)
        a.operation = r.operation

    def create_table(self, reviews, keep_docs=True, resident=False, process=None, pre_matched=False):
        n = len(reviews)
        arr = (L.gk_review_in * max(1, n))()
        keep = []
        for i, r in enumerate(reviews):
            a = arr[i]
            a.kind, a.source = r.kind, r.source
            a.json, a.json_len = r.json, len(r.json)
            keep.append(r)
            if r.namespace is not None:
                a.namespace_json, a.namespace_len = r.namespace, len(r.namespace)
            if r.ns_object is not None:
                a.ns_object_json, a.ns_object_len = r.ns_object, len(r.ns_object)
            a.operation = r.operation
        st = (C.c_int32 * max(1, n))()
        h = C.c_void_p()
        flags = (L.GK_TABLE_KEEP_DOCS if keep_docs else 0) | (L.GK_TABLE_RESIDENT if resident else 0) | self._process_flag(process) | (
            L.GK_TABLE_PRE_MATCHED if pre_matched else 0)
        self._check(self.lib.gk_table_create(self.handle, arr, n, flags, st, C.byref(h)))
        return Table(self, h, list(st)[:n], n)

    def create_table_spool(self, api_cache_dir, kind, folders, keep_docs=False, resident=True, process=None, keep_text=False):
        info, h = C.POINTER(L.gk_spool_info)(), C.c_void_p()
        flags = (L.GK_TABLE_KEEP_DOCS if keep_docs else 0) | (L.GK_TABLE_RESIDENT if resident else 0) | self._process_flag(process) | (L.GK_TABLE_KEEP_TEXT if keep_text else 0)
        self._check(self.lib.gk_table_create_spool(self.handle, str(api_cache_dir).encode(), kind.encode(), int(folders), flags, C.byref(info), C.byref(h)))
        o = info.contents
        n = int(o.n_reviews)
        d = {"n_files": int(o.n_files), "n_reviews": n, "n_unreadable": int(o.n_unreadable), "n_namespace_missing": int(o.n_namespace_missing),
             "n_folders_missing": int(o.n_folders_missing),
             "bytes": int(o.bytes), "names": [o.names[i].decode() for i in range(n)], "n_rejected": int(o.n_rejected), "n_excluded": int(o.n_excluded)}
        statuses = [int(o.statuses[i]) for i in range(n)]
        self.lib.gk_spool_info_free(info)
        return Table(self, h, statuses, n), d

    def create_table_native(self, reviews_ptr, n, keep_docs=False, resident=False, process=None, keep_text=False, pruned=False):
        st = (C.c_int32 * max(1, n))()
        h = C.c_void_p()
        flags = ((L.GK_TABLE_KEEP_DOCS if keep_docs else 0) | (L.GK_TABLE_RESIDENT if resident else 0) | self._process_flag(process) | (L.GK_TABLE_KEEP_TEXT if keep_text else 0)
                 | (L.GK_TABLE_PRUNED if pruned else 0))
        self._check(self.lib.gk_table_create(self.handle, reviews_ptr, n, flags, st, C.byref(h)))
        return Table(self, h, st, n)

    def dump(self):
        p = C.c_void_p()
        self._check(self.lib.gk_dump(self.handle, C.byref(p)))
        s = C.string_at(p).decode()
        self.lib.gk_free(p)
        return s


class Result:

    def __init__(self, msg, constraint, details=None, enforcement_action="deny", scoped_actions=None, target=TARGET_NAME):
        self.target = target
        self.msg = msg
        self.constraint = constraint
        self.metadata = {"details": details if details is not None else {}}
        self.enforcement_action = enforcement_action
        self.scoped_enforcement_actions = scoped_actions

    def key(self):
        c = self.constraint
        return (c.get("kind"), (c.get("metadata") or {}).get("name"), self.msg, json.dumps(self.metadata, sort_keys=True),
                self.enforcement_action, tuple(self.scoped_enforcement_actions or ()))

    def __repr__(self):
        return "Result(%r, %s/%s, %s)" % (self.msg, self.constraint.get("kind"),
                                          (self.constraint.get("metadata") or {}).get("name"), self.enforcement_action)


class QueryResponse:

    def __init__(self, results, stats_entries=None, trace=None):
        self.results = results
        self.stats_entries = stats_entries or []
        self.trace = trace


class ClientError(Exception):
    pass


def template_source(ct):
    spec = ct.get("spec")
    if not isinstance(spec, dict):
        raise ClientError("invalid ConstraintTemplate: spec must be an object")
    names = spec
    for step in ("crd", "spec", "names"):
        names = names.get(step) if isinstance(names, dict) else None
    if not isinstance(names, dict) or "kind" not in names:
        raise ClientError("invalid ConstraintTemplate: missing spec.crd.spec.names.kind")
    targets = spec.get("targets") or []
    if len(targets) != 1:
        raise ClientError("invalid ConstraintTemplate: expected exactly 1 target, got %d" % len(targets))
    target = targets[0]
    rego_entries = [e.get("source") or {} for e in (target.get("code") or []) if e.get("engine") == "Rego"]
    source = rego_entries[-1] if rego_entries and rego_entries[-1].get("rego") is not None else target
    return names["kind"], target.get("target"), source.get("rego"), list(source.get("libs") or [])


@dataclasses.dataclass
class VerifyEntry:
    kind: str
    constraint_kind: str
    constraint_name: str
    constraint_id: int
    review: int
    specialised_bit: int
    path: tuple = None


@dataclasses.dataclass
class VerifyResult:
    ok: bool
    n_reviews: int
    n_plan_groups: int
    specialised_groups: int
    kernel_text_hash: int
    constraint_ids: list
    diff_viol: dict
    diff_err: dict
    diff_match: dict
    diff_too_big: int
    diff_total: int
    entries_total: int
    entries: list
    quarantined_groups: int
    specialised_ms: float
    bytecode_ms: float
    diff_ms: float


class Driver:

    RUN_TIME_NS = "templateRunTimeNS"
    CONSTRAINT_COUNT = "constraintCount"

    def __init__(self, device=0, gather_stats=False, hostemu=None, elem_cap=None, tracing=False, referential=True, disabled_builtins=None, print_enabled=False):
        self.engine = Engine(device, elem_cap=elem_cap, hostemu=hostemu, referential=referential, gather_stats=gather_stats, tracing=tracing,
                             disabled_builtins=disabled_builtins)
        self.gather_stats = gather_stats
        self.tracing = tracing
        self.print_enabled = print_enabled
        self._ids = {}

    def Name(self):
        return "Rego"

    def AddTemplate(self, ct):
        kind, _, rego, libs = template_source(ct)
        if not rego:
            raise ClientError("template %s has no Rego source" % kind)
        self.engine.add_template(kind, rego, libs)

    def RemoveTemplate(self, ct):
        kind, _, _, _ = template_source(ct)
        try:
            self.engine.remove_template(kind)
        except EngineError as e:
            if e.code != L.GK_ERR_NOT_FOUND:
                raise
        for k in [k for k in self._ids if k[0].lower() == kind.lower()]:
            del self._ids[k]

    def AddConstraint(self, constraint):
        cid = self.engine.add_constraint(constraint)
        self._ids[(constraint.get("kind", ""), (constraint.get("metadata") or {}).get("name", ""))] = cid
        return cid

    def RemoveConstraint(self, constraint):
        key = (constraint.get("kind", ""), (constraint.get("metadata") or {}).get("name", ""))
        if key in self._ids:
            self.engine.remove_constraint(*key)
            del self._ids[key]

    def AddData(self, target, path, data):
        self.engine.put_data(list(path), data)

    def RemoveData(self, target, path):
        self.engine.remove_data(list(path))

    def constraint_id(self, constraint):
        key = (constraint.get("kind", ""), (constraint.get("metadata") or {}).get("name", ""))
        if key not in self._ids:
            raise EngineError(L.GK_ERR_NOT_FOUND, "unknown constraint template validator: %s" % constraint.get("kind"))
        return self._ids[key]

    def Query(self, target, constraints, review, namespace=None, stats_enabled=False, tracing=False):
        return self._query(target, constraints, review, namespace, stats_enabled, tracing, True)

    def QueryMatching(self, target, constraints, review, namespace=None, stats_enabled=False, tracing=False):
        return self._query(target, constraints, review, namespace, stats_enabled, tracing, False)

    def _query(self, target, constraints, review, namespace, stats_enabled, tracing, pre_matched):
# ... 572 lines not shown
```

### include/gkgpu.h

```cpp
#ifndef GKGPU_H
#define GKGPU_H
#include <stddef.h>
#include <stdint.h>

#ifdef __cplusplus
extern "C" {
#endif

typedef struct gk_engine gk_engine;
typedef struct gk_table gk_table;

typedef enum {
  GK_OK = 0,
  GK_ERR_INVALID = -1,
  GK_ERR_REGO = -2,
  GK_ERR_UNSUPPORTED = -3,
  GK_ERR_NOT_FOUND = -4,
  GK_ERR_DEVICE = -5,
  GK_ERR_REVIEW = -6,
  GK_ERR_INTERNAL = -7,
  GK_ERR_LIMIT = -8
} gk_status;

#define GK_OPT_NO_REFERENTIAL 1u
// ... 116 lines not shown
int gk_render_error(gk_engine* e, gk_table* t, uint32_t constraint_id, uint32_t review, char** json_out);
void gk_free(void* p);

typedef struct {
  uint32_t n_constraints, stride;
  const uint32_t* constraint_ids;
  const uint32_t* counts;
  const uint32_t* reviews;
  const uint32_t* overflow;
} gk_topk_out;
int gk_table_topk(gk_engine* e, gk_table* t, uint32_t k, gk_topk_out** out);
void gk_topk_free(gk_topk_out* o);

typedef struct {
  uint32_t n_constraints;
  const uint32_t* constraint_ids;
  const uint64_t* results;
  const uint64_t* pairs;
  uint64_t rendered_pairs;
} gk_totals_out;
int gk_table_totals(gk_engine* e, gk_table* t, gk_totals_out** out);
void gk_totals_free(gk_totals_out* o);

#define GK_COMM_ID_BYTES 128
int gk_comm_unique_id(char id[GK_COMM_ID_BYTES]);
int gk_comm_init(gk_engine* e, const char id[GK_COMM_ID_BYTES], int rank, int world);
void gk_comm_destroy(gk_engine* e);
int gk_comm_info(gk_engine* e, int32_t* rank, int32_t* world);
typedef struct {
  uint32_t world, rank, n_constraints, stride_tiles;
  uint64_t slot_bytes;
  const uint32_t* constraint_ids;
  const uint32_t* shard_reviews;
  const int64_t* totals;
  const uint64_t* gathered;
  const void* d_gathered;
  float kernel_ms, fast_kernel_ms;
  uint32_t n_overflow;
  const int64_t* err_totals;
  int64_t beyond_limits;
  int64_t not_evaluated;
  float exchange_ms;
  uint32_t exchange_overlapped;
  uint64_t exchange_bytes_inbound;
} gk_shard_out;
#define GK_SHARD_DOWNLOAD 1u
#define GK_SHARD_ENQUEUE 2u
#define GK_SHARD_COLLECT 4u
int gk_table_sweep_sharded(gk_engine* e, gk_table* t, uint32_t flags, gk_shard_out** out);
void gk_shard_free(gk_shard_out* o);

typedef struct {
  uint64_t n_objects;
  uint32_t n_constraints, n_chunks;
  const uint32_t* constraint_ids;
  const uint64_t* pairs;
  const uint64_t* results;
  uint64_t flattened;
  uint64_t beyond_limits;
  double sync_s, eval_s;
} gk_sweep_out;
#define GK_SWEEP_RESULT_TOTALS 1u
int gk_resident_sweep(gk_engine* e, uint32_t flags, gk_sweep_out** out);
void gk_sweep_free(gk_sweep_out* o);
typedef struct {
  uint64_t n_objects;
  uint32_t n_constraints, stride, n_chunks;
  const uint32_t* constraint_ids;
  const uint64_t* pairs;
  const uint64_t* results;
  const uint32_t* counts;
  const uint32_t* objects;
  const uint32_t* overflow;
  uint32_t n_paths;
  const char* const* paths;
  uint64_t beyond_limits;
  const uint64_t* err_pairs;
} gk_audit_out;
int gk_resident_audit(gk_engine* e, uint32_t k, uint32_t flags, gk_audit_out** out);
void gk_audit_free(gk_audit_out* o);
#define GK_VIOLATIONS_RENDER 1u
typedef struct {
  uint64_t n_objects;
  uint32_t n_constraints, n_chunks, mask_words;
  const uint32_t* constraint_ids;
  uint64_t total_objects;
  uint32_t n_entries;
  const char* const* paths;
  const uint64_t* viol;
  const uint64_t* err;
  const char* const* results_json;
  uint64_t beyond_limits;
  uint64_t next_cursor;
} gk_violations_out;
int gk_resident_violations(gk_engine* e, uint64_t cursor, uint32_t max_objects, uint32_t flags, gk_violations_out** out);
void gk_violations_free(gk_violations_out* o);
int gk_resident_review(gk_engine* e, const char* const* path, size_t npath, char** results_json);
int gk_resident_review_ex(gk_engine* e, const char* const* path, size_t npath, const uint32_t* constraint_ids, size_t n_constraints,
                          uint32_t flags, char** results_json);

#define GK_VERIFY_WANT_MATCH 1u
#define GK_VERIFY_QUARANTINE 2u
#define GK_VERIFY_VIOL 0u
#define GK_VERIFY_ERR 1u
#define GK_VERIFY_MATCH 2u
#define GK_VERIFY_TOO_BIG 3u
typedef struct { uint32_t kind, row, review, specialised_bit; } gk_verify_entry;
typedef struct {
  uint32_t n_reviews, n_constraints, n_plan_groups;
  const uint32_t* constraint_ids;
  uint32_t specialised_groups;
  uint64_t kernel_text_hash;
  const uint64_t *diff_viol, *diff_err, *diff_match;
  uint64_t diff_too_big, diff_total;
  uint32_t n_entries; uint64_t entries_total;
  const gk_verify_entry* entries;
  uint32_t quarantined_groups;
  float specialised_ms, bytecode_ms, diff_ms;
} gk_verify_out;
int gk_table_verify(gk_engine* e, gk_table* t, uint32_t flags, uint32_t max_entries, gk_verify_out** out);
void gk_verify_free(gk_verify_out* o);
int gk_resident_verify(gk_engine* e, uint32_t flags, uint32_t max_entries, gk_verify_out** out, char*** entry_paths);

typedef struct {
  uint32_t max_batch;
  uint32_t window_us;
  uint32_t workers;
  uint32_t reserved;
} gk_batch_opts;
typedef struct {
  uint32_t batch_size;
  uint32_t reserved;
  double queue_us;
  double device_us;
  double total_us;
} gk_query_stats;
int gk_batcher_start(gk_engine* e, const gk_batch_opts* opts);
void gk_batcher_stop(gk_engine* e);
int gk_query(gk_engine* e, const gk_review_in* review, char** results_json, gk_query_stats* stats);
#define GK_QUERY_TRACE 1u
int gk_query_ex(gk_engine* e, const gk_review_in* review, uint32_t flags, char** results_json, char** trace_out, gk_query_stats* stats);
#define GK_QUERY_PRE_MATCHED 2u
int gk_query_ex2(gk_engine* e, const gk_review_in* review, const uint32_t* constraint_ids, size_t n_constraints, uint32_t flags,
                 char** results_json, char** trace_out, gk_query_stats* stats);

void gk_jit_quiesce(void);
void gk_jit_cache_stats(uint64_t* cache_hits, uint64_t* compiles);
const char* gk_jit_cache_dir(void);
void gk_jit_cache_drop_memory(void);

int gk_debug_set(const char* key, int64_t value);

int gk_dump(gk_engine* e, char** text_out);

#ifdef __cplusplus
}
#endif
#endif
```

Before: 1387 billion evals/s.

## Hoist review-only predicate classes into precomputed per-review words

Adds an analysis that finds predicate classes depending only on review-global bits, precomputes those words per review in a bind-time kernel, and ORs them into LDS inside the JIT kernel. The hoisted paths are dropped from the per-tile chunk lists, so the main kernel reads fewer rows and headers. In exchange it adds a bind kernel, an extra device buffer, per-review loads and LDS atomics, and a second embedded kernel body built by text anchors. It is on by default for large tables with rpt>=128.

```diff
diff --git a/gatekeeper_amd/_lib.py b/gatekeeper_amd/_lib.py
--- a/gatekeeper_amd/_lib.py
+++ b/gatekeeper_amd/_lib.py
@@ -28,7 +28,7 @@
 EXPORTS = [
     "gk_engine_create", "gk_engine_destroy", "gk_last_error", "gk_version", "gk_template_add", "gk_template_remove",
     "gk_constraint_add", "gk_constraint_remove", "gk_data_put", "gk_data_remove", "gk_excluder_replace", "gk_excluder_excluded", "gk_table_create", "gk_table_free",
-    "gk_table_eval", "gk_eval_free", "gk_render", "gk_render_error", "gk_free", "gk_dump", "gk_table_topk", "gk_topk_free",
+    "gk_table_eval", "gk_eval_free", "gk_render", "gk_render_error", "gk_free", "gk_dump", "gk_table_review_words", "gk_table_topk", "gk_topk_free",
     "gk_table_totals", "gk_totals_free", "gk_table_get_stats", "gk_batcher_start", "gk_batcher_stop", "gk_query", "gk_query_ex", "gk_query_ex2",
     "gk_resident_sweep", "gk_sweep_free", "gk_resident_review", "gk_resident_review_ex", "gk_resident_audit", "gk_audit_free",
     "gk_resident_violations", "gk_violations_free", "gk_table_verify", "gk_verify_free", "gk_resident_verify",
@@ -226,6 +226,7 @@
     lib.gk_free.argtypes = [vp]
     lib.gk_free.restype = None
     lib.gk_dump.argtypes = [vp, C.POINTER(vp)]
+    lib.gk_table_review_words.argtypes = [vp, vp, C.POINTER(vp)]
     lib.gk_table_topk.argtypes = [vp, vp, u32, C.POINTER(C.POINTER(gk_topk_out))]
     lib.gk_topk_free.argtypes = [C.POINTER(gk_topk_out)]
     lib.gk_topk_free.restype = None
diff --git a/gatekeeper_amd/csrc/device.hpp b/gatekeeper_amd/csrc/device.hpp
--- a/gatekeeper_amd/csrc/device.hpp
+++ b/gatekeeper_amd/csrc/device.hpp
@@ -40,6 +40,8 @@
   uint32_t n_launches = 0;
   uint32_t lds_bytes = 0;
   uint64_t list_bytes = 0;
+  uint64_t rw_bytes = 0;
+  uint64_t rw_rows = 0, rw_hdr_rows = 0;
   uint64_t kernel_hash = 0;
   bool specialised = false;
   const void *d_viol = nullptr, *d_err = nullptr, *d_counts = nullptr;
diff --git a/gatekeeper_amd/csrc/embed_sources.py b/gatekeeper_amd/csrc/embed_sources.py
--- a/gatekeeper_amd/csrc/embed_sources.py
+++ b/gatekeeper_amd/csrc/embed_sources.py
@@ -14,6 +14,48 @@
     return "".join(out)
 
 
-with open(sys.argv[1], "w", encoding="utf-8") as f:
-    for var, name in (("kPlanHpp", "plan.hpp"), ("kVmCoreHpp", "vm_core.hpp"), ("kKernelBody", "kernel_body.inc")):
-        f.write("static const char %s[] = R\"GKSRC(%s)GKSRC\";\n" % (var, text(name)))
+RW_HOOKS = [
+    ("uint32_t dbg, uint32_t rpp", "inline", ", const uint32_t* __restrict__ rwords, uint32_t rw_stride"),
+    ("  auto entry_of = [&](const Item& it, uint32_t tid_now) -> ChunkDesc {", "before",
+     "  uint32_t rwv[GK_RW_K];\n"
+     "  auto rw_of = [&](const Item& it) {\n"
+     "    const uint32_t t0 = tile_of(it) * GK_RPT_K, nr = min((uint32_t)GK_RPT_K, n_reviews - t0), g = it.pass * RPP + rl2;\n"
+     "    const bool mine = it.ok && wave_on && part == 0u && g < nr;\n"
+     "#pragma unroll\n"
+     "    for (uint32_t k = 0; k < (uint32_t)GK_RW_K; k++) { const uint32_t* __restrict__ wk = rwords + (size_t)k * rw_stride; rwv[k] = mine ? wk[t0 + g] : 0u; }   // (a scalar base per word, one vector offset for all)\n"
+     "  };\n"),
+    ("    const uint2* wl = s_work[buf];", "before", "    rw_of(it);\n"),
+    ("    GK_PROF(2);", "before",
+     "    if (wave_on && part == 0u) {\n"
+     "#pragma unroll\n"
+     "      for (uint32_t k = 0; k < (uint32_t)GK_RW_K; k++)\n"
+     "        (void)__hip_atomic_fetch_or(&lds[GK_RW_WORD(k) * RPP + rl2], rwv[k], __ATOMIC_RELAXED, __HIP_MEMORY_SCOPE_WORKGROUP);\n"
+     "    }\n"),
+]
+
+
+def with_hooks(body, hooks):
+    for anchor, where, ins in hooks:
+        if where == "inline":
+            if body.count(anchor) != 1:
+                sys.exit("embed_sources.py: anchor %r matches %d times in kernel_body.inc" % (anchor, body.count(anchor)))
+            body = body.replace(anchor, anchor + ins)
+            continue
+        lines = body.split("\n")
+        at = [i for i, line in enumerate(lines) if anchor in line]
+        if len(at) != 1:
+            sys.exit("embed_sources.py: anchor %r matches %d lines of kernel_body.inc" % (anchor, len(at)))
+        new = ins.rstrip("\n").split("\n")
+        i = at[0]
+        lines[i:i] = new
+        body = "\n".join(lines)
+    return body
+
+
+if sys.argv[1] == "--rw":
+    with open(sys.argv[2], "w", encoding="utf-8") as f:
+        f.write("static const char kKernelBodyRw[] = R\"GKSRC(%s)GKSRC\";\n" % with_hooks(text("kernel_body.inc"), RW_HOOKS))
+else:
+    with open(sys.argv[1], "w", encoding="utf-8") as f:
+        for var, name in (("kPlanHpp", "plan.hpp"), ("kVmCoreHpp", "vm_core.hpp"), ("kKernelBody", "kernel_body.inc")):
+            f.write("static const char %s[] = R\"GKSRC(%s)GKSRC\";\n" % (var, text(name)))
diff --git a/gatekeeper_amd/csrc/engine.cpp b/gatekeeper_amd/csrc/engine.cpp
--- a/gatekeeper_amd/csrc/engine.cpp
+++ b/gatekeeper_amd/csrc/engine.cpp
@@ -24,12 +24,14 @@
 #include "lower.hpp"
 #include "pe.hpp"
 #include "regex.hpp"
+#include "review_words.hpp"
 #include "verify_merge.hpp"
 #include "viol_stream.hpp"
 
 using namespace gk;
 
 static std::atomic<int64_t> g_debug_verify_flip{-1};
+static std::atomic<bool> g_debug_keep_slot_index{false};
 static std::atomic<int> g_debug_group_max{0};
 namespace {
 
@@ -1339,7 +1341,7 @@
     t->stats.upload_s = std::chrono::duration<double>(t_up - t_indexed).count();
     t->stats.flatten_s = std::chrono::duration<double>(t_indexed - t_begin).count();
     for (size_t i = 0; i < n; i++) t->stats.json_bytes += reviews[i].json_len;
-    t->host.tile_idx.clear(); t->host.tile_idx.shrink_to_fit();
+    if (!g_debug_keep_slot_index.load()) { t->host.tile_idx.clear(); t->host.tile_idx.shrink_to_fit(); }
     *out = t.release();
     return GK_OK;
   } catch (const std::exception& ex) { return fail(GK_ERR_DEVICE, ex.what()); }
@@ -1520,6 +1522,7 @@
         o.n_overflow += og.n_overflow;
         o.kernel_ms += og.kernel_ms; o.fast_kernel_ms += og.fast_kernel_ms;
         o.list_bytes += og.list_bytes;
+        o.rw_bytes += og.rw_bytes; o.rw_rows += og.rw_rows; o.rw_hdr_rows += og.rw_hdr_rows;
         o.kernel_hash = o.kernel_hash * 1099511628211ull ^ og.kernel_hash;
         o.n_constraints += og.n_constraints;
         o.d_viol = o.d_err = o.d_counts = nullptr;
@@ -1572,9 +1575,12 @@
       account(e->fast);
       for (auto& g : e->extra) account(g->fast);
     }
+    const uint64_t rw_rows = std::min<uint64_t>(h->out.rw_rows, rows_read), rw_hdrs = std::min<uint64_t>(h->out.rw_hdr_rows, hdrs_read);
+    rows_read -= rw_rows; hdrs_read -= rw_hdrs;
+    if (e->extra.empty()) { rows_once -= std::min(rows_once, rw_rows); hdrs_once -= std::min(hdrs_once, rw_hdrs); }
     p.n_rows_read = rows_read;
     (void)bound;
-    p.algo_bytes = rows_read * sizeof(Row) + hdrs_read * sizeof(StrHdr) + h->out.list_bytes +
+    p.algo_bytes = rows_read * sizeof(Row) + hdrs_read * sizeof(StrHdr) + h->out.list_bytes + h->out.rw_bytes +
                    t->dir_bytes * (1 + e->extra.size()) + plan_bytes + (uint64_t)p.n_constraints * p.n_tiles * 16 + (uint64_t)p.list_total * 8;
     p.algo_bytes_once = p.algo_bytes - (rows_read - rows_once) * sizeof(Row) - (hdrs_read - hdrs_once) * sizeof(StrHdr) - t->dir_bytes * e->extra.size();
     p.n_plan_groups = 1 + (uint32_t)e->extra.size();
@@ -3250,6 +3256,7 @@
   if (strcmp(key, "group_max") == 0) { g_debug_group_max.store((int)std::max<int64_t>(0, std::min<int64_t>(value, 1 << 20))); return GK_OK; }
   if (strcmp(key, "verify_flip") == 0) { g_debug_verify_flip.store(value < 0 ? -1 : value); return GK_OK; }
   if (strcmp(key, "fold_match_labels") == 0) { g_test_fold_match_labels.store(value != 0); return GK_OK; }
+  if (strcmp(key, "keep_slot_index") == 0) { g_debug_keep_slot_index.store(value != 0); return GK_OK; }
   return fail(GK_ERR_NOT_FOUND, std::string("gk_debug_set: unknown key ") + key);
 }
 
@@ -3261,6 +3268,58 @@
   dev_jit_cache_stats(&h, &c);
   if (cache_hits) *cache_hits = h;
   if (compiles) *compiles = c;
+}
+
+int gk_table_review_words(gk_engine* e, const gk_table* t, char** text_out) {
+  if (!e || !t || !text_out) return fail(GK_ERR_INVALID, "NULL argument");
+  try {
+    ensure_plan(e);
+    std::shared_lock<std::shared_mutex> l(e->plan_rw);
+    const HostPlan& p = e->fast;
+    const HostTable& h = t->host;
+    const uint32_t n_groups = h.n_tiles(), S = h.n_slots();
+    if (h.tile_idx.size() != (size_t)n_groups * (S + 1u)) return fail(GK_ERR_INVALID, "the table did not keep its slot index: gk_debug_set(\"keep_slot_index\", 1) before it is created");
+    std::vector<std::vector<Pred>> classes;
+    const std::vector<uint32_t> cls = jit_path_classes(p, &classes);
+    const ReviewWords rw = analyse_review_words(classes, p.dims.n_gwords);
+    std::vector<BoundPath> bound, kept, hoisted;
+    for (uint32_t s = 0; s < S; s++) {
+      const uint32_t path = h.slot_path[s];
+      if (path >= cls.size() || !cls[path]) continue;
+      const uint32_t ent = p.ptab[path];
+      bound.push_back(BoundPath{s, cls[path], pred_list_cost<Pred>(&p.path_preds[ent >> 8], ent & 0xFF, [](const Pred& q) { return pred_needs_str(q); })});
+    }
+    split_bound(bound, rw, &kept, &hoisted);
+    const int block = gk_block_of((int)h.rpt);
+    const uint32_t list_cap = (uint32_t)std::min(block / GK_TILE, 8) * GK_WAVE_CHUNKS, n_waves = (uint32_t)(block / GK_TILE);
+    const ChunkLists full = build_chunk_lists(h.tile_idx.data(), n_groups, S, bound, list_cap, n_waves);
+    const ChunkLists part = build_chunk_lists(h.tile_idx.data(), n_groups, S, kept, list_cap, n_waves);
+    uint32_t only = 0, only_ok = 0;
+    for (uint32_t g = 0; g < n_groups; g++) {
+      const uint32_t* ix = h.tile_idx.data() + (size_t)g * (S + 1u);
+      bool any_h = false, any_k = false;
+      for (const BoundPath& b : hoisted) any_h = any_h || ix[b.slot + 1u] > ix[b.slot];
+      for (const BoundPath& b : kept) any_k = any_k || ix[b.slot + 1u] > ix[b.slot];
+      if (!any_h || any_k) continue;
+      only++;
+      const ChunkDesc& hd = part.d[(size_t)g * part.capg];
+      if (hd.st == 0u && hd.info == 0u) only_ok++;
+    }
+    uint32_t n_hoisted_classes = 0;
+    for (size_t c = 1; c < rw.hoisted.size(); c++) n_hoisted_classes += rw.hoisted[c] ? 1u : 0u;
+    std::ostringstream os;
+    os << "n_gwords=" << p.dims.n_gwords << "\nclasses=" << (classes.size() ? classes.size() - 1 : 0) << "\nhoisted_classes=" << n_hoisted_classes << "\nk=" << rw.k() << "\nwords=";
+    for (uint32_t k = 0; k < rw.k(); k++) os << (k ? "," : "") << rw.words[k];
+    os << "\nrpt=" << h.rpt << "\ngroups=" << n_groups << "\nbound_paths=" << bound.size() << "\nkept_paths=" << kept.size() << "\nhoisted_paths=" << hoisted.size()
+       << "\nchunks_full=" << full.n_chunks << "\nchunks_kept=" << part.n_chunks << "\ncapg_full=" << full.capg << "\ncapg_kept=" << part.capg
+       << "\noverflow_groups_full=" << full.n_overflow_groups << "\noverflow_groups_kept=" << part.n_overflow_groups
+       << "\ngroups_only_hoisted=" << only << "\ngroups_only_hoisted_with_empty_list=" << only_ok << "\n";
+    const std::string s = os.str();
+    char* buf = (char*)malloc(s.size() + 1);
+    memcpy(buf, s.c_str(), s.size() + 1);
+    *text_out = buf;
+    return GK_OK;
+  } catch (const std::exception& ex) { return fail(GK_ERR_INTERNAL, ex.what()); }
 }
 
 int gk_dump(gk_engine* e, char** text_out) {
diff --git a/gatekeeper_amd/csrc/jit_source.hpp b/gatekeeper_amd/csrc/jit_source.hpp
--- a/gatekeeper_amd/csrc/jit_source.hpp
+++ b/gatekeeper_amd/csrc/jit_source.hpp
@@ -9,6 +9,7 @@
 #include "codegen.hpp"
 #include "lower.hpp"
 #include "plan.hpp"
+#include "review_words.hpp"
 
 namespace gk {
 
@@ -76,7 +77,16 @@
 }
 
 inline std::string assemble_jit_source(const HostPlan& plan, uint32_t rpt, uint32_t rpp, const char* plan_hpp,
-                                       const char* vm_core_hpp, const char* kernel_body, uint32_t list_cap = 0) {
+                                       const char* vm_core_hpp, const char* kernel_body, uint32_t list_cap = 0,
+                                       const std::vector<uint32_t>* rw_words = nullptr) {
+  std::vector<uint32_t> rw_forced;
+  if (const char* f = getenv("GK_JIT_REVIEW_WORDS"); !rw_words && f && std::string(f) == "force") {
+    std::vector<std::vector<Pred>> classes;
+    jit_path_classes(plan, &classes);
+    rw_forced = analyse_review_words(classes, plan.dims.n_gwords).words;
+    rw_words = &rw_forced;
+  }
+  const bool rw = rw_words && !rw_words->empty();
   std::string src =
       "typedef unsigned char uint8_t; typedef unsigned short uint16_t; typedef unsigned int uint32_t; typedef unsigned long long uint64_t;\n"
       "typedef short int16_t; typedef int int32_t; typedef long long int64_t;\n";
@@ -114,6 +124,11 @@
   src += "#define GK_RPT_K " + std::to_string(rpt) + "\n#define GK_RPP_K " + std::to_string(rpp) + "\n";
   if (list_cap) src += "#define GK_LIST_CAP_K " + std::to_string(list_cap) + "\n";
   if (const uint32_t tk = jit_tot_k(plan.dims.n_constraints, (size_t)plan.dims.acc_words * rpp * 4, rpt, block, jit_res_k(plan), list_cap ? list_cap : list_cap_of(block))) src += "#define GK_TOT_K " + std::to_string(tk) + "\n";
+  if (rw) {
+    std::string sel = "0u";
+    for (size_t k = rw_words->size(); k-- > 0;) sel = "(k) == " + std::to_string(k) + "u ? " + std::to_string((*rw_words)[k]) + "u : " + sel;
+    src += "#define GK_RW_K " + std::to_string(rw_words->size()) + "\n#define GK_RW_WORD(k) (" + sel + ")\n";
+  }
   if (const char* defs = getenv("GK_JIT_DEFINES")) {
     std::string d = defs, item;
     for (size_t i = 0; i <= d.size(); i++) {
@@ -133,6 +148,12 @@
     while (fgets(buf, sizeof buf, f)) { line = buf; if (line.rfind("#include", 0) != 0 && line.rfind("#pragma once", 0) != 0) body += line; }
     fclose(f);
     src += body;
+  } else if (rw) {
+#ifdef GK_HAVE_BODY_RW
+    src += kKernelBodyRw;
+#else
+    throw std::runtime_error("the review-words kernel body is not part of this build");
+#endif
   } else src += kernel_body;
   src += "}\n";
   return src;
diff --git a/gatekeeper_amd/csrc/kernels.hip b/gatekeeper_amd/csrc/kernels.hip
--- a/gatekeeper_amd/csrc/kernels.hip
+++ b/gatekeeper_amd/csrc/kernels.hip
@@ -26,7 +26,10 @@
 #include "code_cache.hpp"
 #include "codegen.hpp"
 #include "device.hpp"
+#include "jit_body_rw.inc"
+#define GK_HAVE_BODY_RW 1
 #include "jit_source.hpp"
+#include "review_words.hpp"
 #include "shard_pipe.hpp"
 #include "jit_sources.inc"
 #include "vm_core.hpp"
@@ -173,7 +176,12 @@
   uint32_t rpt = GK_RPT_MIN;
   std::vector<uint32_t> slot_path;
   std::shared_ptr<const std::vector<uint32_t>> h_tile_idx;
-  struct Binding { uint64_t plan_id = 0; Bind* d = nullptr; uint32_t n = 0; ChunkDesc* lists = nullptr; uint32_t capg = 1; uint64_t list_bytes = 0; };
+  struct Binding {
+    uint64_t plan_id = 0; Bind* d = nullptr; uint32_t n = 0; ChunkDesc* lists = nullptr; uint32_t capg = 1; uint64_t list_bytes = 0;
+    uint32_t* rwords = nullptr; Bind* rw_bind = nullptr; uint32_t rw_k = 0, rw_stride = 0; uint64_t rw_plan = 0, rw_rows = 0, rw_hdr_rows = 0;
+    bool lists_hoisted = false;
+    void free_all() { pool_free(d); pool_free(lists); pool_free(rwords); pool_free(rw_bind); d = nullptr; lists = nullptr; rwords = nullptr; rw_bind = nullptr; }
+  };
   Binding bind_fast, bind_big;
   bool is_view = false;
   uint64_t chunk_need_plan = 0;
@@ -200,6 +208,7 @@
   std::string source;
   uint64_t source_hash = 0;
   uint32_t tot_k = 0;
+  bool rw = false;
 };
 struct JitSlot {
   std::mutex mu;
@@ -225,7 +234,10 @@
   std::vector<uint32_t> cls;
   std::vector<uint32_t> path_cost;
   uint32_t res_k = GK_MAX_VIOL + 2 * GK_MAX_RES, n_scopes = 0;
+  ReviewWords rw;
 };
+
+static bool rw_on(const DevPlan* p, const DevTable* t) { return t && p->want_jit && review_words_wanted(p->rw, t->rpt, t->n_reviews); }
 
 #define GK_RPT_K 64
 #define GK_KERNEL_TILES gk_eval_tiles_64
@@ -709,9 +721,9 @@
   if (t->stream) { stream_release(t->device, t->stream); t->stream = nullptr; }
   else (void)hipStreamSynchronize(0);
   dev_table_free_work(t);
-  if (t->is_view) { pool_free(t->bind_fast.d); pool_free(t->bind_big.d); pool_free(t->bind_fast.lists); delete t; return; }
+  t->bind_fast.free_all(); t->bind_big.free_all();
+  if (t->is_view) { delete t; return; }
   pool_free(t->rows); pool_free(t->shdr); pool_free(t->tile_idx); pool_free(t->rflags); pool_free(t->heap);
-  pool_free(t->bind_fast.d); pool_free(t->bind_big.d); pool_free(t->bind_fast.lists);
   delete t;
 }
 uint64_t dev_table_bytes(const DevTable* t) { return t->bytes; }
@@ -853,6 +865,7 @@
     p->host_fast = fast;
     std::vector<std::vector<Pred>> classes;
     p->cls = jit_path_classes(fast, &classes);
+    p->rw = analyse_review_words(classes, fast.dims.n_gwords);
   }
   p->path_cost.assign(fast.ptab.size(), 0);
   for (size_t i = 0; i < fast.ptab.size(); i++) {
@@ -884,7 +897,13 @@
   const uint32_t n_groups = (t->n_reviews + t->rpt - 1) / t->rpt, S = t->n_slots;
   const uint32_t* ix = t->h_tile_idx->data();
   std::vector<uint32_t> slots;
-  for (uint32_t s = 0; s < t->slot_path.size(); s++) { const uint32_t path = t->slot_path[s]; if (path < p->ptab_fast.size() && p->ptab_fast[path]) slots.push_back(s); }
+  const bool rw = rw_on(p, t);
+  for (uint32_t s = 0; s < t->slot_path.size(); s++) {
+    const uint32_t path = t->slot_path[s];
+    if (path >= p->ptab_fast.size() || !p->ptab_fast[path]) continue;
+    if (rw && path < p->cls.size() && p->rw.is_hoisted(p->cls[path] & ~GK_ENT_NEEDS_STR)) continue;
+    slots.push_back(s);
+  }
   uint32_t most = 0;
   for (uint32_t g = 0; g < n_groups; g++) {
     uint32_t n = 0;
@@ -923,22 +942,23 @@
   std::shared_ptr<JitSlot> slot;
   {
     std::lock_guard<std::mutex> l(p->jit_mu);
-    const uint32_t key = (rpt * 1024u + rpp) ^ (list_cap << 20);
+    const bool rw = rw_on(p, t);
+    const uint32_t key = ((rpt * 1024u + rpp) ^ (list_cap << 20)) | (rw ? 1u << 31 : 0u);
     auto it = p->jit.find(key);
     if (it != p->jit.end()) slot = it->second;
     else {
       slot = std::make_shared<JitSlot>();
       p->jit.emplace(key, slot);
       std::string src;
-      try { src = assemble_jit_source(p->host_fast, rpt, rpp, kPlanHpp, kVmCoreHpp, kKernelBody, list_cap); }
+      try { src = assemble_jit_source(p->host_fast, rpt, rpp, kPlanHpp, kVmCoreHpp, kKernelBody, list_cap, rw ? &p->rw.words : nullptr); }
       catch (const std::exception& ex) { slot->state = JitSlot::FAILED; slot->error = ex.what(); }
       if (slot->state == JitSlot::PENDING) {
         const int device = p->device;
         const uint32_t res_k = jit_res_k(p->host_fast), tot_k = jit_tot_k(p->host_fast.dims.n_constraints, (size_t)p->host_fast.dims.acc_words * rpp * 4, rpt, jit_block_of(rpt), res_k, list_cap ? list_cap : list_cap_of(jit_block_of(rpt)));
-        auto build = [slot, src, device, rpt, res_k, list_cap, tot_k]() {
+        auto build = [slot, src, device, rpt, res_k, list_cap, tot_k, rw]() {
           std::unique_ptr<JitKernel> k;
           std::string err;
-          try { k.reset(jit_build(device, src, rpt, res_k, list_cap, tot_k)); } catch (const std::exception& ex) { err = ex.what(); }
+          try { k.reset(jit_build(device, src, rpt, res_k, list_cap, tot_k)); k->rw = rw; } catch (const std::exception& ex) { err = ex.what(); }
           std::lock_guard<std::mutex> l(slot->mu);
           slot->k = std::move(k);
           slot->error = err;
@@ -1030,6 +1050,7 @@
     PlanView pv{};
     const Row* rows = nullptr; const StrHdr* shdr = nullptr; const ChunkDesc* lists = nullptr; const uint32_t* rflags = nullptr; const uint8_t* heap = nullptr;
     const ConstraintSlot* slots = nullptr;
+    const uint32_t* rwords = nullptr; uint32_t rws = 0;
     uint32_t cg = 0, nn = 0, nt = 0, dd = 0, rp = 0;
     OutPtrs out{};
   } cached;
@@ -1133,8 +1154,74 @@
   b->plan_id = plan_id;
 }
 
+struct RwSlots { uint8_t of[GK_RW_MAX_WORD]; };
+struct ReviewWordAcc {
+  uint32_t* rwords;
+  uint32_t n_pad, review;
+  const RwSlots* sl;
+  __device__ void or_word(uint32_t w, uint32_t m) { if (w < GK_RW_MAX_WORD && sl->of[w] != 0xFFu) atomicOr(&rwords[(size_t)sl->of[w] * n_pad + review], m); }
+  __device__ void max_word(uint32_t, uint32_t) {}
+  __device__ void store_word(uint32_t, uint32_t) {}
+  __device__ uint32_t load(uint32_t) const { return 0u; }
+};
+__global__ __launch_bounds__(256) void gk_bind_review_words(PlanView pv, const Row* __restrict__ rows, const StrHdr* __restrict__ shdr,
+                                                            const uint32_t* __restrict__ tile_idx, uint32_t n_slots, const Bind* __restrict__ bind,
+                                                            uint32_t n_bind, const uint8_t* __restrict__ heap, uint32_t n_reviews, uint32_t rpt,
+                                                            RwSlots sl, uint32_t* __restrict__ rwords, uint32_t n_pad) {
+  const uint32_t group = blockIdx.x;
+  const uint32_t* __restrict__ ix = tile_idx + (size_t)group * (n_slots + 1u);
+  for (uint32_t k = 0; k < n_bind; k++) {
+    const Bind b = bind[k];
+    const uint32_t row_lo = ix[b.slot], row_hi = ix[b.slot + 1u];
+    for (uint32_t i = row_lo + threadIdx.x; i < row_hi; i += blockDim.x) {
+      const uint4 v = reinterpret_cast<const uint4*>(rows)[i];
+      Row rw{v.x, v.y, v.z, v.w};
+      const uint32_t review = group * rpt + (rw.rev & ROW_REV_MASK);
+      if (review >= n_reviews) continue;
+      const uint4 s = reinterpret_cast<const uint4*>(shdr)[i];
+      StrHdr h = {{s.x, s.y, s.z, s.w}};
+      ReviewWordAcc acc{rwords, n_pad, review, &sl};
+      eval_row_ent(rw, i, b.ent, h, pv, heap, acc);
+    }
+  }
+}
+
+static void bind_review_words(DevTable* t, DevTable::Binding* b, const DevPlan* p) {
+  if (b->rw_plan == p->id && b->rwords) return;
+  if (!t->h_tile_idx) throw std::runtime_error("table without a host slot index");
+  std::vector<Bind> v;
+  uint64_t n_rows = 0, n_hdr = 0;
+  const uint32_t n_groups = (t->n_reviews + t->rpt - 1) / t->rpt;
+  const uint32_t* ix = t->h_tile_idx->data();
+  for (uint32_t s = 0; s < t->slot_path.size(); s++) {
+    const uint32_t path = t->slot_path[s];
+    if (path >= p->cls.size() || !p->cls[path] || !p->rw.is_hoisted(p->cls[path] & ~GK_ENT_NEEDS_STR) || path >= p->ptab_fast.size() || !p->ptab_fast[path]) continue;
+    v.push_back(Bind{s, p->ptab_fast[path]});
+    uint64_t n = 0;
+    for (uint32_t g = 0; g < n_groups; g++) n += ix[(size_t)g * (t->n_slots + 1u) + s + 1u] - ix[(size_t)g * (t->n_slots + 1u) + s];
+    n_rows += n;
+    if (p->cls[path] & GK_ENT_NEEDS_STR) n_hdr += n;
+  }
+  RwSlots sl;
+  memset(sl.of, 0xFF, sizeof sl.of);
+  for (uint32_t k = 0; k < p->rw.k(); k++) sl.of[p->rw.words[k]] = (uint8_t)k;
+  if (b->rwords) { if (t->work) t->work->drop_graph(); (void)hipStreamSynchronize(t->stream); }
+  pool_free(b->rwords); pool_free(b->rw_bind);
+  b->rwords = nullptr; b->rw_bind = nullptr;
+  const uint32_t n_pad = (t->n_reviews + 63u) / 64u * 64u;
+  HIP_OK(pool_malloc(&b->rwords, (size_t)p->rw.k() * n_pad * 4));
+  b->rw_bind = upload(v.data(), v.size());
+  HIP_OK(hipMemsetAsync(b->rwords, 0, (size_t)p->rw.k() * n_pad * 4, t->stream));
+  if (!v.empty() && n_groups) {
+    hipLaunchKernelGGL(gk_bind_review_words, dim3(n_groups), dim3(256), 0, t->stream, p->fast.view(), t->rows, t->shdr, t->tile_idx, t->n_slots,
+                       b->rw_bind, (uint32_t)v.size(), t->heap, t->n_reviews, t->rpt, sl, b->rwords, n_pad);
+    HIP_OK(hipGetLastError());
+  }
+  b->rw_k = p->rw.k(); b->rw_stride = n_pad; b->rw_plan = p->id; b->rw_rows = n_rows; b->rw_hdr_rows = n_hdr;
+}
+
 static void bind_chunks(DevTable* t, DevTable::Binding* b, uint64_t key, const std::vector<uint32_t>& entries, const std::vector<uint32_t>& cost,
-                        bool generic, int block, uint32_t list_cap) {
+                        bool generic, int block, uint32_t list_cap, const ReviewWords* hoist = nullptr) {
   if (b->plan_id == key && b->lists) return;
   if (!t->h_tile_idx) throw std::runtime_error("table without a host slot index");
   std::vector<BoundPath> bound;
@@ -1144,6 +1231,8 @@
     if (generic && entries[path] > GK_DESC_ENT_MASK) throw Unsupported("plan too large for the chunk descriptors (predicate table beyond 2^17 entries)");
     bound.push_back(BoundPath{s, entries[path], path < cost.size() ? cost[path] : 1u});
   }
+  if (hoist) { std::vector<BoundPath> kept; split_bound(bound, *hoist, &kept, nullptr); bound.swap(kept); }
+  b->lists_hoisted = hoist != nullptr;
   const uint32_t n_groups = (t->n_reviews + t->rpt - 1) / t->rpt;
   ChunkLists cl = build_chunk_lists(t->h_tile_idx->data(), n_groups, t->n_slots, std::move(bound), list_cap, (uint32_t)(block / GK_TILE));
   if (b->lists) (void)hipStreamSynchronize(t->stream);
@@ -1235,7 +1324,7 @@
     cw->per_launch = false;
     cw->partial_rows = c.grid; cw->partial_stride = c.tot_k; cw->partial_live = true;
     cw->lds_bytes = c.lds; cw->kernel_hash = c.kernel_hash;
-    void* args[] = {&c.pv, &c.rows, &c.shdr, &c.lists, &c.cg, &c.rflags, &c.heap, &c.nn, &c.nt, &c.slots, &c.out, &c.dd, &c.rp};
+    void* args[] = {&c.pv, &c.rows, &c.shdr, &c.lists, &c.cg, &c.rflags, &c.heap, &c.nn, &c.nt, &c.slots, &c.out, &c.dd, &c.rp, &c.rwords, &c.rws};
     HIP_OK(hipModuleLaunchKernel(c.fn, c.grid, 1, 1, c.block, 1, 1, c.lds, stream, args, nullptr));
     return;
   }
@@ -1283,8 +1372,9 @@
   else if ((size_t)p->fast.dims.acc_words * rpp * 4 > max_dyn_lds_of(rpt)) {
     while (rpp > (uint32_t)GK_TILE && (size_t)p->fast.dims.acc_words * rpp * 4 > max_dyn_lds_of(rpt)) rpp /= 2;
   }
+  if (jit && jit->rw) bind_review_words(mt, &mt->bind_fast, p);
   bind_chunks(mt, &mt->bind_fast, (p->id * 2 + (jit ? 1 : 0)) * 2048 + (uint64_t)block, jit ? p->cls : p->ptab_fast, p->path_cost, !jit, block,
-              jit ? jit_lcap : list_cap_of(block));
+              jit ? jit_lcap : list_cap_of(block), jit && jit->rw ? &p->rw : nullptr);
   const size_t lds = (size_t)p->fast.dims.acc_words * rpp * 4;
   const uint32_t dbg = dbg_phase | (n_groups >= 1024u ? (stagger << 8) | (stagger_mode << 20) : 0u);
   uint32_t grid = grid_for(t->device, n_groups, lds + static_lds_of(rpt, block, jit ? p->res_k : 0, jit ? jit_lcap : 0, jit ? jit->tot_k : 0), block);
@@ -1316,12 +1406,16 @@
     const ChunkDesc* lists = t->bind_fast.lists;
     uint32_t nn = n, nt = n_tiles, dd = dbg, cg = t->bind_fast.capg, rp = rpp;
     const ConstraintSlot* slots = p->slots;
-    void* args[] = {&pv, &rows, &shdr, &lists, &cg, &rflags, &heap, &nn, &nt, &slots, &out, &dd, &rp};
+    const uint32_t* rwords = jit->rw ? t->bind_fast.rwords : nullptr;
+    uint32_t rws = jit->rw ? t->bind_fast.rw_stride : 0u;
+    if (jit->rw && (!rwords || !t->bind_fast.lists_hoisted || t->bind_fast.rw_k != p->rw.k())) throw std::runtime_error("review-words kernel without its binding");
+    void* args[] = {&pv, &rows, &shdr, &lists, &cg, &rflags, &heap, &nn, &nt, &slots, &out, &dd, &rp, &rwords, &rws};
     HIP_OK(hipModuleLaunchKernel(jit->tiles, grid, 1, 1, block, 1, 1, (unsigned)lds, stream, args, nullptr));
     if (fused_totals && !opt.detached && !per_launch && opt.list_capacity == 0 && !w->d_prof) {
       Work::Launch& c = w->cached;
       c.want_match = opt.want_match; c.fn = jit->tiles; c.grid = grid; c.block = (uint32_t)block; c.lds = (uint32_t)lds;
       c.tot_k = jit->tot_k; c.kernel_hash = jit->source_hash; c.pv = pv; c.rows = rows; c.shdr = shdr; c.lists = lists; c.rflags = rflags; c.heap = heap;
+      c.rwords = rwords; c.rws = rws;
       c.slots = slots; c.cg = cg; c.nn = nn; c.nt = nt; c.dd = dd; c.rp = rp; c.out = out;
       c.plan = p->id;
     }
@@ -1373,6 +1467,7 @@
   o->kernel_hash = w->kernel_hash;
   o->specialised = w->kernel_hash != 0;
   o->list_bytes = t->bind_fast.list_bytes;
+  if (t->bind_fast.lists_hoisted) { o->rw_bytes = (uint64_t)t->bind_fast.rw_k * t->bind_fast.rw_stride * 4; o->rw_rows = t->bind_fast.rw_rows; o->rw_hdr_rows = t->bind_fast.rw_hdr_rows; }
   o->fast_kernel_ms = total / (float)(w->per_launch || !w->timed ? w->pending : w->pending - w->timed_from);
   o->kernel_ms = o->fast_kernel_ms;
   w->pending = 0;
diff --git a/gatekeeper_amd/csrc/review_words.hpp b/gatekeeper_amd/csrc/review_words.hpp
--- /dev/null
+++ b/gatekeeper_amd/csrc/review_words.hpp
@@ -0,0 +1,60 @@
+#pragma once
+#include <algorithm>
+#include <cstdint>
+#include <cstdlib>
+#include <vector>
+
+#include "chunks.hpp"
+#include "plan.hpp"
+
+namespace gk {
+
+struct ReviewWords {
+  std::vector<uint8_t> hoisted;
+  std::vector<uint32_t> words;
+  uint32_t k() const { return (uint32_t)words.size(); }
+  bool is_hoisted(uint32_t cls) const { return cls < hoisted.size() && hoisted[cls] != 0; }
+  int slot_of(uint32_t word) const {
+    for (size_t i = 0; i < words.size(); i++) if (words[i] == word) return (int)i;
+    return -1;
+  }
+};
+
+constexpr uint32_t GK_RW_MAX_WORD = 32;
+
+inline ReviewWords analyse_review_words(const std::vector<std::vector<Pred>>& classes, uint32_t n_gwords) {
+  n_gwords = std::min(n_gwords, GK_RW_MAX_WORD);
+  ReviewWords rw;
+  rw.hoisted.assign(classes.size(), 0);
+  for (size_t c = 1; c < classes.size(); c++) {
+    bool all = !classes[c].empty();
+    for (const Pred& p : classes[c]) all = all && p.dst == D_GLOBAL && p.op != P_STORE && p.op != P_PRESENT && (uint32_t)(p.bit >> 5) < n_gwords;
+    if (!all) continue;
+    rw.hoisted[c] = 1;
+    for (const Pred& p : classes[c]) rw.words.push_back((uint32_t)(p.bit >> 5));
+  }
+  std::sort(rw.words.begin(), rw.words.end());
+  rw.words.erase(std::unique(rw.words.begin(), rw.words.end()), rw.words.end());
+  return rw;
+}
+
+inline void split_bound(const std::vector<BoundPath>& bound, const ReviewWords& rw, std::vector<BoundPath>* kept, std::vector<BoundPath>* hoisted) {
+  for (const BoundPath& b : bound) {
+    if (rw.is_hoisted(b.ent & ~GK_ENT_NEEDS_STR)) { if (hoisted) hoisted->push_back(b); }
+    else if (kept) kept->push_back(b);
+  }
+}
+
+inline bool review_words_enabled() {
+  static const bool on = !(getenv("GK_REVIEW_WORDS") && atoi(getenv("GK_REVIEW_WORDS")) == 0);
+  return on;
+}
+inline uint32_t review_words_min_reviews() {
+  static const uint32_t n = getenv("GK_REVIEW_WORDS_MIN") ? (uint32_t)atoll(getenv("GK_REVIEW_WORDS_MIN")) : 8192u;
+  return n;
+}
+inline bool review_words_wanted(const ReviewWords& rw, uint32_t rpt, uint32_t n_reviews) {
+  return review_words_enabled() && rw.k() > 0 && rpt >= 128u && n_reviews >= review_words_min_reviews();
+}
+
+}
diff --git a/gatekeeper_amd/driver.py b/gatekeeper_amd/driver.py
--- a/gatekeeper_amd/driver.py
+++ b/gatekeeper_amd/driver.py
@@ -500,6 +500,17 @@
                  | (L.GK_TABLE_PRUNED if pruned else 0))
         self._check(self.lib.gk_table_create(self.handle, reviews_ptr, n, flags, st, C.byref(h)))
         return Table(self, h, st, n)
+
+    def table_review_words(self, table):
+        p = C.c_void_p()
+        self._check(self.lib.gk_table_review_words(self.handle, table.handle, C.byref(p)))
+        s = C.string_at(p).decode()
+        self.lib.gk_free(p)
+        out = {}
+        for line in s.splitlines():
+            k, _, v = line.partition("=")
+            out[k] = [int(x) for x in v.split(",") if x] if k == "words" else int(v)
+        return out
 
     def dump(self):
         p = C.c_void_p()
diff --git a/include/gkgpu.h b/include/gkgpu.h
--- a/include/gkgpu.h
+++ b/include/gkgpu.h
@@ -292,6 +292,7 @@
 int gk_debug_set(const char* key, int64_t value);
 
 int gk_dump(gk_engine* e, char** text_out);
+int gk_table_review_words(gk_engine* e, const gk_table* t, char** text_out);
 
 #ifdef __cplusplus
 }
```

Result: faster. 1485 billion evals/s (median of 6 runs) (+7.1%).
